# PKU-DAIR/SGL

Hardware: AMD Instinct MI355X
Metric: pre-prop SpMM throughput (edge·featdim/s), ogbn-products k=3, 1/2/4/8 GPU (higher is better)
Workload: dtype f32

## Files before the change

include/sgl_hip.h:

```cpp
#ifndef SGL_HIP_H
#define SGL_HIP_H

#include <stddef.h>
#include <stdint.h>

#ifdef __cplusplus
extern "C" {
#endif

#define SGL_OK 0
#define SGL_ERR_INVALID 1001
#define SGL_ERR_NO_DEVICE 1002
#define SGL_ERR_UNSUPPORTED 1003
#define SGL_ERR_ALLOC 1004

#define SGL_MAX_HOPS 64

int sgl_version(void);
const char *sgl_last_error(void);
int sgl_device_count(int *count);
int sgl_set_tuning(const char *key, int64_t value);
int sgl_get_tuning(const char *key, int64_t *value);

typedef struct sgl_plan sgl_plan_t;
int sgl_plan_build(sgl_plan_t **out, const int64_t *h_rowptr, int64_t n_rows, int32_t item_nnz, int32_t long_row_nnz);
int sgl_plan_counts(const sgl_plan_t *plan, int64_t counts[8]);
int sgl_plan_export(const sgl_plan_t *plan, int32_t *h_items, int64_t *h_piece_begin, int32_t *h_piece_len,
                    int32_t *h_piece_row, int32_t *h_long_row, int32_t *h_long_first);
void sgl_plan_destroy(sgl_plan_t *plan);

typedef struct sgl_csr sgl_csr_t;

#define SGL_CSR_STRICT_ORDER 0x1u
#define SGL_CSR_NO_XCD_REMAP 0x2u

int sgl_csr_create(sgl_csr_t **out, int64_t n_rows, int64_t n_cols, int64_t nnz, const int64_t *d_rowptr,
                   const int32_t *d_col, const float *d_val, uint32_t flags, int32_t item_nnz,
                   int32_t long_row_nnz, void *stream);
int sgl_csr_destroy(sgl_csr_t *csr);
int sgl_csr_set_values(sgl_csr_t *csr, const float *d_val);
int sgl_csr_info(const sgl_csr_t *csr, int64_t info[8]);

int sgl_spmm_f32(sgl_csr_t *csr, const float *d_x, int64_t ldx, float *d_y, int64_t ldy, int64_t d,
                 int accumulate, void *stream);

int sgl_spmm_multi_f32(sgl_csr_t *csr, const float *d_x, int64_t ldx, int n_out, float *const *h_y, int64_t ldy,
                       int64_t d, const uint8_t *d_row_mask, void *stream);

int sgl_spmm_chain_f32(sgl_csr_t *csr, int n_hops, const float *d_x0, int64_t ldx0, float *const *h_y,
                       const int64_t *h_ldy, int64_t d, void *stream);

typedef struct sgl_graph sgl_graph_t;
int sgl_chain_graph_create(sgl_graph_t **out, sgl_csr_t *csr, int n_hops, const float *d_x0, int64_t ldx0,
                           float *const *h_y, const int64_t *h_ldy, int64_t d);
int sgl_chain_graph_launch(sgl_graph_t *graph, void *stream);
int sgl_chain_graph_destroy(sgl_graph_t *graph);

int sgl_spmm_axpb_clamp_f32(sgl_csr_t *csr, const float *d_x, int64_t ldx, float *d_y, int64_t ldy, int64_t d,
                            float alpha, const float *d_res, int64_t ldres, float lo, float hi, void *stream);

enum { SGL_ACC_SUM = 0, SGL_ACC_WSUM = 1, SGL_ACC_MAX = 2, SGL_ACC_MIN = 3 };
int sgl_spmm_acc_f32(sgl_csr_t *csr, const float *d_x, int64_t ldx, float *d_y, int64_t ldy, int64_t d, float *d_acc,
                     int64_t ldacc, float w, int mode, float divisor, void *stream);

int sgl_spmm_bf16(sgl_csr_t *csr, const uint16_t *d_x, int64_t ldx, uint16_t *d_y, int64_t ldy, int64_t d, void *stream);
int sgl_spmm_chain_bf16(sgl_csr_t *csr, int n_hops, const uint16_t *d_x0, int64_t ldx0, uint16_t *const *h_y,
                        const int64_t *h_ldy, int64_t d, void *stream);
int sgl_spmm_acc_bf16(sgl_csr_t *csr, const uint16_t *d_x, int64_t ldx, uint16_t *d_y, int64_t ldy, int64_t d, float *d_acc,
                      int64_t ldacc, float w, int mode, float divisor, void *stream);
int sgl_gather_rows_bf16_f32(const uint16_t *d_x, int64_t ldx, int64_t n_rows, const int64_t *d_idx, int64_t n_idx, float *d_out,
                             int64_t ldo, int64_t d, int64_t pad_cols, void *stream);
int sgl_gather_hops_bf16_f32(int n_hops, const uint16_t *const *h_x, const int64_t *h_ldx, int64_t n_rows, const int64_t *d_idx,
                             int64_t n_idx, float *const *h_out, const int64_t *h_ldo, int64_t d, int64_t pad_cols, void *stream);

int sgl_hop_reduce_bf16_f32(int op, int n_hops, const uint16_t *const *h_x, const int64_t *h_ldx, const float *d_w, float *d_out,
                            int64_t ldo, int64_t pad_cols, int64_t n, int64_t d, void *stream);
int sgl_hop_concat_bf16(int n_hops, const uint16_t *const *h_x, const int64_t *h_ldx, uint16_t *d_out, int64_t ldo, int64_t pad_cols,
                        int64_t n, int64_t d, void *stream);
int sgl_hop_concat_bf16_f32(int n_hops, const uint16_t *const *h_x, const int64_t *h_ldx, float *d_out, int64_t ldo, int64_t pad_cols,
                            int64_t n, int64_t d, void *stream);
int sgl_nafs_bf16_f32(int n_hops, const uint16_t *const *h_x, const int64_t *h_ldx, float *d_out, int64_t ldo, int64_t pad_cols,
                      float *d_w_out, int64_t ldw, int64_t n, int64_t d, void *stream);

int sgl_download(void *h_dst, const void *d_src, int64_t bytes, void *stream);

int sgl_reorder_community(const int64_t *d_rowptr, const int32_t *d_col, int64_t n, int rounds, int64_t *d_order,
                          int64_t *h_info, void *stream);
int sgl_reorder_lpa_round(const int64_t *d_rowptr, const int32_t *d_col, int64_t n_local, int64_t row0, int64_t n_global,
                          const int32_t *d_labels, int32_t *d_out, int round, int last, uint64_t *d_moved, void *stream);

int sgl_csr_permute_rows(const int64_t *d_rowptr, const int32_t *d_col, const float *d_val, int64_t n, const int32_t *d_perm,
                         int64_t *d_out_rowptr, int32_t *d_out_col, float *d_out_val, void *stream);
int sgl_csr_set_rowmap(sgl_csr_t *csr, const int32_t *d_rowmap, void *stream);

int sgl_allgather_rows(void *nccl_comm, int rank, int world, const int64_t *h_bounds, float *d_x, int64_t ldx, void *stream);
int sgl_exchange_rows(void *nccl_comm, int rank, int world, const float *d_send, const int64_t *h_send_off, float *d_recv,
                      const int64_t *h_recv_off, int64_t ld, void *stream);
const char *sgl_exchange_backend(void);
int sgl_exchange_selftest(void *nccl_comm, int rank, const float *d_src, float *d_dst, int64_t n, int n_ops, void *stream);

void FloatCSRMulDenseOMP(float answer[], float data[], int indices[], int indptr[], float mat[], int mat_row,
                         int mat_col);
int FloatCSRMulDense(float answer[], int data_nnz, float data[], int indices[], int indptr[], float mat[],
                     int mat_row, int mat_col);

int sgl_shim_cache_stats(int64_t *hits, int64_t *misses);

int sgl_norm_prepare(int64_t n, int64_t nnz, const int64_t *d_rowptr, const int32_t *d_col, int64_t *nnz_out,
                     void *stream);
int sgl_norm_execute(int64_t n, int64_t nnz, const int64_t *d_rowptr, const int32_t *d_col, const float *d_val,
                     double r, int use_alpha, double alpha, int64_t nnz_out, int64_t *d_out_rowptr,
                     int32_t *d_out_col, float *d_out_val, double *d_out_val64, void *stream);

int sgl_norm_degrees(int64_t n, int64_t row0, const int64_t *d_rowptr, const int32_t *d_col, const float *d_val,
                     double *d_deg, void *stream);
int sgl_norm_execute_lr(int64_t n, int64_t nnz, const int64_t *d_rowptr, const int32_t *d_col, const float *d_val,
                        const double *d_left, const double *d_right, int use_alpha, double alpha, int64_t nnz_out,
                        int64_t *d_out_rowptr, int32_t *d_out_col, float *d_out_val, double *d_out_val64, void *stream);

int sgl_norm_block_prepare(int64_t n, int64_t row0, int64_t nnz, const int64_t *d_rowptr, const int32_t *d_col,
                           int64_t *nnz_out, void *stream);
int sgl_norm_block_build(int64_t n, int64_t row0, int64_t nnz, const int64_t *d_rowptr, const int32_t *d_col,
                         const float *d_val, int64_t nnz_out, int64_t *d_out_rowptr, int32_t *d_out_col,
                         double *d_out_val64, double *d_rowsum, void *stream);
int sgl_norm_build_symcheck(int64_t n, int64_t nnz, const int64_t *d_rowptr, const int32_t *d_col, const float *d_val,
                            int64_t nnz_out, int64_t *d_out_rowptr, int32_t *d_out_col, double *d_out_val64, double *d_rowsum,
                            uint64_t *d_sym_hash, void *stream);
int sgl_norm_block_colsum(int64_t n_cols, int64_t nnz, const int32_t *d_col, const double *d_val64, double *d_colsum,
                          void *stream);
int sgl_norm_block_scale(int64_t n, int64_t row0, const int64_t *d_rowptr, const int32_t *d_col, const double *d_val64,
                         const double *d_left_local, const double *d_right_global, int use_alpha, double alpha,
                         float *d_out_val, double *d_out_val64, void *stream);
int sgl_norm_block_mix(int64_t n, int64_t row0, const int64_t *d_rowptr, const int32_t *d_col, const double *d_hat64,
                       double alpha, float *d_out_val, double *d_out_val64, void *stream);
int sgl_norm_block_diag_positions(int64_t n, int64_t row0, const int64_t *d_rowptr, const int32_t *d_col, int64_t *d_diag, void *stream);
int sgl_norm_block_mix_at(int64_t nnz, int64_t n, const double *d_hat64, const int64_t *d_diag, double alpha, float *d_out_val,
                          double *d_out_val64, void *stream);
int sgl_norm_degree_powers(int64_t n, const double *d_deg, double r, double *d_left, double *d_right, void *stream);

int sgl_coo_to_csr(int64_t n_rows, int64_t n_cols, int64_t nnz, const int64_t *d_row, const int64_t *d_col,
                   const float *d_val, int64_t *d_out_rowptr, int32_t *d_out_col, float *d_out_val, int64_t *h_nnz_out,
                   void *stream);

#define SGL_REDUCE_SUM 0
#define SGL_REDUCE_MEAN 1
#define SGL_REDUCE_MAX 2
#define SGL_REDUCE_MIN 3
#define SGL_REDUCE_WSUM 4

int sgl_hop_reduce_f32(int op, int n_hops, const float *const *h_x, const int64_t *h_ldx, const float *d_w,
                       float *d_out, int64_t ldo, int64_t n, int64_t d, void *stream);
int sgl_hop_wsum2d_f32(int n_hops, const float *const *h_x, const int64_t *h_ldx, const float *d_w, int64_t ldw,
                       float *d_out, int64_t ldo, int64_t n, int64_t d, void *stream);
int sgl_hop_wsum2d_bwd_f32(int n_hops, const float *const *h_x, const int64_t *h_ldx, const float *d_w, int64_t ldw,
                           const float *d_dout, int64_t lddo, float *d_dw, int64_t lddw, float *const *h_dx,
                           const int64_t *h_lddx, int64_t n, int64_t d, void *stream);
int sgl_hop_rowdot_f32(int n_hops, const float *const *h_x, const int64_t *h_ldx, const float *d_vec, float *d_out,
                       int64_t ldo, int64_t n, int64_t d, void *stream);
int64_t sgl_hop_wsum1d_bwd_scratch(int n_hops);
int sgl_hop_wsum1d_bwd_f32(int n_hops, const float *const *h_x, const int64_t *h_ldx, const float *d_dout,
                           int64_t lddo, float *d_dw, float *d_scratch, int64_t n, int64_t d, void *stream);
int sgl_hop_lincomb_f32(int n_in, const float *const *h_x, const int64_t *h_ldx, int n_out, float *const *h_out, const int64_t *h_ldo,
                        const float *d_w, int64_t ldw, int64_t n, int64_t d, void *stream);
int sgl_hop_select_bwd_f32(int op, int n_hops, const float *const *h_x, const int64_t *h_ldx, const float *d_gout, int64_t ldg,
                           float *const *h_dx, const int64_t *h_lddx, int64_t n, int64_t d, void *stream);
int sgl_hop_concat_f32(int n_hops, const float *const *h_x, const int64_t *h_ldx, float *d_out, int64_t ldo,
                       int64_t n, int64_t d, void *stream);
int sgl_hop_concat_padded_f32(int n_hops, const float *const *h_x, const int64_t *h_ldx, float *d_out, int64_t ldo,
                              int64_t pad_cols, int64_t n, int64_t d, void *stream);
int sgl_nafs_f32(int n_hops, const float *const *h_x, const int64_t *h_ldx, float *d_out, int64_t ldo,
                 float *d_w_out, int64_t ldw, int64_t n, int64_t d, void *stream);
int sgl_nafs_padded_f32(int n_hops, const float *const *h_x, const int64_t *h_ldx, float *d_out, int64_t ldo, int64_t pad_cols,
                        float *d_w_out, int64_t ldw, int64_t n, int64_t d, void *stream);
int sgl_nafs_prefix_f32(int n_hops, const float *const *h_x, const int64_t *h_ldx, uint64_t emit_mask, float *const *h_out,
                        const int64_t *h_ldo, int64_t pad_cols, int combine, float divisor, int64_t n, int64_t d, void *stream);

int sgl_hop_gate_f32(int n_hops, const float *const *h_x, const int64_t *h_ldx, const float *d_vec, float bias, float *d_out,
                     int64_t ldo, float *d_w_out, int64_t ldw, float *d_g_out, int64_t ldg, int64_t n, int64_t d, void *stream);
int sgl_hop_gate_padded_f32(int n_hops, const float *const *h_x, const int64_t *h_ldx, const float *d_vec, float bias, float *d_out,
                            int64_t ldo, int64_t pad_cols, float *d_w_out, int64_t ldw, float *d_g_out, int64_t ldg, int64_t n,
                            int64_t d, void *stream);
int sgl_hop_recursive_f32(int n_hops, const float *const *h_x, const int64_t *h_ldx, const float *d_vec, float bias, float *d_out,
                          int64_t ldo, int64_t pad_cols, float *d_w_out, int64_t ldw, float *d_a_out, int64_t lda, float *d_c_out,
                          int64_t ldc, int64_t n, int64_t d, void *stream);
int sgl_hop_recursive_bwd_f32(int n_hops, const float *d_a, int64_t lda, const float *d_c, int64_t ldc, float bias, const float *d_bias,
                              const float *d_gw, int64_t ldg, float *d_da, int64_t ldda, float *d_dc, int64_t lddc, float *d_db,
                              int64_t n, void *stream);
int64_t sgl_hop_colsum_scratch(int n_hops, int64_t n, int64_t d);
int sgl_hop_colsum_f32(int n_hops, const float *const *h_x, const int64_t *h_ldx, const float *d_w, int64_t ldw, int sw, float *d_out,
                       int64_t ldo, float *d_scratch, int64_t n, int64_t d, void *stream);
int sgl_hop_rowdot2_f32(int n_hops, const float *const *h_x, const int64_t *h_ldx, const float *d_u, int64_t ldu, uint64_t u_mask,
                        const float *d_vec, int h0, int h1, float *d_p, int64_t ldp, float *d_a, int64_t n, int64_t d, void *stream);
int sgl_gather_rows_f32(const float *d_x, int64_t ldx, int64_t n_rows, const int64_t *d_idx, int64_t n_idx,
                        float *d_out, int64_t ldo, int64_t d, void *stream);
int sgl_gather_rows_padded_f32(const float *d_x, int64_t ldx, int64_t n_rows, const int64_t *d_idx, int64_t n_idx, float *d_out,
                               int64_t ldo, int64_t d, int64_t pad_cols, void *stream);
int sgl_gather_hops_padded_f32(int n_hops, const float *const *h_x, const int64_t *h_ldx, int64_t n_rows, const int64_t *d_idx,
                               int64_t n_idx, float *const *h_out, const int64_t *h_ldo, int64_t d, int64_t pad_cols, void *stream);
int sgl_scatter_rows_f32(const float *d_x, int64_t ldx, int64_t n_rows, const int64_t *d_src, const int64_t *d_dst,
                         int64_t n_idx, float *d_out, int64_t ldo, int64_t n_out_rows, int64_t d, void *stream);

int sgl_edge_dot_f32(const float *d_a, int64_t lda, int64_t n_a, const float *d_b, int64_t ldb, int64_t n_b,
                     const int64_t *d_edges, int64_t n_edges, int64_t d, float *d_out, void *stream);

int sgl_col_signature_f32(const float *d_x, int64_t ldx, int64_t n, int64_t d, uint64_t *d_sig, void *stream);

int sgl_content_hash(const void *h_ptr, int64_t bytes, uint64_t *out);

#ifdef __cplusplus
}
#endif
#endif
```

sgl_amd/_lib.py:

```python
import ctypes
import os
from ctypes import POINTER, c_char_p, c_double, c_float, c_int, c_int32, c_int64, c_uint32, c_uint64, c_void_p

import torch

_HERE = os.path.dirname(os.path.abspath(__file__))
LIB_PATH = os.environ.get("SGL_HIP_LIB") or os.path.join(_HERE, "csrc", "libsgl_hip.so")

SGL_CSR_STRICT_ORDER = 0x1
SGL_CSR_NO_XCD_REMAP = 0x2
SGL_REDUCE_SUM, SGL_REDUCE_MEAN, SGL_REDUCE_MAX, SGL_REDUCE_MIN, SGL_REDUCE_WSUM = 0, 1, 2, 3, 4
SGL_MAX_HOPS = 64
SGL_ERR_UNSUPPORTED = 1003
SGL_MEM_DEFAULT, SGL_MEM_CONTIGUOUS, SGL_MEM_VMM = 0, 1, 2

_lib = None

PROTOTYPES = {
    "sgl_version": (c_int, []),
    "sgl_last_error": (c_char_p, []),
    "sgl_device_count": (c_int, [POINTER(c_int)]),
    "sgl_set_tuning": (c_int, [c_char_p, c_int64]),
    "sgl_get_tuning": (c_int, [c_char_p, POINTER(c_int64)]),
    "sgl_plan_build": (c_int, [POINTER(c_void_p), c_void_p, c_int64, c_int32, c_int32]),
    "sgl_plan_counts": (c_int, [c_void_p, POINTER(c_int64)]),
    "sgl_plan_export": (c_int, [c_void_p, c_void_p, c_void_p, c_void_p, c_void_p, c_void_p, c_void_p]),
    "sgl_plan_destroy": (None, [c_void_p]),
    "sgl_csr_create": (c_int, [POINTER(c_void_p), c_int64, c_int64, c_int64, c_void_p, c_void_p, c_void_p, c_uint32,
                               c_int32, c_int32, c_void_p]),
    "sgl_csr_destroy": (c_int, [c_void_p]),
    "sgl_csr_set_values": (c_int, [c_void_p, c_void_p]),
    "sgl_csr_info": (c_int, [c_void_p, POINTER(c_int64)]),
    "sgl_spmm_f32": (c_int, [c_void_p, c_void_p, c_int64, c_void_p, c_int64, c_int64, c_int, c_void_p]),
    "sgl_spmm_multi_f32": (c_int, [c_void_p, c_void_p, c_int64, c_int, c_void_p, c_int64, c_int64, c_void_p, c_void_p]),
    "sgl_spmm_chain_f32": (c_int, [c_void_p, c_int, c_void_p, c_int64, c_void_p, c_void_p, c_int64, c_void_p]),
    "sgl_chain_graph_create": (c_int, [POINTER(c_void_p), c_void_p, c_int, c_void_p, c_int64, c_void_p, c_void_p, c_int64]),
    "sgl_chain_graph_launch": (c_int, [c_void_p, c_void_p]),
    "sgl_chain_graph_destroy": (c_int, [c_void_p]),
    "sgl_spmm_axpb_clamp_f32": (c_int, [c_void_p, c_void_p, c_int64, c_void_p, c_int64, c_int64, c_float, c_void_p, c_int64,
                                        c_float, c_float, c_void_p]),
    "sgl_spmm_acc_f32": (c_int, [c_void_p, c_void_p, c_int64, c_void_p, c_int64, c_int64, c_void_p, c_int64, c_float, c_int,
                                 c_float, c_void_p]),
    "sgl_spmm_bf16": (c_int, [c_void_p, c_void_p, c_int64, c_void_p, c_int64, c_int64, c_void_p]),
    "sgl_spmm_chain_bf16": (c_int, [c_void_p, c_int, c_void_p, c_int64, c_void_p, c_void_p, c_int64, c_void_p]),
    "sgl_spmm_acc_bf16": (c_int, [c_void_p, c_void_p, c_int64, c_void_p, c_int64, c_int64, c_void_p, c_int64, c_float, c_int,
                                  c_float, c_void_p]),
    "sgl_gather_rows_bf16_f32": (c_int, [c_void_p, c_int64, c_int64, c_void_p, c_int64, c_void_p, c_int64, c_int64, c_int64,
                                         c_void_p]),
    "sgl_gather_hops_bf16_f32": (c_int, [c_int, c_void_p, c_void_p, c_int64, c_void_p, c_int64, c_void_p, c_void_p, c_int64, c_int64,
                                         c_void_p]),
    "sgl_hop_reduce_bf16_f32": (c_int, [c_int, c_int, c_void_p, c_void_p, c_void_p, c_void_p, c_int64, c_int64, c_int64, c_int64,
                                        c_void_p]),
    "sgl_hop_concat_bf16": (c_int, [c_int, c_void_p, c_void_p, c_void_p, c_int64, c_int64, c_int64, c_int64, c_void_p]),
    "sgl_hop_concat_bf16_f32": (c_int, [c_int, c_void_p, c_void_p, c_void_p, c_int64, c_int64, c_int64, c_int64, c_void_p]),
    "sgl_nafs_bf16_f32": (c_int, [c_int, c_void_p, c_void_p, c_void_p, c_int64, c_int64, c_void_p, c_int64, c_int64, c_int64,
                                  c_void_p]),
    "sgl_allgather_rows": (c_int, [c_void_p, c_int, c_int, c_void_p, c_void_p, c_int64, c_void_p]),
    "sgl_exchange_rows": (c_int, [c_void_p, c_int, c_int, c_void_p, c_void_p, c_void_p, c_void_p, c_int64, c_void_p]),
    "sgl_exchange_backend": (c_char_p, []),
    "sgl_exchange_selftest": (c_int, [c_void_p, c_int, c_void_p, c_void_p, c_int64, c_int, c_void_p]),
    "FloatCSRMulDenseOMP": (None, [c_void_p, c_void_p, c_void_p, c_void_p, c_void_p, c_int, c_int]),
    "FloatCSRMulDense": (c_int, [c_void_p, c_int, c_void_p, c_void_p, c_void_p, c_void_p, c_int, c_int]),
    "sgl_shim_cache_stats": (c_int, [POINTER(c_int64), POINTER(c_int64)]),
    "sgl_norm_prepare": (c_int, [c_int64, c_int64, c_void_p, c_void_p, POINTER(c_int64), c_void_p]),
    "sgl_norm_execute": (c_int, [c_int64, c_int64, c_void_p, c_void_p, c_void_p, c_double, c_int, c_double, c_int64,
                                 c_void_p, c_void_p, c_void_p, c_void_p, c_void_p]),
    "sgl_norm_degrees": (c_int, [c_int64, c_int64, c_void_p, c_void_p, c_void_p, c_void_p, c_void_p]),
    "sgl_norm_execute_lr": (c_int, [c_int64, c_int64, c_void_p, c_void_p, c_void_p, c_void_p, c_void_p, c_int, c_double,
                                    c_int64, c_void_p, c_void_p, c_void_p, c_void_p, c_void_p]),
    "sgl_norm_block_prepare": (c_int, [c_int64, c_int64, c_int64, c_void_p, c_void_p, POINTER(c_int64), c_void_p]),
    "sgl_norm_block_build": (c_int, [c_int64, c_int64, c_int64, c_void_p, c_void_p, c_void_p, c_int64, c_void_p, c_void_p,
                                     c_void_p, c_void_p, c_void_p]),
    "sgl_norm_build_symcheck": (c_int, [c_int64, c_int64, c_void_p, c_void_p, c_void_p, c_int64, c_void_p, c_void_p, c_void_p,
                                        c_void_p, c_void_p, c_void_p]),
    "sgl_norm_block_colsum": (c_int, [c_int64, c_int64, c_void_p, c_void_p, c_void_p, c_void_p]),
    "sgl_norm_block_scale": (c_int, [c_int64, c_int64, c_void_p, c_void_p, c_void_p, c_void_p, c_void_p, c_int, c_double,
                                     c_void_p, c_void_p, c_void_p]),
    "sgl_norm_block_mix": (c_int, [c_int64, c_int64, c_void_p, c_void_p, c_void_p, c_double, c_void_p, c_void_p, c_void_p]),
    "sgl_norm_block_diag_positions": (c_int, [c_int64, c_int64, c_void_p, c_void_p, c_void_p, c_void_p]),
    "sgl_norm_block_mix_at": (c_int, [c_int64, c_int64, c_void_p, c_void_p, c_double, c_void_p, c_void_p, c_void_p]),
    "sgl_norm_degree_powers": (c_int, [c_int64, c_void_p, c_double, c_void_p, c_void_p, c_void_p]),
    "sgl_coo_to_csr": (c_int, [c_int64, c_int64, c_int64, c_void_p, c_void_p, c_void_p, c_void_p, c_void_p, c_void_p,
                               POINTER(c_int64), c_void_p]),
    "sgl_download": (c_int, [c_void_p, c_void_p, c_int64, c_void_p]),
    "sgl_csr_permute_rows": (c_int, [c_void_p, c_void_p, c_void_p, c_int64, c_void_p, c_void_p, c_void_p, c_void_p, c_void_p]),
    "sgl_csr_set_rowmap": (c_int, [c_void_p, c_void_p, c_void_p]),
    "sgl_reorder_lpa_round": (c_int, [c_void_p, c_void_p, c_int64, c_int64, c_int64, c_void_p, c_void_p, c_int, c_int, c_void_p, c_void_p]),
    "sgl_reorder_community": (c_int, [c_void_p, c_void_p, c_int64, c_int, c_void_p, POINTER(c_int64), c_void_p]),
    "sgl_hop_reduce_f32": (c_int, [c_int, c_int, c_void_p, c_void_p, c_void_p, c_void_p, c_int64, c_int64, c_int64,
                                   c_void_p]),
    "sgl_hop_lincomb_f32": (c_int, [c_int, c_void_p, c_void_p, c_int, c_void_p, c_void_p, c_void_p, c_int64, c_int64, c_int64, c_void_p]),
    "sgl_hop_select_bwd_f32": (c_int, [c_int, c_int, c_void_p, c_void_p, c_void_p, c_int64, c_void_p, c_void_p, c_int64, c_int64,
                                       c_void_p]),
    "sgl_hop_wsum2d_f32": (c_int, [c_int, c_void_p, c_void_p, c_void_p, c_int64, c_void_p, c_int64, c_int64, c_int64,
                                   c_void_p]),
    "sgl_hop_wsum2d_bwd_f32": (c_int, [c_int, c_void_p, c_void_p, c_void_p, c_int64, c_void_p, c_int64, c_void_p,
                                       c_int64, c_void_p, c_void_p, c_int64, c_int64, c_void_p]),
    "sgl_hop_rowdot_f32": (c_int, [c_int, c_void_p, c_void_p, c_void_p, c_void_p, c_int64, c_int64, c_int64, c_void_p]),
    "sgl_hop_gate_f32": (c_int, [c_int, c_void_p, c_void_p, c_void_p, c_float, c_void_p, c_int64, c_void_p, c_int64, c_void_p,
                                 c_int64, c_int64, c_int64, c_void_p]),
    "sgl_hop_rowdot2_f32": (c_int, [c_int, c_void_p, c_void_p, c_void_p, c_int64, c_uint64, c_void_p, c_int, c_int, c_void_p,
                                    c_int64, c_void_p, c_int64, c_int64, c_void_p]),
    "sgl_hop_colsum_scratch": (c_int64, [c_int, c_int64, c_int64]),
    "sgl_hop_colsum_f32": (c_int, [c_int, c_void_p, c_void_p, c_void_p, c_int64, c_int, c_void_p, c_int64, c_void_p, c_int64, c_int64,
                                   c_void_p]),
    "sgl_hop_wsum1d_bwd_scratch": (c_int64, [c_int]),
    "sgl_hop_wsum1d_bwd_f32": (c_int, [c_int, c_void_p, c_void_p, c_void_p, c_int64, c_void_p, c_void_p, c_int64,
                                       c_int64, c_void_p]),
    "sgl_hop_concat_f32": (c_int, [c_int, c_void_p, c_void_p, c_void_p, c_int64, c_int64, c_int64, c_void_p]),
    "sgl_hop_concat_padded_f32": (c_int, [c_int, c_void_p, c_void_p, c_void_p, c_int64, c_int64, c_int64, c_int64, c_void_p]),
    "sgl_nafs_f32": (c_int, [c_int, c_void_p, c_void_p, c_void_p, c_int64, c_void_p, c_int64, c_int64, c_int64,
                             c_void_p]),
    "sgl_nafs_padded_f32": (c_int, [c_int, c_void_p, c_void_p, c_void_p, c_int64, c_int64, c_void_p, c_int64, c_int64, c_int64,
                                    c_void_p]),
    "sgl_nafs_prefix_f32": (c_int, [c_int, c_void_p, c_void_p, c_uint64, c_void_p, c_void_p, c_int64, c_int, c_float, c_int64, c_int64,
                                    c_void_p]),
    "sgl_hop_gate_padded_f32": (c_int, [c_int, c_void_p, c_void_p, c_void_p, c_float, c_void_p, c_int64, c_int64, c_void_p, c_int64,
                                        c_void_p, c_int64, c_int64, c_int64, c_void_p]),
    "sgl_hop_recursive_f32": (c_int, [c_int, c_void_p, c_void_p, c_void_p, c_float, c_void_p, c_int64, c_int64, c_void_p, c_int64,
                                      c_void_p, c_int64, c_void_p, c_int64, c_int64, c_int64, c_void_p]),
    "sgl_hop_recursive_bwd_f32": (c_int, [c_int, c_void_p, c_int64, c_void_p, c_int64, c_float, c_void_p, c_void_p, c_int64, c_void_p,
                                          c_int64, c_void_p, c_int64, c_void_p, c_int64, c_void_p]),
    "sgl_gather_rows_f32": (c_int, [c_void_p, c_int64, c_int64, c_void_p, c_int64, c_void_p, c_int64, c_int64,
                                    c_void_p]),
    "sgl_gather_rows_padded_f32": (c_int, [c_void_p, c_int64, c_int64, c_void_p, c_int64, c_void_p, c_int64, c_int64, c_int64,
                                           c_void_p]),
    "sgl_gather_hops_padded_f32": (c_int, [c_int, c_void_p, c_void_p, c_int64, c_void_p, c_int64, c_void_p, c_void_p, c_int64, c_int64,
                                           c_void_p]),
    "sgl_scatter_rows_f32": (c_int, [c_void_p, c_int64, c_int64, c_void_p, c_void_p, c_int64, c_void_p, c_int64, c_int64,
                                     c_int64, c_void_p]),
    "sgl_edge_dot_f32": (c_int, [c_void_p, c_int64, c_int64, c_void_p, c_int64, c_int64, c_void_p, c_int64, c_int64, c_void_p,
                                 c_void_p]),
    "sgl_col_signature_f32": (c_int, [c_void_p, c_int64, c_int64, c_int64, c_void_p, c_void_p]),
    "sgl_content_hash": (c_int, [c_void_p, c_int64, POINTER(c_uint64)]),
}


PROBE_LIB_PATH = os.environ.get("SGL_PROBE_LIB") or os.path.join(_HERE, "csrc", "libsgl_probe.so")
PROBE_PROTOTYPES = {
    "sgl_probe_last_error": (c_char_p, []),
    "sgl_synth_degrees": (c_int, [c_uint64, c_int64, c_int64, c_void_p, c_void_p, c_void_p]),
    "sgl_synth_fill": (c_int, [c_uint64, c_int64, c_int64, c_int64, c_void_p, c_void_p, c_void_p, c_void_p]),
    "sgl_synth_features": (c_int, [c_uint64, c_int64, c_int64, c_int64, c_int64, c_void_p, c_void_p]),
    "sgl_mem_alloc": (c_int, [POINTER(c_void_p), c_int64, c_int, c_int64]),
    "sgl_mem_free": (c_int, [c_void_p]),
    "sgl_probe_stream_f32": (c_int, [c_void_p, c_int64, c_void_p, c_void_p]),
    "sgl_probe_gather_f32": (c_int, [c_void_p, c_int64, c_void_p, c_int64, c_int, c_int, c_void_p, c_void_p]),
}
_probe = None


class SglHipError(RuntimeError):
    pass


def lib():
    global _lib
    if _lib is None:
        if not os.path.exists(LIB_PATH):
            raise SglHipError(
                f"{LIB_PATH} is missing: build it with `python -m sgl_amd.csrc.build` (needs hipcc). "
                "sgl_amd has no CPU fallback for the propagation hot path.")
        handle = ctypes.CDLL(LIB_PATH)
        for name, (res, args) in PROTOTYPES.items():
            fn = getattr(handle, name)
            fn.restype = res
            fn.argtypes = args
        _lib = handle
    return _lib


def probe_lib():
    global _probe
    if _probe is None:
        if not os.path.exists(PROBE_LIB_PATH):
            raise SglHipError(f"{PROBE_LIB_PATH} is missing: build it with `python -m sgl_amd.csrc.build` (needs hipcc)")
        handle = ctypes.CDLL(PROBE_LIB_PATH)
        for name, (res, args) in PROBE_PROTOTYPES.items():
            fn = getattr(handle, name)
            fn.restype = res
            fn.argtypes = args
        _probe = handle
    return _probe


def check_probe(rc, what=""):
    if rc != 0:
        raise SglHipError(f"{what or 'libsgl_probe'} failed (code {rc}): {probe_lib().sgl_probe_last_error().decode('utf-8', 'replace')}")


def last_error():
    return lib().sgl_last_error().decode("utf-8", "replace")


def check(rc, what=""):
    if rc != 0:
        raise SglHipError(f"{what or 'libsgl_hip'} failed (code {rc}): {last_error()}")


def device_count():
    n = c_int(0)
    check(lib().sgl_device_count(ctypes.byref(n)), "sgl_device_count")
    return n.value


def require_gpu():
    if not torch.cuda.is_available() or device_count() < 1:
        raise SglHipError("no MI355X/HIP device visible: the sgl_amd propagation path is GPU-only (no CPU fallback)")


def set_tuning(key, value):
    check(lib().sgl_set_tuning(key.encode(), int(value)), f"sgl_set_tuning({key})")


def get_tuning(key):
    v = c_int64(0)
    check(lib().sgl_get_tuning(key.encode(), ctypes.byref(v)), f"sgl_get_tuning({key})")
    return v.value


def current_stream_ptr():
    return ctypes.c_void_p(torch.cuda.current_stream().cuda_stream)


def ptr(t):
    return ctypes.c_void_p(t.data_ptr())


def hop_arrays(tensors):
    n = len(tensors)
    ptrs = (c_void_p * n)(*[t.data_ptr() for t in tensors])
    lds = (c_int64 * n)(*[t.stride(0) if t.shape[0] > 1 else max(t.shape[1], t.stride(0)) for t in tensors])
    return ptrs, lds


def content_hash(arr):
    import numpy as np
    a = np.ascontiguousarray(arr)
    h = c_uint64(0)
    check(lib().sgl_content_hash(c_void_p(a.ctypes.data), a.nbytes, ctypes.byref(h)), "sgl_content_hash")
    return int(h.value)
```

sgl_amd/csrc/sgl_common.h:

```cpp
#pragma once
#include <hip/hip_runtime.h>

#include <cstdarg>
#include <cstdint>
#include <cstdio>
#include <cstring>
#include <string>
#include <vector>

#include "../../include/sgl_hip.h"

#define SGL_EXPORT extern "C" __attribute__((visibility("default")))

namespace sgl {

void set_error(const char *fmt, ...) __attribute__((format(printf, 1, 2)));
const char *get_error();

inline int fail(int code, const char *fmt, ...) __attribute__((format(printf, 2, 3)));
inline int fail(int code, const char *fmt, ...) {
    char buf[512];
    va_list ap;
    va_start(ap, fmt);
    vsnprintf(buf, sizeof(buf), fmt, ap);
    va_end(ap);
    set_error("%s", buf);
    return code;
}

#define SGL_HIP_CHECK(expr)                                                                          \
    do {                                                                                             \
        hipError_t _e = (expr);                                                                      \
        if (_e != hipSuccess)                                                                        \
            return ::sgl::fail((int)_e, "%s failed: %s (%s:%d)", #expr, hipGetErrorString(_e), __FILE__, \
                               __LINE__);                                                            \
    } while (0)

#define SGL_REQUIRE(cond, ...)                                     \
    do {                                                           \
        if (!(cond)) return ::sgl::fail(SGL_ERR_INVALID, __VA_ARGS__); \
    } while (0)

struct Piece {
    int64_t begin;
    int32_t len;
    int32_t row;
};

struct Plan {
    int64_t n_rows = 0;
    std::vector<int32_t> items;
    std::vector<Piece> pieces;
    std::vector<int32_t> long_row;
    std::vector<int32_t> long_first;
    int64_t max_item_rows = 0, max_item_nnz = 0;
};

constexpr int kMaxItemRows = 63;
constexpr int kDefaultItemNnz = 512;
constexpr int kDefaultLongRowNnz = 2048;
constexpr int64_t kSmallLaunchNnz = 100000000;

int build_plan(Plan &plan, const int64_t *rowptr, int64_t n_rows, int32_t item_nnz, int32_t long_row_nnz);

int64_t tuning(const char *key, int64_t dflt);

int32_t default_item_nnz(int64_t nnz);
int32_t default_long_row_nnz(int64_t nnz);

struct SpmmLayout {
    int group, nch, ulevel, waves;
    bool nt;
};
SpmmLayout spmm_layout(int lanes, bool strict, int64_t nnz, int64_t n_rows, bool bf16);

constexpr int unroll_of(int group, int nch, int ulevel) {
    const int uh = (nch == 1) ? 8 : (nch == 2 ? 4 : 2);
    return ulevel == 2 ? uh * 2 / (nch == 1 ? 1 : 2) : ulevel == 3 ? ((nch == 1 && group == 64) ? 32 : uh) : ulevel == 0 ? uh / 2 : uh;
}

struct RowLayout {
    int lpr, ch;
};
struct RowInstance {
    int lpr, ch, hmax;
};
int pick_lpr(int64_t d, int vec);
RowLayout row_layout(int64_t d, int n_hops, bool allow_8x5 = false);
RowInstance row_instance(int64_t d, int n_hops, bool allow_8x5 = false);
int out_cols(int64_t d, int64_t pad, int64_t room);
int check_pad(const char *who, int64_t width, int64_t pad, int64_t ldo);

inline hipStream_t as_stream(void *s) { return reinterpret_cast<hipStream_t>(s); }

inline bool launch_fits(int64_t blocks, int64_t threads_per_block) {
    return blocks >= 0 && blocks * threads_per_block < ((int64_t)1 << 32) && blocks < (int64_t)INT32_MAX;
}

}

inline bool aligned_to(const void *p, size_t a) { return (reinterpret_cast<uintptr_t>(p) % a) == 0; }

struct sgl_plan {
    sgl::Plan p;
};
```

sgl_amd/csrc/sgl_core.cpp:

```cpp
#include <algorithm>
#include <atomic>
#include <map>
#include <mutex>
#include <thread>

#include "sgl_common.h"

namespace sgl {

static thread_local std::string g_err;

void set_error(const char *fmt, ...) {
    char buf[512];
    va_list ap;
    va_start(ap, fmt);
    vsnprintf(buf, sizeof(buf), fmt, ap);
    va_end(ap);
    g_err = buf;
}
const char *get_error() { return g_err.c_str(); }

static std::mutex g_tune_mu;
static std::map<std::string, int64_t> &tune_map() {
    static std::map<std::string, int64_t> m = {
        {"spmm_unroll", 0},
        {"spmm_vec", 0},
        {"spmm_nt", 0},
        {"spmm_group", 0},
        {"spmm_waves", 0},
        {"spmm_xcd_remap", 1},
        {"spmm_heavy_first", 1},
        {"agg_blocks", 0},
        {"nafs_fused", 1},
        {"row_lpr32x2", 1},
        {"row_whole_lines", 1},
        {"row_narrow_groups", 1},
        {"gather_lpr", 0},
        {"gather_hops_grid", 1},
        {"gather_rows_per_thread", 0},
        {"concat_flat_read", 1},
        {"concat_lds", 1},
    };
    return m;
}

int64_t tuning(const char *key, int64_t dflt) {
    std::lock_guard<std::mutex> lk(g_tune_mu);
    auto &m = tune_map();
    auto it = m.find(key);
    if (it == m.end()) return dflt;
    return it->second;
}

int32_t default_item_nnz(int64_t nnz) {
    const int64_t want_items = 256 * 4 * 8;
    const int64_t cap = nnz >= kSmallLaunchNnz ? kDefaultItemNnz : kDefaultItemNnz / 2;
    return (int32_t)std::min<int64_t>(cap, std::max<int64_t>(16, nnz / want_items));
}

int32_t default_long_row_nnz(int64_t nnz) {
    return nnz < (1 << 18) ? 32 : nnz < (1 << 20) ? 128 : nnz < (1 << 22) ? 512 : kDefaultLongRowNnz;
}

SpmmLayout spmm_layout(int lanes, bool strict, int64_t nnz, int64_t n_rows, bool bf16) {
    SpmmLayout L;
    L.group = 64;
    L.nch = 1;
    if (lanes > 64) {
        const int need = (lanes + 63) / 64;
        L.nch = need <= 2 ? need : 4;
    } else if (!strict && lanes <= 16) {
        L.group = 8;
        while (L.group < lanes) L.group <<= 1;
    }
    const int64_t forced = tuning("spmm_group", 0);
    if (!strict && (forced == 8 || forced == 16 || forced == 32 || forced == 64) && L.nch == 1 && forced >= lanes) L.group = (int)forced;
    const bool whole_wave = L.group == 64 && L.nch == 1;
    L.ulevel = whole_wave ? 2 : 1;
    if (L.nch == 1 && n_rows > 0) {
        const double avg = (double)nnz / (double)n_rows;
        if (whole_wave) {
            if (avg < 12.0) L.ulevel = 0;
            else if (avg < 40.0) L.ulevel = 1;
        } else {
            L.ulevel = bf16 ? (avg >= 40.0 ? 2 : 1) : 1;
        }
    }
    const int64_t un = tuning("spmm_unroll", 0);
    if (un == 1) L.ulevel = 0;
    if (un == 2) L.ulevel = 2;
    if (un == 3) L.ulevel = 1;
    if (un == 4) L.ulevel = bf16 ? L.ulevel : 3;
    L.nt = bf16 ? false : tuning("spmm_nt", 0) != 0;
    L.waves = (int)tuning("spmm_waves", 0);
    if (L.waves != 1 && L.waves != 2 && L.waves != 4) L.waves = 4;
    return L;
}

int pick_lpr(int64_t d, int vec) {
    const int64_t lanes = (d + vec - 1) / vec;
    int lpr = 8;
    while (lpr < lanes && lpr < 64) lpr <<= 1;
    return lpr;
}

static const int kNarrow[2][3] = {{16, 3, 12}, {8, 5, 6}};

RowLayout row_layout(int64_t d, int n_hops, bool allow_8x5) {
    RowLayout r;
    r.lpr = pick_lpr(d, 4);
    r.ch = (d > r.lpr * 4) ? 2 : 1;
    if (r.lpr == 64 && r.ch == 1 && d > 128 && tuning("row_lpr32x2", 1) != 0) {
        r.lpr = 32;
        r.ch = 2;
    }
    if (tuning("row_narrow_groups", 1) != 0 && d <= r.lpr * 4 * r.ch) {
        const int slots = (int)((d + 3) / 4);
        const int64_t mode = tuning("row_narrow_groups", 1);
        for (const auto &c : kNarrow) {
            const int idle = c[0] * c[1] - slots;
            if (((mode == 2 || !allow_8x5) && c[0] == 8) || (mode == 3 && c[0] == 16)) continue;
            if (idle >= 0 && n_hops <= c[2] && 2 * idle <= r.lpr * r.ch - slots) {
                r.lpr = c[0];
                r.ch = c[1];
            }
        }
    }
    return r;
}

RowInstance row_instance(int64_t d, int n_hops, bool allow_8x5) {
    const RowLayout r = row_layout(d, n_hops, allow_8x5);
    int most = 16;
    for (const auto &c : kNarrow)
        if (r.lpr == c[0] && r.ch == c[1]) most = c[2];
    const int hmax = (n_hops < 1 || n_hops > most) ? 0 : std::max(2, (n_hops + 1) / 2 * 2);
    return RowInstance{r.lpr, r.ch, hmax};
}

int out_cols(int64_t d, int64_t pad, int64_t room) {
    int64_t dw = tuning("row_whole_lines", 1) != 0 ? d + pad : d;
    if (dw > room) dw = room > d ? room / 4 * 4 : d;
    if (dw > d && dw % 4 != 0) dw = d;
    return (int)dw;
}

int check_pad(const char *who, int64_t width, int64_t pad, int64_t ldo) {
    if (pad < 0 || width + pad > ldo) return fail(SGL_ERR_INVALID, "%s: pad_cols=%lld does not fit the output pitch", who, (long long)pad);
    if (pad > 0 && ((width + pad) % 4 != 0 || ldo % 4 != 0))
        return fail(SGL_ERR_INVALID, "%s: padded rows must be whole 16-byte vectors (width + pad_cols and ldo multiples of 4)", who);
    return SGL_OK;
}

static void heavy_items_first(Plan &plan, const int64_t *rowptr, int32_t item_nnz) {
    const int64_t n = (int64_t)plan.items.size() / 2;
    if (n < 64) return;
    const int64_t range = (((n + 3) / 4 + 7) / 8) * 4;
    const int64_t heavy = 2 * (int64_t)std::max(item_nnz, 1);
    struct It {
        int32_t b, e;
        int64_t nnz;
    };
    std::vector<It> seg;
    for (int64_t lo = 0; lo < n; lo += range) {
        const int64_t hi = std::min(n, lo + range);
        seg.clear();
        for (int64_t i = lo; i < hi; ++i) {
            const int32_t b = plan.items[2 * i], e = plan.items[2 * i + 1];
            seg.push_back(It{b, e, rowptr[e] - rowptr[b]});
        }
        auto mid = std::stable_partition(seg.begin(), seg.end(), [&](const It &t) { return t.nnz >= heavy; });
        std::stable_sort(seg.begin(), mid, [](const It &x, const It &y) { return x.nnz > y.nnz; });
        for (int64_t i = lo; i < hi; ++i) {
            plan.items[2 * i] = seg[(size_t)(i - lo)].b;
            plan.items[2 * i + 1] = seg[(size_t)(i - lo)].e;
        }
    }
}

static int build_segment(Plan &plan, const int64_t *rowptr, int64_t r0, int64_t r1, int32_t item_nnz, int32_t long_row_nnz) {
    const bool split = long_row_nnz > 0;
    int64_t cur_begin = r0, cur_nnz = 0;
    auto close_item = [&](int64_t end) {
        if (end > cur_begin) {
            plan.items.push_back((int32_t)cur_begin);
            plan.items.push_back((int32_t)end);
            plan.max_item_rows = std::max<int64_t>(plan.max_item_rows, end - cur_begin);
            plan.max_item_nnz = std::max<int64_t>(plan.max_item_nnz, cur_nnz);
        }
        cur_begin = end;
        cur_nnz = 0;
    };
    for (int64_t r = r0; r < r1; ++r) {
        const int64_t b = rowptr[r], e = rowptr[r + 1];
        if (e < b) return fail(SGL_ERR_INVALID, "build_plan: row pointers decrease at row %lld", (long long)r);
        const int64_t deg = e - b;
        if (!split && deg >= (int64_t)INT32_MAX)
            return fail(SGL_ERR_UNSUPPORTED, "build_plan: a row with >= 2^31 non-zeros needs long_row_nnz > 0");
        if (split && deg > long_row_nnz) {
            close_item(r);
            plan.long_row.push_back((int32_t)r);
            for (int64_t p = b; p < e; p += long_row_nnz) {
                Piece pc;
                pc.begin = p;
                pc.len = (int32_t)std::min<int64_t>(long_row_nnz, e - p);
                pc.row = (int32_t)r;
                plan.pieces.push_back(pc);
            }
            plan.long_first.push_back((int32_t)plan.pieces.size());
            cur_begin = r + 1;
            cur_nnz = 0;
            continue;
        }
        if (cur_nnz > 0 && cur_nnz + deg >= (int64_t)INT32_MAX) close_item(r);
        cur_nnz += deg;
        if (cur_nnz >= item_nnz || (r + 1 - cur_begin) >= kMaxItemRows) close_item(r + 1);
    }
    close_item(r1);
    return SGL_OK;
}

constexpr int64_t kPlanSegmentRows = (int64_t)1 << 20;

int build_plan(Plan &plan, const int64_t *rowptr, int64_t n_rows, int32_t item_nnz, int32_t long_row_nnz) {
    if (n_rows < 0 || (n_rows > 0 && rowptr == nullptr)) return fail(SGL_ERR_INVALID, "build_plan: bad arguments");
    if (n_rows >= (int64_t)INT32_MAX) return fail(SGL_ERR_UNSUPPORTED, "build_plan: n_rows >= 2^31 (shard the matrix)");
    if (item_nnz <= 0) item_nnz = kDefaultItemNnz;
    plan = Plan();
    plan.n_rows = n_rows;
    plan.long_first.push_back(0);
    if (n_rows <= 2 * kPlanSegmentRows) {
        const int rc = build_segment(plan, rowptr, 0, n_rows, item_nnz, long_row_nnz);
        if (rc != SGL_OK) return rc;
    } else {
        const int64_t n_seg = (n_rows + kPlanSegmentRows - 1) / kPlanSegmentRows;
        std::vector<Plan> segs((size_t)n_seg);
        std::vector<int> rcs((size_t)n_seg, SGL_OK);
        std::vector<std::string> errs((size_t)n_seg);
        const int n_thr = (int)std::max<int64_t>(1, std::min<int64_t>({(int64_t)std::thread::hardware_concurrency(), (int64_t)16, n_seg}));
        std::atomic<int64_t> next{0};
        auto work = [&]() {
            for (int64_t sidx = next.fetch_add(1); sidx < n_seg; sidx = next.fetch_add(1)) {
                const int64_t r0 = sidx * kPlanSegmentRows, r1 = std::min(n_rows, r0 + kPlanSegmentRows);
                rcs[(size_t)sidx] = build_segment(segs[(size_t)sidx], rowptr, r0, r1, item_nnz, long_row_nnz);
                if (rcs[(size_t)sidx] != SGL_OK) errs[(size_t)sidx] = get_error();
            }
        };
        std::vector<std::thread> team;
        for (int t = 1; t < n_thr; ++t) team.emplace_back(work);
        work();
        for (auto &t : team) t.join();
        size_t n_items = 0, n_pieces = 0, n_long = 0;
        for (int64_t sidx = 0; sidx < n_seg; ++sidx) {
            if (rcs[(size_t)sidx] != SGL_OK) return fail(rcs[(size_t)sidx], "%s", errs[(size_t)sidx].c_str());
            n_items += segs[(size_t)sidx].items.size();
            n_pieces += segs[(size_t)sidx].pieces.size();
            n_long += segs[(size_t)sidx].long_row.size();
        }
        plan.items.reserve(n_items);
        plan.pieces.reserve(n_pieces);
        plan.long_row.reserve(n_long);
        plan.long_first.reserve(n_long + 1);
        for (auto &sg : segs) {
            const int32_t piece0 = (int32_t)plan.pieces.size();
            plan.items.insert(plan.items.end(), sg.items.begin(), sg.items.end());
            plan.pieces.insert(plan.pieces.end(), sg.pieces.begin(), sg.pieces.end());
            plan.long_row.insert(plan.long_row.end(), sg.long_row.begin(), sg.long_row.end());
            for (int32_t lf : sg.long_first) plan.long_first.push_back(piece0 + lf);
            plan.max_item_rows = std::max(plan.max_item_rows, sg.max_item_rows);
            plan.max_item_nnz = std::max(plan.max_item_nnz, sg.max_item_nnz);
            sg = Plan();
        }
    }
    if (tuning("spmm_heavy_first", 1) != 0) heavy_items_first(plan, rowptr, item_nnz);
    return SGL_OK;
}

}

SGL_EXPORT int sgl_version(void) { return 103; }

SGL_EXPORT const char *sgl_last_error(void) { return sgl::get_error(); }

SGL_EXPORT int sgl_device_count(int *count) {
    if (!count) return sgl::fail(SGL_ERR_INVALID, "sgl_device_count: NULL");
    int n = 0;
    hipError_t e = hipGetDeviceCount(&n);
    if (e != hipSuccess) {
        (void)hipGetLastError();
        n = 0;
    }
    *count = n;
    return SGL_OK;
}

SGL_EXPORT int sgl_set_tuning(const char *key, int64_t value) {
    if (!key) return sgl::fail(SGL_ERR_INVALID, "sgl_set_tuning: NULL key");
    std::lock_guard<std::mutex> lk(sgl::g_tune_mu);
    auto &m = sgl::tune_map();
    auto it = m.find(key);
    if (it == m.end()) return sgl::fail(SGL_ERR_INVALID, "sgl_set_tuning: unknown key '%s'", key);
    it->second = value;
    return SGL_OK;
}

SGL_EXPORT int sgl_get_tuning(const char *key, int64_t *value) {
    if (!key || !value) return sgl::fail(SGL_ERR_INVALID, "sgl_get_tuning: NULL");
    std::lock_guard<std::mutex> lk(sgl::g_tune_mu);
    auto &m = sgl::tune_map();
    auto it = m.find(key);
    if (it == m.end()) return sgl::fail(SGL_ERR_INVALID, "sgl_get_tuning: unknown key '%s'", key);
    *value = it->second;
    return SGL_OK;
}

SGL_EXPORT int sgl_plan_build(sgl_plan_t **out, const int64_t *h_rowptr, int64_t n_rows, int32_t item_nnz,
                              int32_t long_row_nnz) {
    if (!out) return sgl::fail(SGL_ERR_INVALID, "sgl_plan_build: NULL out");
    *out = nullptr;
    sgl_plan_t *p = new (std::nothrow) sgl_plan_t();
    if (!p) return sgl::fail(SGL_ERR_ALLOC, "sgl_plan_build: out of memory");
    int rc = sgl::build_plan(p->p, h_rowptr, n_rows, item_nnz, long_row_nnz);
    if (rc != SGL_OK) {
        delete p;
        return rc;
    }
    *out = p;
    return SGL_OK;
}

SGL_EXPORT int sgl_plan_counts(const sgl_plan_t *plan, int64_t counts[8]) {
    if (!plan || !counts) return sgl::fail(SGL_ERR_INVALID, "sgl_plan_counts: NULL");
    memset(counts, 0, 8 * sizeof(int64_t));
    counts[0] = (int64_t)plan->p.items.size() / 2;
    counts[1] = (int64_t)plan->p.pieces.size();
    counts[2] = (int64_t)plan->p.long_row.size();
    counts[3] = plan->p.max_item_rows;
    counts[4] = plan->p.max_item_nnz;
    counts[5] = plan->p.n_rows;
    return SGL_OK;
}

SGL_EXPORT int sgl_plan_export(const sgl_plan_t *plan, int32_t *h_items, int64_t *h_piece_begin, int32_t *h_piece_len,
                               int32_t *h_piece_row, int32_t *h_long_row, int32_t *h_long_first) {
    if (!plan) return sgl::fail(SGL_ERR_INVALID, "sgl_plan_export: NULL plan");
    const sgl::Plan &p = plan->p;
    if (h_items && !p.items.empty()) memcpy(h_items, p.items.data(), p.items.size() * sizeof(int32_t));
    for (size_t i = 0; i < p.pieces.size(); ++i) {
        if (h_piece_begin) h_piece_begin[i] = p.pieces[i].begin;
        if (h_piece_len) h_piece_len[i] = p.pieces[i].len;
        if (h_piece_row) h_piece_row[i] = p.pieces[i].row;
    }
    if (h_long_row && !p.long_row.empty()) memcpy(h_long_row, p.long_row.data(), p.long_row.size() * sizeof(int32_t));
    if (h_long_first) memcpy(h_long_first, p.long_first.data(), p.long_first.size() * sizeof(int32_t));
    return SGL_OK;
}

SGL_EXPORT void sgl_plan_destroy(sgl_plan_t *plan) { delete plan; }
```

sgl_amd/csrc/sgl_csr.h:

```cpp
#pragma once
#include "sgl_common.h"

#include <atomic>
#include <memory>

struct sgl_csr {
    int64_t n_rows = 0, n_cols = 0, nnz = 0;
    const int64_t *d_rowptr = nullptr;
    const int32_t *d_col = nullptr;
    const float *d_val = nullptr;
    uint32_t flags = 0;
    int64_t n_items = 0, n_pieces = 0, n_long = 0;
    int32_t *d_items = nullptr;
    sgl::Piece *d_pieces = nullptr;
    int32_t *d_long_row = nullptr;
    int32_t *d_long_first = nullptr;
    float *d_partial = nullptr;
    size_t partial_cap = 0;
    std::vector<float *> retired;
    int device = 0;
    const int32_t *d_rowmap = nullptr;
    int32_t *d_long_out = nullptr;
    std::shared_ptr<std::atomic<uint64_t>> epoch = std::make_shared<std::atomic<uint64_t>>(0);
};
```

sgl_amd/csrc/sgl_csr.hip:

```cpp
#include "sgl_csr.h"

__global__ __launch_bounds__(256) void rowmap_check_kernel(const int32_t *__restrict__ map, const int64_t n, unsigned *__restrict__ seen,
                                                           int *__restrict__ bad) {
    const int64_t i = (int64_t)blockIdx.x * blockDim.x + threadIdx.x;
    if (i >= n) return;
    const int32_t m = map[i];
    if (m < 0 || m >= n) {
        atomicOr(bad, 1);
        return;
    }
    const unsigned bit = 1u << (m & 31);
    if (atomicOr(&seen[m >> 5], bit) & bit) atomicOr(bad, 2);
}

static int fetch_rowptr(std::vector<int64_t> &h, const int64_t *d, hipStream_t st) {
    const size_t n = h.size();
    constexpr size_t kChunk = (size_t)4 << 20;
    if (n <= 2 * kChunk) {
        SGL_HIP_CHECK(hipMemcpyAsync(h.data(), d, n * sizeof(int64_t), hipMemcpyDeviceToHost, st));
        SGL_HIP_CHECK(hipStreamSynchronize(st));
        return SGL_OK;
    }
    int64_t *stage[2] = {nullptr, nullptr};
    hipEvent_t ev[2] = {nullptr, nullptr};
    int rc = SGL_OK;
    auto cleanup = [&]() {
        for (int i = 0; i < 2; ++i) {
            if (stage[i]) (void)hipHostFree(stage[i]);
            if (ev[i]) (void)hipEventDestroy(ev[i]);
        }
    };
    for (int i = 0; i < 2 && rc == SGL_OK; ++i) {
        if (hipHostMalloc((void **)&stage[i], kChunk * sizeof(int64_t), hipHostMallocDefault) != hipSuccess ||
            hipEventCreateWithFlags(&ev[i], hipEventDisableTiming) != hipSuccess)
            rc = sgl::fail(SGL_ERR_ALLOC, "sgl_csr_create: no page-locked staging buffer for the row pointers");
    }
    const size_t n_chunks = (n + kChunk - 1) / kChunk;
    auto issue = [&](size_t c) -> hipError_t {
        const size_t off = c * kChunk, len = std::min(kChunk, n - off);
        hipError_t e = hipMemcpyAsync(stage[c & 1], d + off, len * sizeof(int64_t), hipMemcpyDeviceToHost, st);
        return e != hipSuccess ? e : hipEventRecord(ev[c & 1], st);
    };
    if (rc == SGL_OK && issue(0) != hipSuccess) rc = sgl::fail(SGL_ERR_INVALID, "sgl_csr_create: copying the row pointers failed");
    for (size_t c = 0; c < n_chunks && rc == SGL_OK; ++c) {
        if (hipEventSynchronize(ev[c & 1]) != hipSuccess) {
            rc = sgl::fail(SGL_ERR_INVALID, "sgl_csr_create: copying the row pointers failed");
            break;
        }
        const size_t off = c * kChunk, len = std::min(kChunk, n - off);
        if (c + 1 < n_chunks && issue(c + 1) != hipSuccess) {
            rc = sgl::fail(SGL_ERR_INVALID, "sgl_csr_create: copying the row pointers failed");
            break;
        }
        memcpy(h.data() + off, stage[c & 1], len * sizeof(int64_t));
    }
    if (rc != SGL_OK) (void)hipStreamSynchronize(st);
    cleanup();
    return rc;
}

SGL_EXPORT int sgl_csr_create(sgl_csr_t **out, int64_t n_rows, int64_t n_cols, int64_t nnz, const int64_t *d_rowptr,
                              const int32_t *d_col, const float *d_val, uint32_t flags, int32_t item_nnz,
                              int32_t long_row_nnz, void *stream) {
    if (!out) return sgl::fail(SGL_ERR_INVALID, "sgl_csr_create: NULL out");
    *out = nullptr;
    SGL_REQUIRE(n_rows >= 0 && n_cols >= 0 && nnz >= 0, "sgl_csr_create: negative size");
    SGL_REQUIRE(n_rows < INT32_MAX && n_cols < INT32_MAX, "sgl_csr_create: n_rows/n_cols must be < 2^31 (int32 ids)");
    SGL_REQUIRE(d_rowptr != nullptr, "sgl_csr_create: NULL row pointers");
    SGL_REQUIRE(nnz == 0 || (d_col && d_val), "sgl_csr_create: NULL col/val with nnz > 0");
    hipStream_t st = sgl::as_stream(stream);
    std::vector<int64_t> h_rowptr((size_t)n_rows + 1);
    {
        const int rc_fetch = fetch_rowptr(h_rowptr, d_rowptr, st);
        if (rc_fetch != SGL_OK) return rc_fetch;
    }
    SGL_REQUIRE(h_rowptr[0] == 0 && h_rowptr[n_rows] == nnz, "sgl_csr_create: rowptr[0]=%lld rowptr[n]=%lld but nnz=%lld",
                (long long)h_rowptr[0], (long long)h_rowptr[n_rows], (long long)nnz);
    if (item_nnz <= 0) item_nnz = sgl::default_item_nnz(nnz);
    if (long_row_nnz == 0) long_row_nnz = sgl::default_long_row_nnz(nnz);
    if (flags & SGL_CSR_STRICT_ORDER) long_row_nnz = -1;
    sgl::Plan plan;
    int rc = sgl::build_plan(plan, h_rowptr.data(), n_rows, item_nnz, long_row_nnz);
    if (rc != SGL_OK) return rc;

    sgl_csr_t *h = new (std::nothrow) sgl_csr_t();
    if (!h) return sgl::fail(SGL_ERR_ALLOC, "sgl_csr_create: out of memory");
    h->n_rows = n_rows;
    h->n_cols = n_cols;
    h->nnz = nnz;
    h->d_rowptr = d_rowptr;
    h->d_col = d_col;
    h->d_val = d_val;
    h->flags = flags;
    h->n_items = (int64_t)plan.items.size() / 2;
    h->n_pieces = (int64_t)plan.pieces.size();
    h->n_long = (int64_t)plan.long_row.size();
    (void)hipGetDevice(&h->device);
    auto upload = [&](void **dst, const void *src, size_t bytes) -> int {
        if (bytes == 0) return SGL_OK;
        SGL_HIP_CHECK(hipMalloc(dst, bytes));
        SGL_HIP_CHECK(hipMemcpyAsync(*dst, src, bytes, hipMemcpyHostToDevice, st));
        return SGL_OK;
    };
    rc = upload((void **)&h->d_items, plan.items.data(), plan.items.size() * sizeof(int32_t));
    if (rc == SGL_OK) rc = upload((void **)&h->d_pieces, plan.pieces.data(), plan.pieces.size() * sizeof(sgl::Piece));
    if (rc == SGL_OK) rc = upload((void **)&h->d_long_row, plan.long_row.data(), plan.long_row.size() * sizeof(int32_t));
    if (rc == SGL_OK && h->n_long > 0)
        rc = upload((void **)&h->d_long_first, plan.long_first.data(), plan.long_first.size() * sizeof(int32_t));
    if (rc == SGL_OK) {
        hipError_t e = hipStreamSynchronize(st);
        if (e != hipSuccess) rc = sgl::fail((int)e, "sgl_csr_create: sync failed: %s", hipGetErrorString(e));
    }
    if (rc != SGL_OK) {
        sgl_csr_destroy(h);
        return rc;
    }
    *out = h;
    return SGL_OK;
}

SGL_EXPORT int sgl_csr_destroy(sgl_csr_t *h) {
    if (!h) return SGL_OK;
    h->epoch->store(~0ull);
    (void)hipFree(h->d_items);
    (void)hipFree(h->d_pieces);
    (void)hipFree(h->d_long_row);
    (void)hipFree(h->d_long_first);
    (void)hipFree(h->d_partial);
    (void)hipFree(h->d_long_out);
    for (float *p : h->retired) (void)hipFree(p);
    delete h;
    return SGL_OK;
}

SGL_EXPORT int sgl_csr_set_rowmap(sgl_csr_t *h, const int32_t *d_rowmap, void *stream) {
    if (!h) return sgl::fail(SGL_ERR_INVALID, "sgl_csr_set_rowmap: NULL handle");
    h->d_rowmap = nullptr;
    h->epoch->fetch_add(1);
    if (!d_rowmap || h->n_rows == 0) return SGL_OK;
    hipStream_t st = sgl::as_stream(stream);
    {
        const size_t words = (size_t)(h->n_rows + 31) / 32;
        unsigned *d_seen = nullptr;
        SGL_HIP_CHECK(hipMalloc(&d_seen, (words + 1) * sizeof(unsigned)));
        int *d_bad = reinterpret_cast<int *>(d_seen + words);
        hipError_t e = hipMemsetAsync(d_seen, 0, (words + 1) * sizeof(unsigned), st);
        int bad = 0;
        if (e == hipSuccess) {
            hipLaunchKernelGGL(rowmap_check_kernel, dim3((unsigned)((h->n_rows + 255) / 256)), dim3(256), 0, st, d_rowmap, h->n_rows, d_seen, d_bad);
            e = hipGetLastError();
        }
        if (e == hipSuccess) e = hipMemcpyAsync(&bad, d_bad, sizeof(int), hipMemcpyDeviceToHost, st);
        if (e == hipSuccess) e = hipStreamSynchronize(st);
        (void)hipFree(d_seen);
        if (e != hipSuccess) return sgl::fail((int)e, "sgl_csr_set_rowmap: validation failed: %s", hipGetErrorString(e));
        SGL_REQUIRE(!(bad & 1), "sgl_csr_set_rowmap: map entry outside [0, n_rows)");
        SGL_REQUIRE(!(bad & 2), "sgl_csr_set_rowmap: the map names an output row twice (it must be a permutation)");
    }
    if (h->n_long > 0) {
        std::vector<int32_t> map((size_t)h->n_rows), rows((size_t)h->n_long);
        SGL_HIP_CHECK(hipMemcpyAsync(map.data(), d_rowmap, map.size() * sizeof(int32_t), hipMemcpyDeviceToHost, st));
        SGL_HIP_CHECK(hipMemcpyAsync(rows.data(), h->d_long_row, rows.size() * sizeof(int32_t), hipMemcpyDeviceToHost, st));
        SGL_HIP_CHECK(hipStreamSynchronize(st));
        for (auto &r : rows) {
            SGL_REQUIRE(r >= 0 && r < h->n_rows && map[r] >= 0 && map[r] < h->n_rows, "sgl_csr_set_rowmap: map entry outside [0, n_rows)");
            r = map[r];
        }
        if (!h->d_long_out) SGL_HIP_CHECK(hipMalloc(&h->d_long_out, rows.size() * sizeof(int32_t)));
        SGL_HIP_CHECK(hipMemcpyAsync(h->d_long_out, rows.data(), rows.size() * sizeof(int32_t), hipMemcpyHostToDevice, st));
        SGL_HIP_CHECK(hipStreamSynchronize(st));
    }
    h->d_rowmap = d_rowmap;
    return SGL_OK;
}

SGL_EXPORT int sgl_csr_set_values(sgl_csr_t *h, const float *d_val) {
    if (!h) return sgl::fail(SGL_ERR_INVALID, "sgl_csr_set_values: NULL handle");
    SGL_REQUIRE(h->nnz == 0 || d_val, "sgl_csr_set_values: NULL values");
    if (d_val != h->d_val) h->epoch->fetch_add(1);
    h->d_val = d_val;
    return SGL_OK;
}

SGL_EXPORT int sgl_csr_info(const sgl_csr_t *h, int64_t info[8]) {
    if (!h || !info) return sgl::fail(SGL_ERR_INVALID, "sgl_csr_info: NULL");
    info[0] = h->n_rows;
    info[1] = h->n_cols;
    info[2] = h->nnz;
    info[3] = h->n_items;
    info[4] = h->n_pieces;
    info[5] = h->n_long;
    info[6] = h->flags;
    info[7] = (int64_t)(h->partial_cap * sizeof(float));
    return SGL_OK;
}
```

sgl_amd/csrc/sgl_spmm.hip:

```cpp
#include "sgl_spmm_common.h"

namespace {

template <int VEC>
struct VecT;
template <>
struct VecT<1> {
    using type = float;
};
template <>
struct VecT<2> {
    using type = float __attribute__((ext_vector_type(2)));
};
template <>
struct VecT<4> {
    using type = float __attribute__((ext_vector_type(4)));
};

template <int VEC>
__device__ __forceinline__ typename VecT<VEC>::type vzero() {
    typename VecT<VEC>::type z;
    if constexpr (VEC == 1) {
        z = 0.f;
    } else {
#pragma unroll
        for (int e = 0; e < VEC; ++e) z[e] = 0.f;
    }
    return z;
}

template <int VEC>
__device__ __forceinline__ void vfma(typename VecT<VEC>::type &acc, float v, const typename VecT<VEC>::type &x) {
    if constexpr (VEC == 1) {
        acc = __builtin_fmaf(v, x, acc);
    } else {
#pragma unroll
        for (int e = 0; e < VEC; ++e) acc[e] = __builtin_fmaf(v, x[e], acc[e]);
    }
}

template <int VEC>
__device__ __forceinline__ void vadd_xor(typename VecT<VEC>::type &acc, int off) {
    if constexpr (VEC == 1) {
        acc += __shfl_xor(acc, off, 64);
    } else {
#pragma unroll
        for (int e = 0; e < VEC; ++e) acc[e] += __shfl_xor(acc[e], off, 64);
    }
}

template <bool NT, typename T>
__device__ __forceinline__ T ld_stream(const T *p) {
    if constexpr (NT)
        return __builtin_nontemporal_load(p);
    else
        return *p;
}

template <bool NT, typename T>
__device__ __forceinline__ void st_stream(T *p, const T &v) {
    if constexpr (NT)
        __builtin_nontemporal_store(v, p);
    else
        *p = v;
}

struct SpmmArgs {
    const int32_t *items;
    const sgl::Piece *pieces;
    const int64_t *rowptr;
    const int32_t *col;
    const float *val;
    const float *x;
    float *y;
    float *partial;
    int64_t ldx, ldy, ldp;
    int32_t n_items, n_pieces, d, accumulate;
    BlockMap map;
    const float *res;
    int64_t ldres;
    float epi_alpha, epi_lo, epi_hi;
    int32_t epi;
    float *acc;
    int64_t ldacc;
    float acc_w, acc_div;
    int32_t acc_mode;
    float *y_more[7];
    int32_t n_more;
    const uint8_t *row_mask;
    const int32_t *rowmap;
};

struct MultiOut {
    float *p[7];
    int n;
    const uint8_t *mask;
};

struct Epilogue {
    const float *res = nullptr;
    float alpha = 1.f, lo = 0.f, hi = 0.f;
    int on = 0;
    float *acc = nullptr;
    int64_t ldacc = 0;
    float acc_w = 1.f, acc_div = 1.f;
    int acc_mode = 0;
};

__device__ __forceinline__ float acc_apply(float a, float y, const Epilogue &e) { return acc_apply(a, y, e.acc_mode, e.acc_w, e.acc_div); }

__device__ __forceinline__ float epi_apply(float v, float r, const Epilogue &e, bool has_res) {
    float t = __fmul_rn(e.alpha, v);
    if (has_res) t = __fadd_rn(t, r);
    return t < e.lo ? e.lo : (t > e.hi ? e.hi : t);
}

template <int VEC, int GROUP, int NCH, int U, bool NT, bool MULTI>
__device__ __forceinline__ void run_rows(const int32_t *__restrict__ colb, const float *__restrict__ valb,
                                         const int my_rel, const int nrows, const int tot,
                                         const float *__restrict__ x, const int64_t ldx, float *__restrict__ out,
                                         const int64_t ldo, const int d, const bool accumulate, const int lane,
                                         const Epilogue epi, const int64_t ldres, const MultiOut mo,
                                         const RowMap rm = RowMap()) {
    using V = typename VecT<VEC>::type;
    constexpr int R = 64 / GROUP;
    const int s = (R == 1) ? 0 : (lane / GROUP);
    const int l = lane % GROUP;
    int colofs[NCH];
    bool on[NCH];
#pragma unroll
    for (int ch = 0; ch < NCH; ++ch) {
        colofs[ch] = (ch * GROUP + l) * VEC;
        on[ch] = colofs[ch] < d;
    }
    int cbr = 0;
    int my_c = 0, nx_c = 0;
    float my_v = 0.f, nx_v = 0.f;
    if (lane < tot) {
        my_c = ld_stream<NT>(colb + lane);
        my_v = ld_stream<NT>(valb + lane);
    }
    if (64 + lane < tot) {
        nx_c = ld_stream<NT>(colb + 64 + lane);
        nx_v = ld_stream<NT>(valb + 64 + lane);
    }

    for (int ri = 0; ri < nrows; ++ri) {
        const int jb = __builtin_amdgcn_readlane(my_rel, ri);
        const int je = __builtin_amdgcn_readlane(my_rel, ri + 1);
        const int64_t ro = rm.on ? (int64_t)__builtin_amdgcn_readlane(rm.my_map, ri) : (int64_t)ri;
        float *orow = out + ro * ldo;
        V acc[NCH];
#pragma unroll
        for (int ch = 0; ch < NCH; ++ch) acc[ch] = vzero<VEC>();
        if (accumulate && s == 0) {
#pragma unroll
            for (int ch = 0; ch < NCH; ++ch)
                if (on[ch]) acc[ch] = *reinterpret_cast<const V *>(orow + colofs[ch]);
        }
        int j = jb;
        while (j < je) {
            const int lim = min(je, cbr + 64);
            const int o = j - cbr;
            const int cnt = lim - j;
            const int sh = (R == 1) ? 0 : ((s - (j - jb)) & (R - 1));
            int t = 0;
            for (; t + R * U <= cnt; t += R * U) {
                int c[U];
                float v[U];
                V xv[U][NCH];
#pragma unroll
                for (int u = 0; u < U; ++u) {
                    const int idx = o + t + u * R + sh;
                    c[u] = bcast_i<R>(my_c, idx);
                    v[u] = bcast_f<R>(my_v, idx);
                }
#pragma unroll
                for (int ch = 0; ch < NCH; ++ch) {
                    if (on[ch]) {
#pragma unroll
                        for (int u = 0; u < U; ++u)
                            xv[u][ch] = *reinterpret_cast<const V *>(x + (int64_t)c[u] * ldx + colofs[ch]);
                    } else {
#pragma unroll
                        for (int u = 0; u < U; ++u) xv[u][ch] = vzero<VEC>();
                    }
                }
#pragma unroll
                for (int u = 0; u < U; ++u)
#pragma unroll
                    for (int ch = 0; ch < NCH; ++ch) vfma<VEC>(acc[ch], v[u], xv[u][ch]);
            }
            for (; t < cnt; t += R) {
                const int idx = (o + t + sh) & 63;
                const bool valid = (t + sh) < cnt;
                const int c = bcast_i<R>(my_c, idx);
                const float v = bcast_f<R>(my_v, idx);
                if (valid) {
#pragma unroll
                    for (int ch = 0; ch < NCH; ++ch)
                        if (on[ch]) {
                            const V xv = *reinterpret_cast<const V *>(x + (int64_t)c * ldx + colofs[ch]);
                            vfma<VEC>(acc[ch], v, xv);
                        }
                }
            }
            j = lim;
            if (lim == cbr + 64) {
                cbr += 64;
                my_c = nx_c;
                my_v = nx_v;
                if (cbr + 64 + lane < tot) {
                    nx_c = ld_stream<NT>(colb + cbr + 64 + lane);
                    nx_v = ld_stream<NT>(valb + cbr + 64 + lane);
                }
            }
        }
        if constexpr (R > 1) {
#pragma unroll
            for (int off = GROUP; off < 64; off <<= 1)
#pragma unroll
                for (int ch = 0; ch < NCH; ++ch) vadd_xor<VEC>(acc[ch], off);
        }
        if (s == 0) {
#pragma unroll
            for (int ch = 0; ch < NCH; ++ch)
                if (on[ch]) {
                    V v = acc[ch];
                    if (epi.on) {
                        const bool has_res = epi.res != nullptr;
                        V r = vzero<VEC>();
                        if (has_res) r = *reinterpret_cast<const V *>(epi.res + ro * ldres + colofs[ch]);
                        if constexpr (VEC == 1) {
                            v = epi_apply(v, r, epi, has_res);
                        } else {
#pragma unroll
                            for (int e = 0; e < VEC; ++e) v[e] = epi_apply(v[e], r[e], epi, has_res);
                        }
                    }
                    if (epi.acc) {
                        float *ap = epi.acc + ro * epi.ldacc + colofs[ch];
                        V a = *reinterpret_cast<const V *>(ap);
                        if constexpr (VEC == 1) {
                            a = acc_apply(a, v, epi);
                        } else {
#pragma unroll
                            for (int e = 0; e < VEC; ++e) a[e] = acc_apply(a[e], v[e], epi);
                        }
                        *reinterpret_cast<V *>(ap) = a;
                    }
                    st_stream<NT>(reinterpret_cast<V *>(orow + colofs[ch]), v);
                    if constexpr (MULTI) {
                        const int need = mo.mask ? (int)mo.mask[ri] : 0x7f;
#pragma unroll
                        for (int q = 0; q < 7; ++q)
                            if (q < mo.n && ((need >> q) & 1))
                                *reinterpret_cast<V *>(mo.p[q] + ro * ldo + colofs[ch]) = v;
                    }
                }
        }
    }
}

template <int VEC, int GROUP, int NCH, int U, bool NT, bool MULTI>
__global__ __launch_bounds__(256) void spmm_kernel(const SpmmArgs a) {
    const int lane = threadIdx.x & 63;
    const int wave = __builtin_amdgcn_readfirstlane(threadIdx.x >> 6);
    const int b = blockIdx.x;
    if (b < a.map.piece_blocks) {
        const int p = b * a.map.waves + wave;
        if (p >= a.n_pieces) return;
        const sgl::Piece pc = a.pieces[p];
        const int my_rel = (lane == 0) ? 0 : pc.len;
        const Epilogue none;
        MultiOut solo;
        solo.n = 0;
        solo.mask = nullptr;
        run_rows<VEC, GROUP, NCH, U, NT, false>(a.col + pc.begin, a.val + pc.begin, my_rel, 1, pc.len, a.x, a.ldx,
                                         a.partial + (int64_t)p * a.ldp, a.ldp, a.d, false, lane, none, 0, solo);
    } else {
        int ib = b - a.map.piece_blocks;
        if (a.map.xcd_remap) ib = xcd_block(ib, a.map.item_blocks_per_xcd);
        const int item = ib * a.map.waves + wave;
        if (item >= a.n_items) return;
        const int row_begin = a.items[2 * item], row_end = a.items[2 * item + 1];
        const int nrows = row_end - row_begin;
        const ItemWindow w = item_window(a.rowptr, row_begin, nrows, lane);
        const RowMap rm = item_rowmap(a.rowmap, row_begin, nrows, lane);
        const int64_t first = rm.on ? 0 : row_begin;
        Epilogue epi;
        epi.res = a.res ? a.res + first * a.ldres : nullptr;
        epi.alpha = a.epi_alpha;
        epi.lo = a.epi_lo;
        epi.hi = a.epi_hi;
        epi.on = a.epi;
        epi.acc = a.acc ? a.acc + first * a.ldacc : nullptr;
        epi.ldacc = a.ldacc;
        epi.acc_w = a.acc_w;
        epi.acc_div = a.acc_div;
        epi.acc_mode = a.acc_mode;
        MultiOut mo;
        mo.n = MULTI ? a.n_more : 0;
        mo.mask = (MULTI && a.row_mask) ? a.row_mask + row_begin : nullptr;
#pragma unroll
        for (int q = 0; q < 7; ++q) mo.p[q] = (MULTI && q < a.n_more) ? a.y_more[q] + (int64_t)row_begin * a.ldy : nullptr;
        run_rows<VEC, GROUP, NCH, U, NT, MULTI>(a.col + w.base, a.val + w.base, w.my_rel, nrows, w.tot, a.x, a.ldx,
                                         a.y + first * a.ldy, a.ldy, a.d, a.accumulate != 0, lane, epi,
                                         a.ldres, mo, rm);
    }
}

__global__ __launch_bounds__(256) void spmm_fixup_kernel(const int32_t *__restrict__ long_row,
                                                         const int32_t *__restrict__ long_first,
                                                         const float *__restrict__ partial, int64_t ldp,
                                                         float *__restrict__ y, int64_t ldy, int d, int accumulate,
                                                         const float *__restrict__ res, int64_t ldres, Epilogue epi,
                                                         MultiOut mo) {
    const int kblocks = (d + 255) / 256;
    const int lr = blockIdx.x / kblocks;
    const int k = (blockIdx.x % kblocks) * 256 + threadIdx.x;
    if (k >= d) return;
    const int row = long_row[lr];
    const int p0 = long_first[lr], p1 = long_first[lr + 1];
    float *yp = y + (int64_t)row * ldy + k;
    float acc = accumulate ? *yp : 0.f;
    for (int p = p0; p < p1; ++p) acc += partial[(int64_t)p * ldp + k];
    if (epi.on) acc = epi_apply(acc, res ? res[(int64_t)row * ldres + k] : 0.f, epi, res != nullptr);
    if (epi.acc) {
        float *ap = epi.acc + (int64_t)row * epi.ldacc + k;
        *ap = acc_apply(*ap, acc, epi);
    }
    *yp = acc;
    const int need = mo.mask ? (int)mo.mask[row] : 0x7f;
#pragma unroll
    for (int q = 0; q < 7; ++q)
        if (q < mo.n && ((need >> q) & 1)) mo.p[q][(int64_t)row * ldy + k] = acc;
}

template <int VEC, int GROUP, int NCH, int U, bool NT>
hipError_t launch_variant(const SpmmArgs &a, int grid, hipStream_t st) {
    if (a.n_more > 0)
        hipLaunchKernelGGL((spmm_kernel<VEC, GROUP, NCH, U, NT, true>), dim3(grid), dim3(64 * a.map.waves), 0, st, a);
    else
        hipLaunchKernelGGL((spmm_kernel<VEC, GROUP, NCH, U, NT, false>), dim3(grid), dim3(64 * a.map.waves), 0, st, a);
    return hipGetLastError();
}

template <int VEC, int GROUP, int NCH, int U>
hipError_t launch_nt(const SpmmArgs &a, int grid, hipStream_t st, bool nt) {
    return nt ? launch_variant<VEC, GROUP, NCH, U, true>(a, grid, st)
              : launch_variant<VEC, GROUP, NCH, U, false>(a, grid, st);
}

template <int VEC, int GROUP, int NCH>
hipError_t launch_u(const SpmmArgs &a, int grid, hipStream_t st, bool nt, int ulevel) {
    using sgl::unroll_of;
    if (ulevel == 2) return launch_nt<VEC, GROUP, NCH, unroll_of(GROUP, NCH, 2)>(a, grid, st, nt);
    if (ulevel == 3) return launch_nt<VEC, GROUP, NCH, unroll_of(GROUP, NCH, 3)>(a, grid, st, nt);
    return ulevel == 0 ? launch_nt<VEC, GROUP, NCH, unroll_of(GROUP, NCH, 0)>(a, grid, st, nt)
                       : launch_nt<VEC, GROUP, NCH, unroll_of(GROUP, NCH, 1)>(a, grid, st, nt);
}

template <int VEC>
hipError_t launch_group(const SpmmArgs &a, int grid, hipStream_t st, bool nt, int ulevel, int group, int nch) {
    if (nch == 1) {
        switch (group) {
            case 8:
                return launch_u<VEC, 8, 1>(a, grid, st, nt, ulevel);
            case 16:
                return launch_u<VEC, 16, 1>(a, grid, st, nt, ulevel);
            case 32:
                return launch_u<VEC, 32, 1>(a, grid, st, nt, ulevel);
            default:
                return launch_u<VEC, 64, 1>(a, grid, st, nt, ulevel);
        }
    }
    if (nch == 2) return launch_u<VEC, 64, 2>(a, grid, st, nt, ulevel);
    return launch_u<VEC, 64, 4>(a, grid, st, nt, ulevel);
}

}

static int pick_vec(const float *d_x, int64_t ldx, const float *d_y, int64_t ldy, int64_t d) {
    if (d % 4 == 0 && ldx % 4 == 0 && ldy % 4 == 0 && aligned_to(d_x, 16) && aligned_to(d_y, 16)) return 4;
    if (d % 2 == 0 && ldx % 2 == 0 && ldy % 2 == 0 && aligned_to(d_x, 8) && aligned_to(d_y, 8)) return 2;
    return 1;
}

struct EpiHost {
    int on = 0;
    float alpha = 1.f, lo = 0.f, hi = 0.f;
    const float *res = nullptr;
    int64_t ldres = 0;
    int n_more = 0;
    float *y_more[7] = {nullptr, nullptr, nullptr, nullptr, nullptr, nullptr, nullptr};
    const uint8_t *row_mask = nullptr;
    float *acc = nullptr;
    int64_t ldacc = 0;
    float acc_w = 1.f, acc_div = 1.f;
    int acc_mode = 0;
};

static int spmm_slice(sgl_csr_t *h, const float *d_x, int64_t ldx, float *d_y, int64_t ldy, int d, int vec,
                      int accumulate, hipStream_t st, const EpiHost &eh, const char *who) {
    SpmmLaunch L;
    int rc = spmm_launch(L, h, d / vec, d, false, who);
    if (rc == SGL_OK) rc = grow_partial(h, L.ldp);
    if (rc != SGL_OK) return rc;
    if (L.grid == 0) return SGL_OK;

    SpmmArgs a;
    a.items = h->d_items;
    a.pieces = h->d_pieces;
    a.rowptr = h->d_rowptr;
    a.col = h->d_col;
    a.val = h->d_val;
    a.x = d_x;
    a.y = d_y;
    a.ldx = ldx;
    a.ldy = ldy;
    a.ldp = L.ldp;
    a.n_items = (int32_t)h->n_items;
    a.n_pieces = (int32_t)h->n_pieces;
    a.d = d;
    a.accumulate = accumulate;
    a.res = eh.res;
    a.ldres = eh.ldres;
    a.epi_alpha = eh.alpha;
    a.epi_lo = eh.lo;
    a.epi_hi = eh.hi;
    a.epi = eh.on;
    a.acc = eh.acc;
    a.ldacc = eh.ldacc;
    a.acc_w = eh.acc_w;
    a.acc_div = eh.acc_div;
    a.acc_mode = eh.acc_mode;
    a.n_more = eh.n_more;
    a.row_mask = eh.row_mask;
    for (int q = 0; q < 7; ++q) a.y_more[q] = eh.y_more[q];
    a.rowmap = h->d_rowmap;
    a.map = L.map;
    a.partial = h->d_partial;
    hipError_t e;
    if (vec == 4)
        e = launch_group<4>(a, L.grid, st, L.nt, L.ulevel, L.group, L.nch);
    else if (vec == 2)
        e = launch_group<2>(a, L.grid, st, L.nt, L.ulevel, L.group, L.nch);
    else
        e = launch_group<1>(a, L.grid, st, L.nt, L.ulevel, L.group, L.nch);
    if (e != hipSuccess) return sgl::fail((int)e, "%s: kernel launch failed: %s", who, hipGetErrorString(e));
    if (L.fixup_grid > 0) {
        Epilogue fe;
        fe.alpha = eh.alpha;
        fe.lo = eh.lo;
        fe.hi = eh.hi;
        fe.on = eh.on;
        fe.acc = eh.acc;
        fe.ldacc = eh.ldacc;
        fe.acc_w = eh.acc_w;
        fe.acc_div = eh.acc_div;
        fe.acc_mode = eh.acc_mode;
        MultiOut fmo;
        fmo.n = eh.n_more;
        fmo.mask = eh.row_mask;
        for (int q = 0; q < 7; ++q) fmo.p[q] = eh.y_more[q];
        hipLaunchKernelGGL(spmm_fixup_kernel, dim3((unsigned)L.fixup_grid), dim3(256), 0, st, h->d_rowmap ? h->d_long_out : h->d_long_row,
                           h->d_long_first, h->d_partial, a.ldp,
                           d_y, ldy, d, accumulate, eh.res, eh.ldres, fe, fmo);
        e = hipGetLastError();
        if (e != hipSuccess) return sgl::fail((int)e, "%s: fix-up launch failed: %s", who, hipGetErrorString(e));
    }
    return SGL_OK;
}

static int spmm_impl(sgl_csr_t *h, const float *d_x, int64_t ldx, float *d_y, int64_t ldy, int64_t d, int accumulate,
                     void *stream, EpiHost eh, const char *who) {
    if (!h) return sgl::fail(SGL_ERR_INVALID, "%s: NULL handle", who);
    SGL_REQUIRE(d >= 0 && d < INT32_MAX, "%s: bad d", who);
    if (d == 0 || h->n_rows == 0) return SGL_OK;
    SGL_REQUIRE(d_x && d_y, "%s: NULL X or Y", who);
    if (h->d_rowmap && eh.n_more > 0)
        return sgl::fail(SGL_ERR_UNSUPPORTED, "%s: a row-mapped handle does not support replicas", who);
    SGL_REQUIRE(ldx >= d && ldy >= d, "%s: leading dimension smaller than d", who);
    SGL_REQUIRE(aligned_to(d_x, 4) && aligned_to(d_y, 4), "%s: X/Y not 4-byte aligned", who);
    hipStream_t st = sgl::as_stream(stream);
    int vec = pick_vec(d_x, ldx, d_y, ldy, d);
    for (int q = 0; q < eh.n_more; ++q) {
        SGL_REQUIRE(eh.y_more[q] && aligned_to(eh.y_more[q], 4), "%s: bad replica pointer", who);
        if (vec == 4 && !aligned_to(eh.y_more[q], 16)) vec = aligned_to(eh.y_more[q], 8) && d % 2 == 0 ? 2 : 1;
        if (vec == 2 && !aligned_to(eh.y_more[q], 8)) vec = 1;
    }
    const int64_t vcap = sgl::tuning("spmm_vec", 0);
    if ((vcap == 1 || vcap == 2) && vcap < vec) vec = (int)vcap;
    if (eh.on && eh.res) {
        SGL_REQUIRE(eh.ldres >= d && aligned_to(eh.res, 4), "%s: bad residual matrix", who);
        if (vec == 4 && !(eh.ldres % 4 == 0 && aligned_to(eh.res, 16))) vec = (eh.ldres % 2 == 0 && aligned_to(eh.res, 8) && d % 2 == 0) ? 2 : 1;
        if (vec == 2 && !(eh.ldres % 2 == 0 && aligned_to(eh.res, 8))) vec = 1;
    }
    if (eh.acc) {
        SGL_REQUIRE(eh.ldacc >= d && aligned_to(eh.acc, 4), "%s: bad accumulator matrix", who);
        if (vec == 4 && !(eh.ldacc % 4 == 0 && aligned_to(eh.acc, 16))) vec = (eh.ldacc % 2 == 0 && aligned_to(eh.acc, 8) && d % 2 == 0) ? 2 : 1;
        if (vec == 2 && !(eh.ldacc % 2 == 0 && aligned_to(eh.acc, 8))) vec = 1;
    }
    const int64_t max_cols = 64 * 4 * vec;
    for (int64_t c0 = 0; c0 < d; c0 += max_cols) {
        const int dc = (int)std::min<int64_t>(max_cols, d - c0);
        EpiHost es = eh;
        if (es.res) es.res += c0;
        if (es.acc) es.acc += c0;
        for (int q = 0; q < es.n_more; ++q) es.y_more[q] += c0;
        int rc = spmm_slice(h, d_x + c0, ldx, d_y + c0, ldy, dc, vec, accumulate, st, es, who);
        if (rc != SGL_OK) return rc;
    }
    return SGL_OK;
}

SGL_EXPORT int sgl_spmm_f32(sgl_csr_t *h, const float *d_x, int64_t ldx, float *d_y, int64_t ldy, int64_t d,
                            int accumulate, void *stream) {
    return spmm_impl(h, d_x, ldx, d_y, ldy, d, accumulate, stream, EpiHost(), "sgl_spmm_f32");
}

SGL_EXPORT int sgl_spmm_multi_f32(sgl_csr_t *h, const float *d_x, int64_t ldx, int n_out, float *const *h_y, int64_t ldy,
                                  int64_t d, const uint8_t *d_row_mask, void *stream) {
    SGL_REQUIRE(n_out >= 1 && n_out <= 8 && h_y, "sgl_spmm_multi_f32: n_out must be in [1, 8]");
    EpiHost eh;
    eh.row_mask = d_row_mask;
    eh.n_more = n_out - 1;
    for (int q = 1; q < n_out; ++q) eh.y_more[q - 1] = h_y[q];
    return spmm_impl(h, d_x, ldx, h_y[0], ldy, d, 0, stream, eh, "sgl_spmm_multi_f32");
}

SGL_EXPORT int sgl_spmm_chain_f32(sgl_csr_t *h, int n_hops, const float *d_x0, int64_t ldx0, float *const *h_y,
                                  const int64_t *h_ldy, int64_t d, void *stream) {
    if (!h) return sgl::fail(SGL_ERR_INVALID, "sgl_spmm_chain_f32: NULL handle");
    SGL_REQUIRE(n_hops >= 0 && (n_hops == 0 || (h_y && h_ldy)), "sgl_spmm_chain_f32: bad hop arrays");
    SGL_REQUIRE(n_hops == 0 || h->n_rows == h->n_cols, "sgl_spmm_chain_f32: repeated products need a square matrix");
    const float *cur = d_x0;
    int64_t ldc = ldx0;
    for (int k = 0; k < n_hops; ++k) {
        int rc = spmm_impl(h, cur, ldc, h_y[k], h_ldy[k], d, 0, stream, EpiHost(), "sgl_spmm_chain_f32");
        if (rc != SGL_OK) return rc;
        cur = h_y[k];
        ldc = h_ldy[k];
    }
    return SGL_OK;
}

struct sgl_graph {
    hipGraph_t graph = nullptr;
    hipGraphExec_t exec = nullptr;
    std::shared_ptr<std::atomic<uint64_t>> epoch;
    uint64_t captured = 0;
};

SGL_EXPORT int sgl_chain_graph_create(sgl_graph_t **out, sgl_csr_t *h, int n_hops, const float *d_x0, int64_t ldx0,
                                      float *const *h_y, const int64_t *h_ldy, int64_t d) {
    if (!out) return sgl::fail(SGL_ERR_INVALID, "sgl_chain_graph_create: NULL out");
    *out = nullptr;
    SGL_REQUIRE(h && n_hops >= 1 && h_y && h_ldy, "sgl_chain_graph_create: bad arguments");
    int rc = sgl_spmm_chain_f32(h, n_hops, d_x0, ldx0, h_y, h_ldy, d, nullptr);
    if (rc != SGL_OK) return rc;
    SGL_HIP_CHECK(hipDeviceSynchronize());
    hipStream_t cap = nullptr;
    SGL_HIP_CHECK(hipStreamCreateWithFlags(&cap, hipStreamNonBlocking));
    sgl_graph_t *g = new (std::nothrow) sgl_graph_t();
    if (!g) {
        (void)hipStreamDestroy(cap);
        return sgl::fail(SGL_ERR_ALLOC, "sgl_chain_graph_create: out of memory");
    }
    hipError_t e = hipStreamBeginCapture(cap, hipStreamCaptureModeThreadLocal);
    if (e == hipSuccess) {
        rc = sgl_spmm_chain_f32(h, n_hops, d_x0, ldx0, h_y, h_ldy, d, cap);
        e = hipStreamEndCapture(cap, &g->graph);
        if (rc != SGL_OK && e == hipSuccess) e = hipErrorUnknown;
    }
    if (e == hipSuccess) e = hipGraphInstantiate(&g->exec, g->graph, nullptr, nullptr, 0);
    (void)hipStreamDestroy(cap);
    if (e != hipSuccess) {
        if (g->graph) (void)hipGraphDestroy(g->graph);
        delete g;
        return sgl::fail((int)e, "sgl_chain_graph_create: capture/instantiate failed: %s", hipGetErrorString(e));
    }
    g->epoch = h->epoch;
    g->captured = h->epoch->load();
    *out = g;
    return SGL_OK;
}

SGL_EXPORT int sgl_chain_graph_launch(sgl_graph_t *g, void *stream) {
    if (!g || !g->exec) return sgl::fail(SGL_ERR_INVALID, "sgl_chain_graph_launch: NULL graph");
    if (g->epoch && g->epoch->load() != g->captured)
        return sgl::fail(SGL_ERR_INVALID, "sgl_chain_graph_launch: the adjacency handle changed after the capture (new values / row map, "
                                          "or it was destroyed): capture the chain again");
    SGL_HIP_CHECK(hipGraphLaunch(g->exec, sgl::as_stream(stream)));
    return SGL_OK;
}

SGL_EXPORT int sgl_chain_graph_destroy(sgl_graph_t *g) {
    if (!g) return SGL_OK;
    if (g->exec) (void)hipGraphExecDestroy(g->exec);
    if (g->graph) (void)hipGraphDestroy(g->graph);
    delete g;
    return SGL_OK;
}

SGL_EXPORT int sgl_spmm_acc_f32(sgl_csr_t *h, const float *d_x, int64_t ldx, float *d_y, int64_t ldy, int64_t d, float *d_acc,
                                int64_t ldacc, float w, int mode, float divisor, void *stream) {
    EpiHost eh;
    const int rc = acc_mode_of("sgl_spmm_acc_f32", d_acc, mode, divisor, eh.acc_mode);
    if (rc != SGL_OK) return rc;
    eh.acc = d_acc;
    eh.ldacc = ldacc;
    eh.acc_w = w;
    eh.acc_div = divisor;
    return spmm_impl(h, d_x, ldx, d_y, ldy, d, 0, stream, eh, "sgl_spmm_acc_f32");
}

SGL_EXPORT int sgl_spmm_axpb_clamp_f32(sgl_csr_t *h, const float *d_x, int64_t ldx, float *d_y, int64_t ldy, int64_t d,
                                       float alpha, const float *d_res, int64_t ldres, float lo, float hi,
                                       void *stream) {
    EpiHost eh;
    eh.on = 1;
    eh.alpha = alpha;
    eh.lo = lo;
    eh.hi = hi;
    eh.res = d_res;
    eh.ldres = ldres;
    SGL_REQUIRE(!(lo > hi), "sgl_spmm_axpb_clamp_f32: lo > hi");
    return spmm_impl(h, d_x, ldx, d_y, ldy, d, 0, stream, eh, "sgl_spmm_axpb_clamp_f32");
}
```

sgl_amd/csrc/sgl_spmm_bf16.hip:

```cpp
#include "sgl_spmm_common.h"

namespace {

typedef float f2 __attribute__((ext_vector_type(2)));
typedef float f4 __attribute__((ext_vector_type(4)));
typedef __bf16 bf2 __attribute__((ext_vector_type(2)));
typedef uint32_t u2 __attribute__((ext_vector_type(2)));
typedef uint32_t u4 __attribute__((ext_vector_type(4)));

__device__ __forceinline__ uint32_t pack2(float a, float b) {
    const f2 v = {a, b};
    return __builtin_bit_cast(uint32_t, __builtin_convertvector(v, bf2));
}
__device__ __forceinline__ float widen_lo(uint32_t w) { return __uint_as_float(w << 16); }
__device__ __forceinline__ float widen_hi(uint32_t w) { return __uint_as_float(w & 0xffff0000u); }

template <int BV>
struct RawT;
template <>
struct RawT<8> {
    using type = u4;
};
template <>
struct RawT<4> {
// ... 5 lines not shown
};
template <>
struct RawT<1> {
    using type = uint16_t;
};

template <int BV>
__device__ __forceinline__ typename RawT<BV>::type rzero() {
    if constexpr (BV == 8)
        return (u4){0u, 0u, 0u, 0u};
    else if constexpr (BV == 4)
        return (u2){0u, 0u};
    else
        return 0;
}

template <int BV>
__device__ __forceinline__ void widen(const typename RawT<BV>::type &r, float (&f)[BV]) {
    if constexpr (BV == 1) {
        f[0] = __uint_as_float((uint32_t)r << 16);
    } else if constexpr (BV == 2) {
        f[0] = widen_lo(r);
        f[1] = widen_hi(r);
    } else {
#pragma unroll
        for (int w = 0; w < BV / 2; ++w) {
            f[2 * w] = widen_lo(r[w]);
            f[2 * w + 1] = widen_hi(r[w]);
        }
    }
}

template <int BV>
__device__ __forceinline__ typename RawT<BV>::type narrow(const float (&f)[BV]) {
    if constexpr (BV == 1) {
        return (uint16_t)(pack2(f[0], 0.f) & 0xffffu);
    } else if constexpr (BV == 2) {
        return pack2(f[0], f[1]);
    } else {
        typename RawT<BV>::type r;
#pragma unroll
        for (int w = 0; w < BV / 2; ++w) r[w] = pack2(f[2 * w], f[2 * w + 1]);
        return r;
    }
}

template <int BV>
__device__ __forceinline__ void load_f(const float *p, float (&f)[BV]) {
    if constexpr (BV >= 4) {
#pragma unroll
        for (int q = 0; q < BV / 4; ++q) {
            const f4 t = *reinterpret_cast<const f4 *>(p + 4 * q);
#pragma unroll
            for (int e = 0; e < 4; ++e) f[4 * q + e] = t[e];
        }
    } else if constexpr (BV == 2) {
        const f2 t = *reinterpret_cast<const f2 *>(p);
        f[0] = t[0];
        f[1] = t[1];
    } else {
        f[0] = *p;
    }
}

template <int BV>
__device__ __forceinline__ void store_f(float *p, const float (&f)[BV]) {
    if constexpr (BV >= 4) {
#pragma unroll
        for (int q = 0; q < BV / 4; ++q) {
            const f4 t = {f[4 * q], f[4 * q + 1], f[4 * q + 2], f[4 * q + 3]};
            *reinterpret_cast<f4 *>(p + 4 * q) = t;
        }
    } else if constexpr (BV == 2) {
        const f2 t = {f[0], f[1]};
        *reinterpret_cast<f2 *>(p) = t;
    } else {
        *p = f[0];
    }
}

template <int BV>
__device__ __forceinline__ void vfma(float (&acc)[BV], float v, const typename RawT<BV>::type &x) {
    float xf[BV];
    widen<BV>(x, xf);
#pragma unroll
    for (int e = 0; e < BV; ++e) acc[e] = __builtin_fmaf(v, xf[e], acc[e]);
}

struct AccEpi {
    float *acc = nullptr;
    int64_t ldacc = 0;
    float acc_w = 1.f, acc_div = 1.f;
    int acc_mode = 0;
};

__device__ __forceinline__ float acc_apply(float a, float y, const AccEpi &e) { return acc_apply(a, y, e.acc_mode, e.acc_w, e.acc_div); }

struct Bf16Args {
    const int32_t *items;
    const sgl::Piece *pieces;
    const int64_t *rowptr;
    const int32_t *col;
    const float *val;
    const uint16_t *x;
    uint16_t *y;
    float *partial;
    int64_t ldx, ldy, ldp;
    int32_t n_items, n_pieces, d;
    BlockMap map;
    AccEpi epi;
    const int32_t *rowmap;
};

template <int BV, int GROUP, int NCH, int U, bool PARTIAL>
__device__ __forceinline__ void run_rows(const int32_t *__restrict__ colb, const float *__restrict__ valb, const int my_rel,
                                         const int nrows, const int tot, const uint16_t *__restrict__ x, const int64_t ldx,
                                         uint16_t *__restrict__ yout, float *__restrict__ pout, const int64_t ldo, const int d,
                                         const int lane, const AccEpi epi, const RowMap rm = RowMap()) {
    using Raw = typename RawT<BV>::type;
    constexpr int R = 64 / GROUP;
    const int s = (R == 1) ? 0 : (lane / GROUP);
    const int l = lane % GROUP;
    int colofs[NCH];
    bool on[NCH];
#pragma unroll
    for (int ch = 0; ch < NCH; ++ch) {
        colofs[ch] = (ch * GROUP + l) * BV;
        on[ch] = colofs[ch] < d;
    }
    int cbr = 0;
    int my_c = 0, nx_c = 0;
    float my_v = 0.f, nx_v = 0.f;
    if (lane < tot) {
        my_c = colb[lane];
        my_v = valb[lane];
    }
    if (64 + lane < tot) {
        nx_c = colb[64 + lane];
        nx_v = valb[64 + lane];
    }

    for (int ri = 0; ri < nrows; ++ri) {
        const int jb = __builtin_amdgcn_readlane(my_rel, ri);
        const int je = __builtin_amdgcn_readlane(my_rel, ri + 1);
        const int64_t ro = rm.on ? (int64_t)__builtin_amdgcn_readlane(rm.my_map, ri) : (int64_t)ri;
        float acc[NCH][BV];
#pragma unroll
        for (int ch = 0; ch < NCH; ++ch)
#pragma unroll
            for (int e = 0; e < BV; ++e) acc[ch][e] = 0.f;
        int j = jb;
        while (j < je) {
            const int lim = min(je, cbr + 64);
            const int o = j - cbr;
            const int cnt = lim - j;
            const int sh = (R == 1) ? 0 : ((s - (j - jb)) & (R - 1));
            int t = 0;
            for (; t + R * U <= cnt; t += R * U) {
                int c[U];
                float v[U];
                Raw xv[U][NCH];
#pragma unroll
                for (int u = 0; u < U; ++u) {
                    const int idx = o + t + u * R + sh;
                    c[u] = bcast_i<R>(my_c, idx);
                    v[u] = bcast_f<R>(my_v, idx);
                }
#pragma unroll
                for (int ch = 0; ch < NCH; ++ch) {
                    if (on[ch]) {
#pragma unroll
                        for (int u = 0; u < U; ++u)
                            xv[u][ch] = *reinterpret_cast<const Raw *>(x + (int64_t)c[u] * ldx + colofs[ch]);
                    } else {
#pragma unroll
                        for (int u = 0; u < U; ++u) xv[u][ch] = rzero<BV>();
                    }
                }
#pragma unroll
                for (int u = 0; u < U; ++u)
#pragma unroll
                    for (int ch = 0; ch < NCH; ++ch) vfma<BV>(acc[ch], v[u], xv[u][ch]);
            }
            if (t < cnt) {
                int c[U];
                float v[U];
                bool valid[U];
                Raw xv[U][NCH];
#pragma unroll
                for (int u = 0; u < U; ++u) {
                    valid[u] = (t + u * R + sh) < cnt;
                    const int idx = (o + t + u * R + sh) & 63;
                    c[u] = bcast_i<R>(my_c, idx);
                    v[u] = bcast_f<R>(my_v, idx);
                }
#pragma unroll
                for (int ch = 0; ch < NCH; ++ch)
#pragma unroll
                    for (int u = 0; u < U; ++u) {
                        xv[u][ch] = rzero<BV>();
                        if (valid[u] && on[ch]) xv[u][ch] = *reinterpret_cast<const Raw *>(x + (int64_t)c[u] * ldx + colofs[ch]);
                    }
#pragma unroll
                for (int u = 0; u < U; ++u)
                    if (valid[u]) {
#pragma unroll
                        for (int ch = 0; ch < NCH; ++ch) vfma<BV>(acc[ch], v[u], xv[u][ch]);
                    }
            }
            j = lim;
            if (lim == cbr + 64) {
                cbr += 64;
                my_c = nx_c;
                my_v = nx_v;
                if (cbr + 64 + lane < tot) {
                    nx_c = colb[cbr + 64 + lane];
                    nx_v = valb[cbr + 64 + lane];
                }
            }
        }
        if constexpr (R > 1) {
#pragma unroll
            for (int off = GROUP; off < 64; off <<= 1)
#pragma unroll
                for (int ch = 0; ch < NCH; ++ch)
#pragma unroll
                    for (int e = 0; e < BV; ++e) acc[ch][e] += __shfl_xor(acc[ch][e], off, 64);
        }
        if (s == 0) {
#pragma unroll
            for (int ch = 0; ch < NCH; ++ch)
                if (on[ch]) {
                    if constexpr (PARTIAL) {
                        store_f<BV>(pout + ro * ldo + colofs[ch], acc[ch]);
                    } else {
                        const Raw r = narrow<BV>(acc[ch]);
                        if (epi.acc) {
                            float yv[BV], a[BV];
                            widen<BV>(r, yv);
                            float *ap = epi.acc + ro * epi.ldacc + colofs[ch];
                            load_f<BV>(ap, a);
#pragma unroll
                            for (int e = 0; e < BV; ++e) a[e] = acc_apply(a[e], yv[e], epi);
                            store_f<BV>(ap, a);
                        }
                        *reinterpret_cast<Raw *>(yout + ro * ldo + colofs[ch]) = r;
                    }
                }
        }
    }
}

template <int BV, int GROUP, int NCH, int U>
__global__ __launch_bounds__(256) void spmm_bf16_kernel(const Bf16Args a) {
    const int lane = threadIdx.x & 63;
    const int wave = __builtin_amdgcn_readfirstlane(threadIdx.x >> 6);
    const int b = blockIdx.x;
    if (b < a.map.piece_blocks) {
        const int p = b * a.map.waves + wave;
        if (p >= a.n_pieces) return;
        const sgl::Piece pc = a.pieces[p];
        const int my_rel = (lane == 0) ? 0 : pc.len;
        const AccEpi none;
        run_rows<BV, GROUP, NCH, U, true>(a.col + pc.begin, a.val + pc.begin, my_rel, 1, pc.len, a.x, a.ldx, nullptr,
                                          a.partial + (int64_t)p * a.ldp, a.ldp, a.d, lane, none);
    } else {
        int ib = b - a.map.piece_blocks;
        if (a.map.xcd_remap) ib = xcd_block(ib, a.map.item_blocks_per_xcd);
        const int item = ib * a.map.waves + wave;
        if (item >= a.n_items) return;
        const int row_begin = a.items[2 * item], row_end = a.items[2 * item + 1];
        const int nrows = row_end - row_begin;
        const ItemWindow w = item_window(a.rowptr, row_begin, nrows, lane);
        const RowMap rm = item_rowmap(a.rowmap, row_begin, nrows, lane);
        const int64_t first = rm.on ? 0 : row_begin;
        AccEpi epi = a.epi;
        if (epi.acc) epi.acc += first * epi.ldacc;
        run_rows<BV, GROUP, NCH, U, false>(a.col + w.base, a.val + w.base, w.my_rel, nrows, w.tot, a.x, a.ldx, a.y + first * a.ldy,
                                           nullptr, a.ldy, a.d, lane, epi, rm);
    }
}

__global__ __launch_bounds__(256) void spmm_bf16_fixup_kernel(const int32_t *__restrict__ long_row,
                                                              const int32_t *__restrict__ long_first,
                                                              const float *__restrict__ partial, int64_t ldp,
                                                              uint16_t *__restrict__ y, int64_t ldy, int d, AccEpi epi) {
    const int kblocks = (d + 255) / 256;
    const int lr = blockIdx.x / kblocks;
    const int k = (blockIdx.x % kblocks) * 256 + threadIdx.x;
    if (k >= d) return;
    const int row = long_row[lr];
    const int p0 = long_first[lr], p1 = long_first[lr + 1];
    float acc = 0.f;
    for (int p = p0; p < p1; ++p) acc += partial[(int64_t)p * ldp + k];
    const uint16_t r = (uint16_t)(pack2(acc, 0.f) & 0xffffu);
    if (epi.acc) {
        float *ap = epi.acc + (int64_t)row * epi.ldacc + k;
        *ap = acc_apply(*ap, __uint_as_float((uint32_t)r << 16), epi);
    }
    y[(int64_t)row * ldy + k] = r;
}

template <int BV, int GROUP, int NCH, int U>
hipError_t launch_variant(const Bf16Args &a, int grid, hipStream_t st) {
    hipLaunchKernelGGL((spmm_bf16_kernel<BV, GROUP, NCH, U>), dim3(grid), dim3(64 * a.map.waves), 0, st, a);
    return hipGetLastError();
}

template <int BV, int GROUP, int NCH>
hipError_t launch_u(const Bf16Args &a, int grid, hipStream_t st, int ulevel) {
    using sgl::unroll_of;
    if (ulevel == 2) return launch_variant<BV, GROUP, NCH, unroll_of(GROUP, NCH, 2)>(a, grid, st);
    return ulevel == 0 ? launch_variant<BV, GROUP, NCH, unroll_of(GROUP, NCH, 0)>(a, grid, st)
                       : launch_variant<BV, GROUP, NCH, unroll_of(GROUP, NCH, 1)>(a, grid, st);
}

template <int BV>
hipError_t launch_group(const Bf16Args &a, int grid, hipStream_t st, int ulevel, int group, int nch) {
    if (nch == 1) {
        switch (group) {
            case 8:
                return launch_u<BV, 8, 1>(a, grid, st, ulevel);
            case 16:
                return launch_u<BV, 16, 1>(a, grid, st, ulevel);
            case 32:
                return launch_u<BV, 32, 1>(a, grid, st, ulevel);
            default:
                return launch_u<BV, 64, 1>(a, grid, st, ulevel);
        }
    }
    if (nch == 2) return launch_u<BV, 64, 2>(a, grid, st, ulevel);
    return launch_u<BV, 64, 4>(a, grid, st, ulevel);
}

int pick_bv(const uint16_t *d_x, int64_t ldx, const uint16_t *d_y, int64_t ldy, int64_t d) {
    for (int bv = 8; bv > 1; bv >>= 1)
        if (d % bv == 0 && ldx % bv == 0 && ldy % bv == 0 && aligned_to(d_x, 2 * bv) && aligned_to(d_y, 2 * bv)) return bv;
    return 1;
}

int spmm_slice(sgl_csr_t *h, const uint16_t *d_x, int64_t ldx, uint16_t *d_y, int64_t ldy, int d, int bv, hipStream_t st,
               const AccEpi &ah, const char *who) {
    SpmmLaunch L;
    int rc = spmm_launch(L, h, d / bv, d, true, who);
    if (rc == SGL_OK) rc = grow_partial(h, L.ldp);
    if (rc != SGL_OK) return rc;
    if (L.grid == 0) return SGL_OK;

    Bf16Args a;
    a.items = h->d_items;
    a.pieces = h->d_pieces;
    a.rowptr = h->d_rowptr;
    a.col = h->d_col;
    a.val = h->d_val;
    a.x = d_x;
    a.y = d_y;
    a.ldx = ldx;
    a.ldy = ldy;
    a.ldp = L.ldp;
    a.n_items = (int32_t)h->n_items;
    a.n_pieces = (int32_t)h->n_pieces;
    a.d = d;
    a.epi = ah;
    a.rowmap = h->d_rowmap;
    a.map = L.map;
    a.partial = h->d_partial;
    hipError_t e;
    if (bv == 8)
        e = launch_group<8>(a, L.grid, st, L.ulevel, L.group, L.nch);
    else if (bv == 4)
        e = launch_group<4>(a, L.grid, st, L.ulevel, L.group, L.nch);
    else if (bv == 2)
        e = launch_group<2>(a, L.grid, st, L.ulevel, L.group, L.nch);
    else
        e = launch_group<1>(a, L.grid, st, L.ulevel, L.group, L.nch);
    if (e != hipSuccess) return sgl::fail((int)e, "%s: kernel launch failed: %s", who, hipGetErrorString(e));
    if (L.fixup_grid > 0) {
        hipLaunchKernelGGL(spmm_bf16_fixup_kernel, dim3((unsigned)L.fixup_grid), dim3(256), 0, st, h->d_rowmap ? h->d_long_out : h->d_long_row,
                           h->d_long_first, h->d_partial, a.ldp, d_y, ldy, d, a.epi);
        e = hipGetLastError();
        if (e != hipSuccess) return sgl::fail((int)e, "%s: fix-up launch failed: %s", who, hipGetErrorString(e));
    }
    return SGL_OK;
}

int spmm_impl(sgl_csr_t *h, const uint16_t *d_x, int64_t ldx, uint16_t *d_y, int64_t ldy, int64_t d, void *stream, AccEpi ah,
              const char *who) {
    if (!h) return sgl::fail(SGL_ERR_INVALID, "%s: NULL handle", who);
    SGL_REQUIRE(d >= 0 && d < INT32_MAX, "%s: bad d", who);
    if (d == 0 || h->n_rows == 0) return SGL_OK;
    SGL_REQUIRE(d_x && d_y, "%s: NULL X or Y", who);
    SGL_REQUIRE(ldx >= d && ldy >= d, "%s: leading dimension smaller than d", who);
    SGL_REQUIRE(aligned_to(d_x, 2) && aligned_to(d_y, 2), "%s: X/Y not 2-byte aligned", who);
    hipStream_t st = sgl::as_stream(stream);
    int bv = pick_bv(d_x, ldx, d_y, ldy, d);
    if (ah.acc) {
        SGL_REQUIRE(ah.ldacc >= d && aligned_to(ah.acc, 4), "%s: bad accumulator matrix", who);
        if (bv >= 4 && !(ah.ldacc % 4 == 0 && aligned_to(ah.acc, 16))) bv = 2;
        if (bv == 2 && !(ah.ldacc % 2 == 0 && aligned_to(ah.acc, 8))) bv = 1;
    }
    const int64_t vcap = sgl::tuning("spmm_vec", 0);
    if ((vcap == 1 || vcap == 2) && vcap < bv) bv = (int)vcap;
    const int64_t max_cols = 64 * 4 * bv;
    for (int64_t c0 = 0; c0 < d; c0 += max_cols) {
        const int dc = (int)std::min<int64_t>(max_cols, d - c0);
        AccEpi as = ah;
        if (as.acc) as.acc += c0;
        int rc = spmm_slice(h, d_x + c0, ldx, d_y + c0, ldy, dc, bv, st, as, who);
        if (rc != SGL_OK) return rc;
    }
    return SGL_OK;
}

constexpr int kGatherMaxHops = 16;
struct GIn {
    const uint16_t *p[kGatherMaxHops];
    int64_t ld[kGatherMaxHops];
};
struct GOut {
    float *p[kGatherMaxHops];
    int64_t ld[kGatherMaxHops];
};

template <int VEC, int U>
__global__ __launch_bounds__(256) void gather_bf16_kernel(const GIn hx, const GOut ho, const int64_t n_rows,
                                                          const int64_t *__restrict__ idx, const int64_t n_idx, const int d,
                                                          const int dw, const int lpr) {
    const int h = blockIdx.y;
    const uint16_t *__restrict__ x = hx.p[h];
    const int64_t ldx = hx.ld[h];
    float *__restrict__ out = ho.p[h];
    const int64_t ldo = ho.ld[h];
    const int rpb = 256 / lpr;
    const int l = threadIdx.x % lpr;
    const int64_t i0 = (int64_t)blockIdx.x * (rpb * U) + threadIdx.x / lpr;
    int64_t src[U];
#pragma unroll
    for (int u = 0; u < U; ++u) {
        const int64_t i = i0 + (int64_t)u * rpb;
        int64_t s = i < n_idx ? idx[i] : 0;
        if (s < 0) s += n_rows;
        if (s < 0 || s >= n_rows) s = -1;
        src[u] = s;
    }
    const float qnan = __uint_as_float(0x7fc00000u);
    for (int c = l * VEC; c < dw; c += lpr * VEC) {
        if constexpr (VEC == 4) {
            f4 v[U];
#pragma unroll
            for (int u = 0; u < U; ++u) {
                v[u] = (f4){0.f, 0.f, 0.f, 0.f};
                if (src[u] < 0) {
#pragma unroll
                    for (int e = 0; e < 4; ++e)
                        if (c + e < d) v[u][e] = qnan;
                } else if (c + 4 <= d) {
                    const u2 r = *reinterpret_cast<const u2 *>(x + src[u] * ldx + c);
                    v[u] = (f4){widen_lo(r[0]), widen_hi(r[0]), widen_lo(r[1]), widen_hi(r[1])};
                } else {
#pragma unroll
                    for (int e = 0; e < 4; ++e)
                        if (c + e < d) v[u][e] = __uint_as_float((uint32_t)x[src[u] * ldx + c + e] << 16);
                }
            }
#pragma unroll
            for (int u = 0; u < U; ++u) {
                const int64_t i = i0 + (int64_t)u * rpb;
                if (i < n_idx) __builtin_nontemporal_store(v[u], reinterpret_cast<f4 *>(out + i * ldo + c));
            }
        } else {
            float v[U];
#pragma unroll
            for (int u = 0; u < U; ++u)
                v[u] = c >= d ? 0.f : (src[u] < 0 ? qnan : __uint_as_float((uint32_t)x[src[u] * ldx + c] << 16));
#pragma unroll
            for (int u = 0; u < U; ++u) {
                const int64_t i = i0 + (int64_t)u * rpb;
                if (i < n_idx) __builtin_nontemporal_store(v[u], out + i * ldo + c);
            }
        }
    }
}

int gather_impl(const char *who, int n_hops, const uint16_t *const *h_x, const int64_t *h_ldx, int64_t n_rows, const int64_t *d_idx,
                int64_t n_idx, float *const *h_out, const int64_t *h_ldo, int64_t d, int64_t pad, void *stream) {
    SGL_REQUIRE(n_idx >= 0 && d >= 0 && pad >= 0 && n_rows >= 0 && d + pad < INT32_MAX, "%s: bad sizes", who);
    SGL_REQUIRE(n_hops >= 1 && h_x && h_ldx && h_out && h_ldo, "%s: NULL hop arrays or n_hops < 1", who);
    if (n_hops > kGatherMaxHops)
        return sgl::fail(SGL_ERR_UNSUPPORTED, "%s: at most %d hop matrices per launch (gather hop by hop)", who, kGatherMaxHops);
    const int64_t dw = d + pad;
    GIn hx;
    GOut ho;
    bool vec4 = dw % 4 == 0;
    for (int h = 0; h < n_hops; ++h) {
        hx.p[h] = h_x[h];
        hx.ld[h] = h_ldx[h];
        ho.p[h] = h_out[h];
        ho.ld[h] = h_ldo[h];
        SGL_REQUIRE(n_idx == 0 || d == 0 || (hx.p[h] && ho.p[h]), "%s: hop %d: NULL matrix", who, h);
        SGL_REQUIRE(hx.ld[h] >= d && aligned_to(hx.p[h], 2), "%s: hop %d: source pitch < d or pointer not 2-byte aligned", who, h);
        SGL_REQUIRE(ho.ld[h] >= dw && aligned_to(ho.p[h], 4), "%s: output %d: pitch < d + pad_cols or pointer not 4-byte aligned", who, h);
        vec4 = vec4 && hx.ld[h] % 4 == 0 && aligned_to(hx.p[h], 8) && ho.ld[h] % 4 == 0 && aligned_to(ho.p[h], 16);
    }
    for (int h = n_hops; h < kGatherMaxHops; ++h) {
        hx.p[h] = nullptr;
        ho.p[h] = nullptr;
        hx.ld[h] = ho.ld[h] = 0;
    }
    if (n_idx == 0 || dw == 0) return SGL_OK;
    SGL_REQUIRE(d_idx != nullptr, "%s: NULL indices", who);
    SGL_REQUIRE(n_rows > 0, "%s: indices into a matrix without rows", who);
    const int vec = vec4 ? 4 : 1;
    int lpr = 8;
    while (lpr < 64 && (int64_t)lpr * vec < dw) lpr <<= 1;
    constexpr int U = 4;
    const int64_t blocks = (n_idx + (256 / lpr) * U - 1) / ((256 / lpr) * U);
    if (!sgl::launch_fits(blocks * n_hops, 256)) return sgl::fail(SGL_ERR_UNSUPPORTED, "%s: too many indices for one launch", who);
    hipStream_t st = sgl::as_stream(stream);
    if (vec4)
        hipLaunchKernelGGL((gather_bf16_kernel<4, U>), dim3((unsigned)blocks, (unsigned)n_hops), dim3(256), 0, st, hx, ho, n_rows, d_idx,
                           n_idx, (int)d, (int)dw, lpr);
    else
        hipLaunchKernelGGL((gather_bf16_kernel<1, U>), dim3((unsigned)blocks, (unsigned)n_hops), dim3(256), 0, st, hx, ho, n_rows, d_idx,
                           n_idx, (int)d, (int)dw, lpr);
    const hipError_t e = hipGetLastError();
    if (e != hipSuccess) return sgl::fail((int)e, "%s: kernel launch failed: %s", who, hipGetErrorString(e));
    return SGL_OK;
}

}

SGL_EXPORT int sgl_spmm_bf16(sgl_csr_t *h, const uint16_t *d_x, int64_t ldx, uint16_t *d_y, int64_t ldy, int64_t d, void *stream) {
    return spmm_impl(h, d_x, ldx, d_y, ldy, d, stream, AccEpi(), "sgl_spmm_bf16");
}

SGL_EXPORT int sgl_spmm_chain_bf16(sgl_csr_t *h, int n_hops, const uint16_t *d_x0, int64_t ldx0, uint16_t *const *h_y,
                                   const int64_t *h_ldy, int64_t d, void *stream) {
    if (!h) return sgl::fail(SGL_ERR_INVALID, "sgl_spmm_chain_bf16: NULL handle");
    SGL_REQUIRE(n_hops >= 0 && (n_hops == 0 || (h_y && h_ldy)), "sgl_spmm_chain_bf16: bad hop arrays");
    SGL_REQUIRE(n_hops == 0 || h->n_rows == h->n_cols, "sgl_spmm_chain_bf16: repeated products need a square matrix");
    const uint16_t *cur = d_x0;
    int64_t ldc = ldx0;
    for (int k = 0; k < n_hops; ++k) {
        int rc = spmm_impl(h, cur, ldc, h_y[k], h_ldy[k], d, stream, AccEpi(), "sgl_spmm_chain_bf16");
        if (rc != SGL_OK) return rc;
        cur = h_y[k];
        ldc = h_ldy[k];
    }
    return SGL_OK;
}

SGL_EXPORT int sgl_spmm_acc_bf16(sgl_csr_t *h, const uint16_t *d_x, int64_t ldx, uint16_t *d_y, int64_t ldy, int64_t d, float *d_acc,
                                 int64_t ldacc, float w, int mode, float divisor, void *stream) {
    AccEpi ah;
    const int rc = acc_mode_of("sgl_spmm_acc_bf16", d_acc, mode, divisor, ah.acc_mode);
    if (rc != SGL_OK) return rc;
    ah.acc = d_acc;
    ah.ldacc = ldacc;
    ah.acc_w = w;
    ah.acc_div = divisor;
    return spmm_impl(h, d_x, ldx, d_y, ldy, d, stream, ah, "sgl_spmm_acc_bf16");
}

SGL_EXPORT int sgl_gather_rows_bf16_f32(const uint16_t *d_x, int64_t ldx, int64_t n_rows, const int64_t *d_idx, int64_t n_idx,
                                        float *d_out, int64_t ldo, int64_t d, int64_t pad_cols, void *stream) {
    const uint16_t *xs[1] = {d_x};
    float *os[1] = {d_out};
    return gather_impl("sgl_gather_rows_bf16_f32", 1, xs, &ldx, n_rows, d_idx, n_idx, os, &ldo, d, pad_cols, stream);
}

SGL_EXPORT int sgl_gather_hops_bf16_f32(int n_hops, const uint16_t *const *h_x, const int64_t *h_ldx, int64_t n_rows,
                                        const int64_t *d_idx, int64_t n_idx, float *const *h_out, const int64_t *h_ldo, int64_t d,
                                        int64_t pad_cols, void *stream) {
    return gather_impl("sgl_gather_hops_bf16_f32", n_hops, h_x, h_ldx, n_rows, d_idx, n_idx, h_out, h_ldo, d, pad_cols, stream);
}
```

sgl_amd/csrc/sgl_spmm_common.h:

```cpp
#pragma once
#include "sgl_csr.h"

namespace {

template <int R>
__device__ __forceinline__ int bcast_i(int v, int idx) {
    if constexpr (R == 1)
        return __builtin_amdgcn_readlane(v, idx);
    else
        return __builtin_amdgcn_ds_bpermute(idx << 2, v);
}
template <int R>
__device__ __forceinline__ float bcast_f(float v, int idx) {
    return __int_as_float(bcast_i<R>(__float_as_int(v), idx));
}

__device__ __forceinline__ float acc_apply(float a, float y, int mode, float w, float div) {
    if ((mode & 3) == 3)
        return (mode & 8) ? ((y < a || y != y) ? y : a) : ((y > a || y != y) ? y : a);
    a = ((mode & 3) == 2) ? __fadd_rn(a, __fmul_rn(y, w)) : __fadd_rn(a, y);
    if (mode & 4) a = __fdiv_rn(a, div);
    return a;
}

struct RowMap {
    int my_map = 0;
    bool on = false;
};

struct BlockMap {
    int32_t piece_blocks, item_blocks_per_xcd, xcd_remap, waves;
};
__device__ __forceinline__ int xcd_block(int ib, int item_blocks_per_xcd) { return (ib & 7) * item_blocks_per_xcd + (ib >> 3); }

struct ItemWindow {
    int64_t base;
    int my_rel, tot;
};

__device__ __forceinline__ ItemWindow item_window(const int64_t *rowptr, int row_begin, int nrows, int lane) {
    ItemWindow w;
    const int64_t rp = rowptr[(int64_t)row_begin + min(lane, nrows)];
    const int lo = __builtin_amdgcn_readfirstlane((int)(uint32_t)rp);
    const int hi = __builtin_amdgcn_readfirstlane((int)(uint32_t)((uint64_t)rp >> 32));
    w.base = (int64_t)(((uint64_t)(uint32_t)hi << 32) | (uint32_t)lo);
    w.my_rel = (int)(rp - w.base);
    w.tot = __builtin_amdgcn_readlane(w.my_rel, nrows);
    return w;
}

__device__ __forceinline__ RowMap item_rowmap(const int32_t *rowmap, int row_begin, int nrows, int lane) {
    RowMap rm;
    rm.on = rowmap != nullptr;
    rm.my_map = rm.on ? rowmap[(int64_t)row_begin + max(min(lane, nrows - 1), 0)] : 0;
    return rm;
}

struct SpmmLaunch : sgl::SpmmLayout {
    BlockMap map;
    int64_t ldp;
    int grid, fixup_grid;
};

int spmm_launch(SpmmLaunch &L, const sgl_csr_t *h, int lanes, int d, bool bf16, const char *who) {
    static_cast<sgl::SpmmLayout &>(L) = sgl::spmm_layout(lanes, (h->flags & SGL_CSR_STRICT_ORDER) != 0, h->nnz, h->n_rows, bf16);
    L.ldp = bf16 ? (d + 7) / 8 * 8 : (d + 3) / 4 * 4;
    L.map.waves = L.waves;
    L.map.piece_blocks = (int32_t)((h->n_pieces + L.waves - 1) / L.waves);
    const int64_t item_blocks = (h->n_items + L.waves - 1) / L.waves;
    L.map.xcd_remap = (!(h->flags & SGL_CSR_NO_XCD_REMAP) && sgl::tuning("spmm_xcd_remap", 1) != 0) ? 1 : 0;
    L.map.item_blocks_per_xcd = (int32_t)((item_blocks + 7) / 8);
    const int64_t grid64 = L.map.piece_blocks + (L.map.xcd_remap ? (int64_t)L.map.item_blocks_per_xcd * 8 : item_blocks);
    if (grid64 >= INT32_MAX) return sgl::fail(SGL_ERR_UNSUPPORTED, "%s: grid too large", who);
    const int64_t fg = (int64_t)((d + 255) / 256) * h->n_long;
    if (fg >= INT32_MAX) return sgl::fail(SGL_ERR_UNSUPPORTED, "%s: fix-up grid too large", who);
    L.grid = (int)grid64;
    L.fixup_grid = (int)fg;
    return SGL_OK;
}

int grow_partial(sgl_csr_t *h, int64_t ldp) {
    const size_t need = (size_t)h->n_pieces * (size_t)ldp;
    if (need > h->partial_cap) {
        if (h->d_partial) h->retired.push_back(h->d_partial);
        h->d_partial = nullptr;
        h->partial_cap = 0;
        SGL_HIP_CHECK(hipMalloc((void **)&h->d_partial, need * sizeof(float)));
        h->partial_cap = need;
    }
    return SGL_OK;
}

int acc_mode_of(const char *who, const float *d_acc, int mode, float divisor, int &acc_mode) {
    SGL_REQUIRE(d_acc != nullptr, "%s: NULL accumulator", who);
    SGL_REQUIRE(!(divisor == 0.f), "%s: zero divisor", who);
    SGL_REQUIRE(mode >= SGL_ACC_SUM && mode <= SGL_ACC_MIN, "%s: unknown mode %d", who, mode);
    SGL_REQUIRE(mode < SGL_ACC_MAX || divisor == 1.f, "%s: max / min take no divisor", who);
    acc_mode = mode >= SGL_ACC_MAX ? (3 | (mode == SGL_ACC_MIN ? 8 : 0)) : ((mode == SGL_ACC_WSUM ? 2 : 1) | (divisor != 1.f ? 4 : 0));
    return SGL_OK;
}

}
```

sgl_amd/device.py:

```python
import ctypes
import os
from ctypes import c_int64, c_void_p

import numpy as np
import torch
import torch.nn.functional as F

from . import _lib
from ._lib import check, current_stream_ptr, lib, ptr

__all__ = [
    "DeviceCSR", "default_long_row_nnz", "ChainGraph", "round_up", "row_pitch", "expected_lines", "alloc_rows", "upload_rows", "normalize_adj",
    "normalize_block", "degree_powers", "PreparedAdjacency", "PreparedBlock",
    "placed_empty", "MEM_MODES",
    "hop_reduce", "hop_concat", "hop_reduce_grad", "hop_concat_grad", "hop_lincomb", "hop_wsum1d", "hop_wsum2d", "hop_scores", "hop_scores2", "hop_gate", "gate_fusable", "nafs_aggregate", "nafs_prefix",
    "gather_rows", "edge_dot",
]


def round_up(x, m):
    return (x + m - 1) // m * m


HOP_DTYPES = {"float32": torch.float32, "bfloat16": torch.bfloat16}


def hop_torch_dtype(dtype):
    if isinstance(dtype, str):
        if dtype.strip().lower() not in HOP_DTYPES:
            raise ValueError(f"hop_dtype must be one of {sorted(HOP_DTYPES)}, not {dtype!r}")
        return HOP_DTYPES[dtype.strip().lower()]
    if dtype not in HOP_DTYPES.values():
        raise ValueError(f"hop matrices are stored as float32 or bfloat16, not {dtype}")
    return dtype


def _esize(dtype):
    return 2 if dtype == torch.bfloat16 else 4


def expected_lines(ld, d, elem_size=4):
    import math
    step = math.gcd(ld * elem_size, 128)
    offs = range(0, 128, step)
    return sum((o + d * elem_size + 127) // 128 for o in offs) / len(offs)


def row_pitch(d, growth=1.25, elem_size=4):
    d = max(int(d), 1)
    if elem_size not in (2, 4):
        raise ValueError("row_pitch: elem_size must be 4 (float32) or 2 (bfloat16)")
    vec, line = 16 // elem_size, 128 // elem_size
    ld4, ld32 = round_up(d, vec), round_up(d, line)
    cands = [(ld32, growth)]
    if d < line:
        p2 = vec
        while p2 < d:
            p2 *= 2
        cands.insert(0, (p2, max(growth, 1.34)))
    best, best_lines = ld4, expected_lines(ld4, d, elem_size)
    for ld, cap in cands:
        if ld != ld4 and ld <= cap * ld4 and expected_lines(ld, d, elem_size) <= 0.97 * best_lines:
            best, best_lines = ld, expected_lines(ld, d, elem_size)
    return best


def alloc_rows(n, d, device, zero_pad=True, dtype=torch.float32):
    ld = row_pitch(d, elem_size=_esize(dtype))
    buf = torch.empty((n, ld), dtype=dtype, device=device)
    if zero_pad and ld != d:
        buf[:, d:].zero_()
    return buf[:, :d] if ld != d else buf


def own_pad(t):
    n, d = t.shape
    if n <= 1:
        return 0
    ld = t.stride(0)
    return ld - d if (ld > d and (ld * t.element_size()) % 16 == 0 and t.stride(1) == 1 and t.data_ptr() % 16 == 0) else 0


def padded_parent(t):
    n, d = t.shape
    ld = t.stride(0) if n > 1 else row_pitch(d, elem_size=t.element_size())
    if ld == d:
        return t
    return torch.as_strided(t, (n, ld), (ld, 1), t.storage_offset())


MEM_MODES = {"default": _lib.SGL_MEM_DEFAULT, "contiguous": _lib.SGL_MEM_CONTIGUOUS, "vmm": _lib.SGL_MEM_VMM}


class _PlacedBlock:

    def __init__(self, n_floats, mode, chunk_bytes, device):
        self.device = torch.device(device)
        self.n = int(n_floats)
        p = c_void_p()
        with torch.cuda.device(self.device):
            _lib.check_probe(_lib.probe_lib().sgl_mem_alloc(ctypes.byref(p), self.n * 4, MEM_MODES[mode], int(chunk_bytes)), f"sgl_mem_alloc({mode})")
        self.ptr = p.value
        self.__cuda_array_interface__ = {"shape": (self.n,), "typestr": "<f4", "data": (self.ptr, False), "version": 2}

    def __del__(self):
        p, self.ptr = getattr(self, "ptr", None), None
        if p:
            try:
                with torch.cuda.device(self.device):
                    _lib.probe_lib().sgl_mem_free(c_void_p(p))
            except Exception:
                pass


def placed_empty(shape, device, mode="contiguous", chunk_bytes=0):
    n = 1
    for s_ in shape:
        n *= int(s_)
    blk = _PlacedBlock(max(n, 1), mode, chunk_bytes, device)
    flat = torch.as_tensor(blk, device=blk.device)
    return flat[:n].view(*shape)


_STAGED_MIN_BYTES = 8 << 20


def upload_rows(x, device):
    if isinstance(x, np.ndarray):
        x = torch.from_numpy(np.ascontiguousarray(x, dtype=np.float32))
    x = x.detach()
    n, d = x.shape
    out = alloc_rows(n, d, device)
    out.copy_(x.to(dtype=torch.float32), non_blocking=False)
    return out


def permute_rows(rowptr, col, val, perm):
    n = rowptr.numel() - 1
    perm = perm.to(torch.int32).contiguous()
    out_ptr = torch.empty(n + 1, dtype=torch.int64, device=rowptr.device)
    out_col = torch.empty_like(col)
    out_val = torch.empty_like(val)
    with torch.cuda.device(rowptr.device):
        check(lib().sgl_csr_permute_rows(ptr(rowptr), ptr(col), ptr(val), n, ptr(perm), ptr(out_ptr), ptr(out_col), ptr(out_val),
                                         current_stream_ptr()), "sgl_csr_permute_rows")
    return out_ptr, out_col, out_val


def download_rows(t):
    src = t if t.is_contiguous() else t.contiguous()
    host = torch.empty(src.shape, dtype=torch.float32)
    if src.numel() * 4 < _STAGED_MIN_BYTES:
        host.copy_(src)
        return host
    with torch.cuda.device(src.device):
        check(lib().sgl_download(host.data_ptr(), ptr(src), src.numel() * 4, current_stream_ptr()), "sgl_download")
    return host


def _wrote(*tensors):
    for t in tensors:
        if torch.is_tensor(t):
            torch.autograd.graph.increment_version(t)


def _check_mat(t, name, bf16=False):
    if not (isinstance(t, torch.Tensor) and t.is_cuda and t.dim() == 2 and (t.dtype == torch.float32 or (bf16 and t.dtype == torch.bfloat16))):
        raise TypeError(f"{name} must be a 2-D float32{' or bfloat16' if bf16 else ''} CUDA tensor")
    if t.shape[1] > 1 and t.stride(1) != 1:
        raise ValueError(f"{name} must be row-major (column stride 1)")
    if t.shape[0] > 1 and t.stride(0) < t.shape[1]:
        raise ValueError(f"{name}: row stride smaller than the row length")


def _ld(t):
    return t.stride(0) if t.shape[0] > 1 else max(t.shape[1], 1)


def _same_hop_dtype(who, *tensors):
    dts = {t.dtype for t in tensors}
    if len(dts) != 1:
        raise TypeError(f"{who}: x and out must have the same dtype (float32 or bfloat16), got {sorted(str(d_) for d_ in dts)}")
    return dts.pop()


def _no_bf16(who, *tensors):
    if any(torch.is_tensor(t) and t.dtype == torch.bfloat16 for t in tensors):
        raise TypeError(f"{who} has no bfloat16 form (bf16 hop storage covers spmm, spmm_chain, spmm_acc, the row gathers and the "
                        "reduce / concat / NAFS aggregators)")


def widen_hops(feats):
    out = []
    for f in feats:
        if torch.is_tensor(f) and f.is_cuda and f.dtype == torch.bfloat16 and f.dim() == 2:
            w = alloc_rows(f.shape[0], f.shape[1], f.device)
            w.copy_(f)
            f = w
        out.append(f)
    return out


def default_long_row_nnz(nnz):
    nnz = int(nnz)
    return 32 if nnz < (1 << 18) else 128 if nnz < (1 << 20) else 512 if nnz < (1 << 22) else 2048


class DeviceCSR:

    def __init__(self, rowptr, col, val, shape, strict=False, item_nnz=0, long_row_nnz=0, xcd_remap=True):
        _lib.require_gpu()
        for t, dt, nm in ((rowptr, torch.int64, "rowptr"), (col, torch.int32, "col"), (val, torch.float32, "val")):
            if not (t.is_cuda and t.dtype == dt and t.dim() == 1 and t.is_contiguous()):
                raise TypeError(f"{nm} must be a contiguous 1-D CUDA tensor of dtype {dt}")
        self.rowptr, self.col, self.val = rowptr, col, val
        self.shape = (int(shape[0]), int(shape[1]))
        self.nnz = int(col.numel())
        self.device = rowptr.device
        self.strict = bool(strict)
        flags = (_lib.SGL_CSR_STRICT_ORDER if strict else 0) | (0 if xcd_remap else _lib.SGL_CSR_NO_XCD_REMAP)
        h = c_void_p()
        with torch.cuda.device(self.device):
            check(lib().sgl_csr_create(ctypes.byref(h), self.shape[0], self.shape[1], self.nnz, ptr(rowptr), ptr(col),
                                       ptr(val), flags, int(item_nnz), int(long_row_nnz), current_stream_ptr()),
                  "sgl_csr_create")
        self._h = h

    @classmethod
    def from_scipy(cls, adj, device="cuda", **kw):
        import scipy.sparse as sp
        if not sp.isspmatrix_csr(adj):
            raise TypeError("expected a scipy.sparse.csr_matrix")
        rowptr = torch.from_numpy(adj.indptr.astype(np.int64)).to(device)
        col = torch.from_numpy(adj.indices.astype(np.int32)).to(device)
        val = torch.from_numpy(adj.data.astype(np.float32)).to(device)
        return cls(rowptr, col, val, adj.shape, **kw)

    def set_values(self, val):
        if not (val.is_cuda and val.dtype == torch.float32 and val.dim() == 1 and val.is_contiguous() and val.numel() == self.nnz):
            raise TypeError("val must be a contiguous float32 CUDA tensor with one entry per non-zero")
        check(lib().sgl_csr_set_values(self._h, ptr(val)), "sgl_csr_set_values")
        self.val = val
        return self

    rowmap = None

    def set_rowmap(self, rowmap):
        if rowmap is not None and not (rowmap.is_cuda and rowmap.dtype == torch.int32 and rowmap.dim() == 1
                                       and rowmap.is_contiguous() and rowmap.numel() == self.shape[0]):
            raise TypeError("rowmap must be a contiguous int32 CUDA tensor with one entry per row")
        with torch.cuda.device(self.device):
            check(lib().sgl_csr_set_rowmap(self._h, ptr(rowmap) if rowmap is not None else None, current_stream_ptr()),
                  "sgl_csr_set_rowmap")
        self.rowmap = rowmap
        return self

    def info(self):
        a = (c_int64 * 8)()
        check(lib().sgl_csr_info(self._h, a), "sgl_csr_info")
        keys = ("n_rows", "n_cols", "nnz", "n_items", "n_pieces", "n_long_rows", "flags", "workspace_bytes")
        return dict(zip(keys, list(a)))

    def spmm(self, x, out=None, accumulate=False):
        _check_mat(x, "x", bf16=True)
        if x.shape[0] != self.shape[1]:
            raise ValueError("Dimension mismatch detected for the adjacency and the feature matrix!")
        d = x.shape[1]
        if out is None:
            if accumulate:
                raise ValueError("accumulate=True needs an `out` tensor")
            out = alloc_rows(self.shape[0], d, x.device, zero_pad=True, dtype=x.dtype)
        else:
            _check_mat(out, "out", bf16=True)
            if out.shape != (self.shape[0], d):
                raise ValueError("out has the wrong shape")
        if _same_hop_dtype("spmm", x, out) == torch.bfloat16:
            if accumulate:
                raise ValueError("spmm: bfloat16 hops have no accumulate form")
            with torch.cuda.device(self.device):
                check(lib().sgl_spmm_bf16(self._h, ptr(x), _ld(x), ptr(out), _ld(out), d, current_stream_ptr()), "sgl_spmm_bf16")
            _wrote(out)
            return out
        with torch.cuda.device(self.device):
            check(lib().sgl_spmm_f32(self._h, ptr(x), _ld(x), ptr(out), _ld(out), d, int(bool(accumulate)),
                                     current_stream_ptr()), "sgl_spmm_f32")
        _wrote(out)
        return out

    ACC_MODES = {"sum": 0, "wsum": 1, "max": 2, "min": 3}

    def spmm_acc(self, x, out, acc, w=1.0, weighted=False, divisor=1.0, mode=None):
        mode = self.ACC_MODES[mode] if mode is not None else int(bool(weighted))
        _check_mat(x, "x", bf16=True)
        _check_mat(out, "out", bf16=True)
        _check_mat(acc, "acc")
        if x.shape[0] != self.shape[1] or out.shape != (self.shape[0], x.shape[1]) or acc.shape != out.shape:
            raise ValueError("Dimension mismatch detected for the adjacency and the feature matrix!")
        fn, name = ((lib().sgl_spmm_acc_bf16, "sgl_spmm_acc_bf16") if _same_hop_dtype("spmm_acc", x, out) == torch.bfloat16
                    else (lib().sgl_spmm_acc_f32, "sgl_spmm_acc_f32"))
        with torch.cuda.device(self.device):
            check(fn(self._h, ptr(x), _ld(x), ptr(out), _ld(out), x.shape[1], ptr(acc), _ld(acc),
                                         float(w), mode, float(divisor), current_stream_ptr()), name)
        _wrote(out, acc)
        return out

    def spmm_multi(self, x, out_ptrs, ld, row_mask=None):
        _no_bf16("spmm_multi", x)
        _check_mat(x, "x")
        if x.shape[0] != self.shape[1]:
            raise ValueError("Dimension mismatch detected for the adjacency and the feature matrix!")
        n_out = len(out_ptrs)
        if not 1 <= n_out <= 8:
            raise ValueError("between 1 and 8 output replicas are supported")
        arr = (c_void_p * n_out)(*[int(p) for p in out_ptrs])
        with torch.cuda.device(self.device):
            if row_mask is not None and not (row_mask.is_cuda and row_mask.dtype == torch.uint8 and row_mask.is_contiguous()
                                             and row_mask.numel() == self.shape[0]):
                raise ValueError("row_mask must be a contiguous uint8 CUDA tensor with one entry per row")
            check(lib().sgl_spmm_multi_f32(self._h, ptr(x), _ld(x), n_out, arr, int(ld), x.shape[1],
                                           ptr(row_mask) if row_mask is not None else None, current_stream_ptr()),
                  "sgl_spmm_multi_f32")

    def spmm_chain(self, x, n_hops, outs=None):
        _check_mat(x, "x", bf16=True)
        if x.shape[0] != self.shape[1] or self.shape[0] != self.shape[1]:
            raise ValueError("Dimension mismatch detected for the adjacency and the feature matrix!")
        d = x.shape[1]
        if outs is None:
            outs = [alloc_rows(self.shape[0], d, x.device, zero_pad=True, dtype=x.dtype) for _ in range(n_hops)]
        else:
            if len(outs) != n_hops:
                raise ValueError("need one output matrix per hop")
            for o in outs:
                _check_mat(o, "outs[*]", bf16=True)
                if o.shape != (self.shape[0], d):
                    raise ValueError("an output matrix has the wrong shape")
        if n_hops:
            bf16 = _same_hop_dtype("spmm_chain", x, *outs) == torch.bfloat16
            fn, name = (lib().sgl_spmm_chain_bf16, "sgl_spmm_chain_bf16") if bf16 else (lib().sgl_spmm_chain_f32, "sgl_spmm_chain_f32")
            ptrs = (c_void_p * n_hops)(*[o.data_ptr() for o in outs])
            lds = (c_int64 * n_hops)(*[_ld(o) for o in outs])
            with torch.cuda.device(self.device):
                check(fn(self._h, n_hops, ptr(x), _ld(x), ptrs, lds, d, current_stream_ptr()), name)
            _wrote(*outs)
        return outs

    def capture_chain(self, x, outs):
        _no_bf16("capture_chain", x, *outs)
        _check_mat(x, "x")
        for o in outs:
            _check_mat(o, "outs[*]")
            if o.shape != (self.shape[0], x.shape[1]):
                raise ValueError("an output matrix has the wrong shape")
        n_hops = len(outs)
        ptrs = (c_void_p * n_hops)(*[o.data_ptr() for o in outs])
        lds = (c_int64 * n_hops)(*[_ld(o) for o in outs])
        g = c_void_p()
        torch.cuda.synchronize(self.device)
        with torch.cuda.device(self.device):
            check(lib().sgl_chain_graph_create(ctypes.byref(g), self._h, n_hops, ptr(x), _ld(x), ptrs, lds, x.shape[1]),
                  "sgl_chain_graph_create")
        return ChainGraph(g, self, x, list(outs))

    def spmm_axpb_clamp(self, x, alpha, res=None, lo=float("-inf"), hi=float("inf"), out=None):
        _no_bf16("spmm_axpb_clamp", x, res, out)
        _check_mat(x, "x")
        if x.shape[0] != self.shape[1]:
            raise ValueError("Dimension mismatch detected for the adjacency and the feature matrix!")
        d = x.shape[1]
        if out is None:
            out = alloc_rows(self.shape[0], d, x.device, zero_pad=True)
        else:
            _check_mat(out, "out")
        if res is not None:
            _check_mat(res, "res")
            if res.shape != (self.shape[0], d):
                raise ValueError("res has the wrong shape")
        with torch.cuda.device(self.device):
            check(lib().sgl_spmm_axpb_clamp_f32(self._h, ptr(x), _ld(x), ptr(out), _ld(out), d, float(alpha),
                                                ptr(res) if res is not None else None, _ld(res) if res is not None else 0,
                                                float(lo), float(hi), current_stream_ptr()), "sgl_spmm_axpb_clamp_f32")
        _wrote(out)
        return out

    def close(self):
        h, self._h = getattr(self, "_h", None), None
        if h:
            lib().sgl_csr_destroy(h)

    def __del__(self):
        try:
            self.close()
        except Exception:
            pass


class ChainGraph:

    def __init__(self, handle, csr, x, outs):
        self._g, self.csr, self.x, self.outs = handle, csr, x, outs

    def replay(self):
        with torch.cuda.device(self.csr.device):
            check(lib().sgl_chain_graph_launch(self._g, current_stream_ptr()), "sgl_chain_graph_launch")
        _wrote(*self.outs)
        return self.outs

    def close(self):
        g, self._g = getattr(self, "_g", None), None
        if g:
            lib().sgl_chain_graph_destroy(g)

    def __del__(self):
        try:
            self.close()
        except Exception:
            pass


_POW_CACHE = []
_POW_THREADS = max(1, min(64, (os.cpu_count() or 2) // 2))
pow_stats = {"cache_hits": 0, "host_unique": 0, "host_full": 0, "device": 0}


def _host_powers(d, r):
    left, right = np.empty_like(d), np.empty_like(d)

    def run(a, b):
        with np.errstate(divide="ignore", invalid="ignore"):
            np.power(d[a:b], r - 1, out=left[a:b])
            left[a:b][np.isinf(left[a:b])] = 0.
            np.power(d[a:b], -r, out=right[a:b])
            right[a:b][np.isinf(right[a:b])] = 0.
    n = d.shape[0]
    chunk = 1 << 20
    if n <= 2 * chunk or _POW_THREADS == 1:
        run(0, n)
    else:
        from concurrent.futures import ThreadPoolExecutor
        with ThreadPoolExecutor(_POW_THREADS) as ex:
            list(ex.map(lambda a: run(a, min(a + chunk, n)), range(0, n, chunk)))
    return left, right


def _few_distinct(deg, sample=4096):
    n = deg.numel()
    if n <= 4 * sample:
        return True
    s = deg[:: n // sample][:sample]
    return torch.unique(s).numel() * 2 <= s.numel()


def degree_powers(deg, r, host_pow=True):
    r = float(r)
    for ent in _POW_CACHE:
        if ent[0] is deg and ent[1] == deg._version and ent[2] == r and ent[3] == host_pow:
            pow_stats["cache_hits"] += 1
            return ent[4], ent[5]
    asked = host_pow
    few = None
    if host_pow == "auto":
        few = (not deg.is_cuda) or deg.numel() <= 4096 or _few_distinct(deg)
        host_pow = few
    if deg.is_cuda and not host_pow:
        left, right = torch.empty_like(deg), torch.empty_like(deg)
        with torch.cuda.device(deg.device):
            check(lib().sgl_norm_degree_powers(deg.numel(), ptr(deg), r, ptr(left), ptr(right), current_stream_ptr()),
                  "sgl_norm_degree_powers")
        pow_stats["device"] += 1
    elif deg.is_cuda and deg.numel() > 4096 and (few if few is not None else _few_distinct(deg)):
        uniq, inv = torch.unique(deg, return_inverse=True)
        lu, ru = _host_powers(uniq.cpu().numpy(), r)
        left, right = torch.from_numpy(lu).to(deg.device)[inv], torch.from_numpy(ru).to(deg.device)[inv]
        pow_stats["host_unique"] += 1
    elif deg.is_cuda:
        from . import hostpool
        n = deg.numel()
        bufs = [hostpool.take((n,), torch.float64) if n >= (1 << 20) else None for _ in range(3)]
        h = bufs[0] if bufs[0] is not None else torch.empty(n, dtype=torch.float64)
        h.copy_(deg)
        hl, hr = _host_powers(h.numpy(), r)
        outs = []
        for src, buf in ((hl, bufs[1]), (hr, bufs[2])):
            t = torch.from_numpy(src)
            if buf is not None:
                buf.copy_(t)
                t = buf
            outs.append(t.to(deg.device, non_blocking=buf is not None))
        torch.cuda.current_stream(deg.device).synchronize()
        left, right = outs
        pow_stats["host_full"] += 1
    else:
        hl, hr = _host_powers(deg.detach().numpy().astype(np.float64, copy=False), r)
        left, right = torch.from_numpy(hl), torch.from_numpy(hr)
    _POW_CACHE[:] = [(deg, deg._version, r, asked, left, right)]
    return left, right


def clear_power_cache():
    _POW_CACHE.clear()


def _all_positive(val, deg=None):
    flags = [t.min() > 0 for t in (val, deg) if t is not None and t.numel()]
    return bool(torch.stack(flags).all().item()) if flags else True


def _drop_exact_zeros(rowptr, col, val32, val64):
    keep = val64 != 0
    if bool(keep.all().item()):
        return rowptr, col, val32, val64
    before = torch.zeros(keep.numel() + 1, dtype=torch.int64, device=keep.device)
    before[1:] = torch.cumsum(keep, 0)
    return before[rowptr], col[keep], val32[keep], val64[keep]


def _reference_pattern(prune, return_fp64, rowptr, col, values):
    if prune:
        rowptr, col, v32, v64 = _drop_exact_zeros(rowptr, col, *values)
        values = (v32, v64) if return_fp64 else (v32,)
    return (rowptr, col) + values


class PreparedAdjacency:

    def __init__(self, rowptr, col, val, n):
        _lib.require_gpu()
        dev = rowptr.device
        nnz = int(col.numel())
        self.n, self.src = int(n), (rowptr, col, val)
        nnz_out = c_int64(0)
        with torch.cuda.device(dev):
            check(lib().sgl_norm_block_prepare(n, 0, nnz, ptr(rowptr), ptr(col), ctypes.byref(nnz_out), current_stream_ptr()),
                  "sgl_norm_block_prepare")
            m = nnz_out.value
            self.rowptr = torch.empty(n + 1, dtype=torch.int64, device=dev)
            self.col = torch.empty(m, dtype=torch.int32, device=dev)
            self.t64 = torch.empty(m, dtype=torch.float64, device=dev)
            self.deg = torch.empty(n, dtype=torch.float64, device=dev)
            fp = torch.zeros(1, dtype=torch.int64, device=dev)
            check(lib().sgl_norm_build_symcheck(n, nnz, ptr(rowptr), ptr(col), ptr(val), m, ptr(self.rowptr), ptr(self.col),
                                                ptr(self.t64), ptr(self.deg), ptr(fp), current_stream_ptr()),
                  "sgl_norm_build_symcheck")
            ok = val.min() > 0 if nnz else torch.ones((), dtype=torch.bool, device=dev)
            asym, ok = torch.stack([fp[0] != 0, ok]).tolist()
            self.symmetric, self.may_hold_zero = not asym, not ok
        self.nnz_out = m
        self.device = dev
        if self.symmetric:
            self.src = None

    def nbytes(self):
        seen, total = set(), 0
        objs = [self] + ([self.__dict__["_tblock"]] if self.__dict__.get("_tblock") is not None else [])
        for o in objs:
            for name, v in o.__dict__.items():
                if name == "src":
                    continue
                if isinstance(v, tuple) and len(v) == 2 and torch.is_tensor(v[1]):
                    v = v[1]
                if torch.is_tensor(v) and v.is_cuda and v.data_ptr() not in seen:
                    seen.add(v.data_ptr())
                    total += v.numel() * v.element_size()
        return total
# ... 981 lines not shown
```

Measured before the change: 1447 billion.

## Add locality-aware finer item lists for SpMM to improve L2 reuse

At CSR creation a sampling kernel measures how often column ids fall near their row, within several window sizes. When enough neighbours are local and the feature table is large relative to the 4 MB L2 per XCD, extra work-item lists with smaller item_nnz (256/128/64) are built. At launch one is chosen from L2 capacity, row bytes and occupancy so that rows in flight on an XCD fit in cache. The cost is an extra sampling kernel and a host sync at create time, plus memory for the additional item lists.

```diff
diff --git a/include/sgl_hip.h b/include/sgl_hip.h
--- a/include/sgl_hip.h
+++ b/include/sgl_hip.h
@@ -29,6 +29,11 @@
                     int32_t *h_piece_row, int32_t *h_long_row, int32_t *h_long_first);
 void sgl_plan_destroy(sgl_plan_t *plan);
 
+int sgl_locality_host(const int64_t *h_rowptr, const int32_t *h_col, int64_t n_rows, const int32_t *h_rowmap, int64_t n_sample,
+                      int64_t counts[8]);
+int sgl_local_list_rule(const int64_t counts[8], int64_t n_rows, int64_t n_cols, int64_t nnz, int64_t row_bytes, int waves_per_cu,
+                        const int32_t *list_nnz, int n_lists, int *applied);
+
 typedef struct sgl_csr sgl_csr_t;
 
 #define SGL_CSR_STRICT_ORDER 0x1u
@@ -40,6 +45,7 @@
 int sgl_csr_destroy(sgl_csr_t *csr);
 int sgl_csr_set_values(sgl_csr_t *csr, const float *d_val);
 int sgl_csr_info(const sgl_csr_t *csr, int64_t info[8]);
+int sgl_csr_locality(const sgl_csr_t *csr, int64_t out[8]);
 
 int sgl_spmm_f32(sgl_csr_t *csr, const float *d_x, int64_t ldx, float *d_y, int64_t ldy, int64_t d,
                  int accumulate, void *stream);
diff --git a/sgl_amd/_lib.py b/sgl_amd/_lib.py
--- a/sgl_amd/_lib.py
+++ b/sgl_amd/_lib.py
@@ -31,6 +31,9 @@
     "sgl_csr_destroy": (c_int, [c_void_p]),
     "sgl_csr_set_values": (c_int, [c_void_p, c_void_p]),
     "sgl_csr_info": (c_int, [c_void_p, POINTER(c_int64)]),
+    "sgl_csr_locality": (c_int, [c_void_p, POINTER(c_int64)]),
+    "sgl_locality_host": (c_int, [c_void_p, c_void_p, c_int64, c_void_p, c_int64, POINTER(c_int64)]),
+    "sgl_local_list_rule": (c_int, [POINTER(c_int64), c_int64, c_int64, c_int64, c_int64, c_int, c_void_p, c_int, POINTER(c_int)]),
     "sgl_spmm_f32": (c_int, [c_void_p, c_void_p, c_int64, c_void_p, c_int64, c_int64, c_int, c_void_p]),
     "sgl_spmm_multi_f32": (c_int, [c_void_p, c_void_p, c_int64, c_int, c_void_p, c_int64, c_int64, c_void_p, c_void_p]),
     "sgl_spmm_chain_f32": (c_int, [c_void_p, c_int, c_void_p, c_int64, c_void_p, c_void_p, c_int64, c_void_p]),
diff --git a/sgl_amd/csrc/sgl_common.h b/sgl_amd/csrc/sgl_common.h
--- a/sgl_amd/csrc/sgl_common.h
+++ b/sgl_amd/csrc/sgl_common.h
@@ -68,6 +68,37 @@
 int32_t default_item_nnz(int64_t nnz);
 int32_t default_long_row_nnz(int64_t nnz);
 
+constexpr int kLocalityWindows = 5;
+constexpr int64_t kLocalityWindow[kLocalityWindows] = {1024, 2048, 4096, 8192, 16384};
+constexpr int64_t kLocalitySample = 65536;
+constexpr int32_t kLocalItemNnz[3] = {256, 128, 64};
+
+#if defined(__HIPCC__)
+#define SGL_HD __host__ __device__
+#else
+#define SGL_HD
+#endif
+SGL_HD inline uint32_t locality_mix(uint32_t v) {
+    v ^= v >> 16;
+    v *= 0x7feb352du;
+    v ^= v >> 15;
+    v *= 0x846ca68bu;
+    v ^= v >> 16;
+    return v;
+}
+SGL_HD inline int64_t locality_sample_row(int64_t s, int64_t n_rows, int64_t n_sample) {
+    if (n_rows <= n_sample) return s;
+    const int64_t lo = s * n_rows / n_sample;
+    return lo + (int64_t)(locality_mix((uint32_t)s + 0x9e3779b9u) % (uint64_t)(n_rows / n_sample));
+}
+int locality_host(const int64_t *rowptr, const int32_t *col, int64_t n_rows, const int32_t *rowmap, int64_t n_sample,
+                  int64_t counts[1 + kLocalityWindows]);
+
+int pick_local_list(const int64_t counts[1 + kLocalityWindows], int64_t n_rows, int64_t n_cols, int64_t nnz, int64_t row_bytes,
+                    int waves_per_cu, const int32_t *list_nnz, int n_lists, bool *applied);
+bool wants_local_lists(const int64_t counts[1 + kLocalityWindows]);
+int build_items(std::vector<int32_t> &items, const int64_t *rowptr, int64_t n_rows, int32_t item_nnz, int32_t long_row_nnz);
+
 struct SpmmLayout {
     int group, nch, ulevel, waves;
     bool nt;
diff --git a/sgl_amd/csrc/sgl_core.cpp b/sgl_amd/csrc/sgl_core.cpp
--- a/sgl_amd/csrc/sgl_core.cpp
+++ b/sgl_amd/csrc/sgl_core.cpp
@@ -30,6 +30,10 @@
         {"spmm_waves", 0},
         {"spmm_xcd_remap", 1},
         {"spmm_heavy_first", 1},
+        {"spmm_local", 0},
+        {"spmm_local_f_pct", 50},
+        {"spmm_local_min_share_pct", 50},
+        {"spmm_local_table_x", 8},
         {"agg_blocks", 0},
         {"nafs_fused", 1},
         {"row_lpr32x2", 1},
@@ -222,7 +226,7 @@
 
 constexpr int64_t kPlanSegmentRows = (int64_t)1 << 20;
 
-int build_plan(Plan &plan, const int64_t *rowptr, int64_t n_rows, int32_t item_nnz, int32_t long_row_nnz) {
+static int build_plan_ordered(Plan &plan, const int64_t *rowptr, int64_t n_rows, int32_t item_nnz, int32_t long_row_nnz, bool heavy_first) {
     if (n_rows < 0 || (n_rows > 0 && rowptr == nullptr)) return fail(SGL_ERR_INVALID, "build_plan: bad arguments");
     if (n_rows >= (int64_t)INT32_MAX) return fail(SGL_ERR_UNSUPPORTED, "build_plan: n_rows >= 2^31 (shard the matrix)");
     if (item_nnz <= 0) item_nnz = kDefaultItemNnz;
@@ -272,8 +276,84 @@
             sg = Plan();
         }
     }
-    if (tuning("spmm_heavy_first", 1) != 0) heavy_items_first(plan, rowptr, item_nnz);
-    return SGL_OK;
+    if (heavy_first) heavy_items_first(plan, rowptr, item_nnz);
+    return SGL_OK;
+}
+
+int build_plan(Plan &plan, const int64_t *rowptr, int64_t n_rows, int32_t item_nnz, int32_t long_row_nnz) {
+    return build_plan_ordered(plan, rowptr, n_rows, item_nnz, long_row_nnz, tuning("spmm_heavy_first", 1) != 0);
+}
+
+int build_items(std::vector<int32_t> &items, const int64_t *rowptr, int64_t n_rows, int32_t item_nnz, int32_t long_row_nnz) {
+    Plan plan;
+    const int rc = build_plan_ordered(plan, rowptr, n_rows, item_nnz, long_row_nnz, false);
+    if (rc == SGL_OK) items.swap(plan.items);
+    return rc;
+}
+
+int locality_host(const int64_t *rowptr, const int32_t *col, int64_t n_rows, const int32_t *rowmap, int64_t n_sample,
+                  int64_t counts[1 + kLocalityWindows]) {
+    for (int w = 0; w <= kLocalityWindows; ++w) counts[w] = 0;
+    if (n_rows < 0 || (n_rows > 0 && !rowptr) || n_sample <= 0) return fail(SGL_ERR_INVALID, "locality: bad arguments");
+    if (n_rows > 0 && rowptr[n_rows] > rowptr[0] && !col) return fail(SGL_ERR_INVALID, "locality: NULL column ids");
+    std::vector<int32_t> inv;
+    if (rowmap) {
+        inv.assign((size_t)n_rows, -1);
+        for (int64_t i = 0; i < n_rows; ++i) {
+            if (rowmap[i] < 0 || rowmap[i] >= n_rows) return fail(SGL_ERR_INVALID, "locality: map entry outside [0, n_rows)");
+            inv[(size_t)rowmap[i]] = (int32_t)i;
+        }
+    }
+    const int64_t ns = std::min(n_rows, n_sample);
+    for (int64_t s = 0; s < ns; ++s) {
+        const int64_t i = locality_sample_row(s, n_rows, n_sample);
+        for (int64_t p = rowptr[i]; p < rowptr[i + 1]; ++p) {
+            const int64_t c = col[p];
+            ++counts[0];
+            int64_t pos = c;
+            if (rowmap) {
+                if (c < 0 || c >= n_rows || inv[(size_t)c] < 0) continue;
+                pos = inv[(size_t)c];
+            }
+            const int64_t dist = pos > i ? pos - i : i - pos;
+            for (int w = 0; w < kLocalityWindows; ++w)
+                if (dist < kLocalityWindow[w]) ++counts[1 + w];
+        }
+    }
+    return SGL_OK;
+}
+
+constexpr int64_t kL2Bytes = (int64_t)4 << 20;
+constexpr int64_t kCusPerXcd = 32;
+
+bool wants_local_lists(const int64_t counts[1 + kLocalityWindows]) {
+    const int64_t mode = tuning("spmm_local", 0);
+    if (mode == 1) return true;
+    if (mode == 2 || counts[0] <= 0) return false;
+    return counts[kLocalityWindows] * 100 >= counts[0] * tuning("spmm_local_min_share_pct", 50);
+}
+
+int pick_local_list(const int64_t counts[1 + kLocalityWindows], int64_t n_rows, int64_t n_cols, int64_t nnz, int64_t row_bytes,
+                    int waves_per_cu, const int32_t *list_nnz, int n_lists, bool *applied) {
+    const int64_t mode = tuning("spmm_local", 0);
+    if (applied) *applied = false;
+    if (mode == 2 || n_lists <= 0 || n_rows <= 0 || row_bytes <= 0 || waves_per_cu <= 0) return 0;
+    const int64_t f = std::max<int64_t>(1, std::min<int64_t>(100, tuning("spmm_local_f_pct", 50)));
+    const int64_t rows_in_flight = kL2Bytes * f / 100 / row_bytes;
+    if (mode != 1) {
+        if (n_cols * row_bytes < tuning("spmm_local_table_x", 8) * kL2Bytes) return 0;
+        int w = -1;
+        for (int k = 0; k < kLocalityWindows; ++k)
+            if (kLocalityWindow[k] <= rows_in_flight) w = k;
+        if (w < 0 || counts[0] <= 0) return 0;
+        if (counts[1 + w] * 100 < counts[0] * tuning("spmm_local_min_share_pct", 50)) return 0;
+    }
+    if (applied) *applied = true;
+    const int64_t rows_per_item = rows_in_flight / (kCusPerXcd * waves_per_cu);
+    const int64_t want_nnz = rows_per_item * nnz / n_rows;
+    for (int k = 0; k < n_lists; ++k)
+        if (list_nnz[k] <= want_nnz) return k;
+    return n_lists - 1;
 }
 
 }
@@ -357,3 +437,19 @@
 }
 
 SGL_EXPORT void sgl_plan_destroy(sgl_plan_t *plan) { delete plan; }
+
+SGL_EXPORT int sgl_locality_host(const int64_t *h_rowptr, const int32_t *h_col, int64_t n_rows, const int32_t *h_rowmap,
+                                 int64_t n_sample, int64_t counts[8]) {
+    if (!counts) return sgl::fail(SGL_ERR_INVALID, "sgl_locality_host: NULL counts");
+    memset(counts, 0, 8 * sizeof(int64_t));
+    return sgl::locality_host(h_rowptr, h_col, n_rows, h_rowmap, n_sample > 0 ? n_sample : sgl::kLocalitySample, counts);
+}
+
+SGL_EXPORT int sgl_local_list_rule(const int64_t counts[8], int64_t n_rows, int64_t n_cols, int64_t nnz, int64_t row_bytes,
+                                   int waves_per_cu, const int32_t *list_nnz, int n_lists, int *applied) {
+    if (!counts || (n_lists > 0 && !list_nnz)) return -1;
+    bool on = false;
+    const int k = sgl::pick_local_list(counts, n_rows, n_cols, nnz, row_bytes, waves_per_cu, list_nnz, n_lists, &on);
+    if (applied) *applied = on ? 1 : 0;
+    return k;
+}
diff --git a/sgl_amd/csrc/sgl_csr.h b/sgl_amd/csrc/sgl_csr.h
--- a/sgl_amd/csrc/sgl_csr.h
+++ b/sgl_amd/csrc/sgl_csr.h
@@ -22,4 +22,15 @@
     const int32_t *d_rowmap = nullptr;
     int32_t *d_long_out = nullptr;
     std::shared_ptr<std::atomic<uint64_t>> epoch = std::make_shared<std::atomic<uint64_t>>(0);
+    struct ItemList {
+        int32_t item_nnz = 0;
+        int64_t n_items = 0;
+        int32_t *d_items = nullptr;
+    };
+    int32_t item_nnz = 0, long_row_nnz = 0;
+    int64_t loc_plain[1 + sgl::kLocalityWindows] = {0, 0, 0, 0, 0, 0}, loc_mapped[1 + sgl::kLocalityWindows] = {0, 0, 0, 0, 0, 0};
+    std::vector<ItemList> lists;
+    unsigned long long *d_loc = nullptr;
+    int32_t last_local = 0, last_item_nnz = 0;
+    const int64_t *loc_counts() const { return d_rowmap ? loc_mapped : loc_plain; }
 };
diff --git a/sgl_amd/csrc/sgl_csr.hip b/sgl_amd/csrc/sgl_csr.hip
--- a/sgl_amd/csrc/sgl_csr.hip
+++ b/sgl_amd/csrc/sgl_csr.hip
@@ -11,6 +11,88 @@
     }
     const unsigned bit = 1u << (m & 31);
     if (atomicOr(&seen[m >> 5], bit) & bit) atomicOr(bad, 2);
+}
+
+__global__ __launch_bounds__(256) void rowmap_invert_kernel(const int32_t *__restrict__ map, const int64_t n, int32_t *__restrict__ inv) {
+    const int64_t i = (int64_t)blockIdx.x * blockDim.x + threadIdx.x;
+    if (i >= n) return;
+    const int32_t m = map[i];
+    if (m >= 0 && m < n) inv[m] = (int32_t)i;
+}
+
+constexpr int kLocalityBlocks = 1024;
+__global__ __launch_bounds__(256) void locality_kernel(const int64_t *__restrict__ rowptr, const int32_t *__restrict__ col, const int64_t n_rows,
+                                                       const int64_t nnz, const int32_t *__restrict__ inv, const int64_t n_sample,
+                                                       unsigned long long *__restrict__ counts) {
+    const int lane = threadIdx.x & 63;
+    const int64_t wave = ((int64_t)blockIdx.x * blockDim.x + threadIdx.x) >> 6;
+    const int64_t n_waves = ((int64_t)gridDim.x * blockDim.x) >> 6;
+    const int64_t ns = n_rows < n_sample ? n_rows : n_sample;
+    unsigned long long tot = 0;
+    unsigned cnt[sgl::kLocalityWindows];
+#pragma unroll
+    for (int w = 0; w < sgl::kLocalityWindows; ++w) cnt[w] = 0;
+    for (int64_t s = wave; s < ns; s += n_waves) {
+        const int64_t i = sgl::locality_sample_row(s, n_rows, n_sample);
+        const int64_t b = min(max(rowptr[i], (int64_t)0), nnz), e = min(max(rowptr[i + 1], b), nnz);
+        tot += (unsigned long long)(e - b);
+        for (int64_t p = b + lane; p < e; p += 64) {
+            const int64_t c = col[p];
+            int64_t pos = c;
+            bool ok = true;
+            if (inv) {
+                ok = c >= 0 && c < n_rows;
+                pos = ok ? (int64_t)inv[c] : 0;
+                ok = ok && pos >= 0;
+            }
+            const int64_t dist = pos > i ? pos - i : i - pos;
+#pragma unroll
+            for (int w = 0; w < sgl::kLocalityWindows; ++w) cnt[w] += (ok && dist < ((int64_t)1024 << w)) ? 1u : 0u;
+        }
+    }
+#pragma unroll
+    for (int w = 0; w < sgl::kLocalityWindows; ++w)
+        for (int off = 32; off > 0; off >>= 1) cnt[w] += __shfl_xor(cnt[w], off, 64);
+    if (lane == 0) {
+        if (tot) atomicAdd(&counts[0], tot);
+#pragma unroll
+        for (int w = 0; w < sgl::kLocalityWindows; ++w)
+            if (cnt[w]) atomicAdd(&counts[1 + w], (unsigned long long)cnt[w]);
+    }
+}
+static_assert(sgl::kLocalityWindow[0] == 1024 && sgl::kLocalityWindow[sgl::kLocalityWindows - 1] == ((int64_t)1024 << (sgl::kLocalityWindows - 1)),
+              "locality_kernel counts the windows 1024 << w");
+
+static int queue_locality(sgl_csr_t *h, const int32_t *d_inv, unsigned long long *host, hipStream_t st) {
+    constexpr size_t bytes = (1 + sgl::kLocalityWindows) * sizeof(unsigned long long);
+    if (!h->d_loc) SGL_HIP_CHECK(hipMalloc((void **)&h->d_loc, bytes));
+    SGL_HIP_CHECK(hipMemsetAsync(h->d_loc, 0, bytes, st));
+    if (h->n_rows > 0 && h->nnz > 0) {
+        const int64_t ns = std::min<int64_t>(h->n_rows, sgl::kLocalitySample);
+        const unsigned grid = (unsigned)std::min<int64_t>(kLocalityBlocks, (ns + 3) / 4);
+        hipLaunchKernelGGL(locality_kernel, dim3(grid), dim3(256), 0, st, h->d_rowptr, h->d_col, h->n_rows, h->nnz, d_inv, sgl::kLocalitySample, h->d_loc);
+        SGL_HIP_CHECK(hipGetLastError());
+    }
+    SGL_HIP_CHECK(hipMemcpyAsync(host, h->d_loc, bytes, hipMemcpyDeviceToHost, st));
+    return SGL_OK;
+}
+
+static int build_local_lists(sgl_csr_t *h, const int64_t *h_rowptr, const int64_t *counts, std::vector<std::vector<int32_t>> &keep, hipStream_t st) {
+    if (h->lists.size() > 1 || h->n_items == 0 || !sgl::wants_local_lists(counts)) return SGL_OK;
+    for (const int32_t inz : sgl::kLocalItemNnz) {
+        if (inz >= h->item_nnz) continue;
+        keep.emplace_back();
+        int rc = sgl::build_items(keep.back(), h_rowptr, h->n_rows, inz, h->long_row_nnz);
+        if (rc != SGL_OK) return rc;
+        sgl_csr::ItemList l;
+        l.item_nnz = inz;
+        l.n_items = (int64_t)keep.back().size() / 2;
+        if (l.n_items >= (int64_t)INT32_MAX / 2) break;
+        SGL_HIP_CHECK(hipMalloc((void **)&l.d_items, keep.back().size() * sizeof(int32_t)));
+        h->lists.push_back(l);
+        SGL_HIP_CHECK(hipMemcpyAsync(l.d_items, keep.back().data(), keep.back().size() * sizeof(int32_t), hipMemcpyHostToDevice, st));
+    }
+    return SGL_OK;
 }
 
 static int fetch_rowptr(std::vector<int64_t> &h, const int64_t *d, hipStream_t st) {
@@ -79,10 +161,6 @@
     if (item_nnz <= 0) item_nnz = sgl::default_item_nnz(nnz);
     if (long_row_nnz == 0) long_row_nnz = sgl::default_long_row_nnz(nnz);
     if (flags & SGL_CSR_STRICT_ORDER) long_row_nnz = -1;
-    sgl::Plan plan;
-    int rc = sgl::build_plan(plan, h_rowptr.data(), n_rows, item_nnz, long_row_nnz);
-    if (rc != SGL_OK) return rc;
-
     sgl_csr_t *h = new (std::nothrow) sgl_csr_t();
     if (!h) return sgl::fail(SGL_ERR_ALLOC, "sgl_csr_create: out of memory");
     h->n_rows = n_rows;
@@ -92,6 +170,21 @@
     h->d_col = d_col;
     h->d_val = d_val;
     h->flags = flags;
+    h->item_nnz = item_nnz;
+    h->long_row_nnz = long_row_nnz;
+    unsigned long long loc[1 + sgl::kLocalityWindows] = {0, 0, 0, 0, 0, 0};
+    int rc = queue_locality(h, nullptr, loc, st);
+    sgl::Plan plan;
+    if (rc == SGL_OK) rc = sgl::build_plan(plan, h_rowptr.data(), n_rows, item_nnz, long_row_nnz);
+    if (rc == SGL_OK) {
+        hipError_t e = hipStreamSynchronize(st);
+        if (e != hipSuccess) rc = sgl::fail((int)e, "sgl_csr_create: sync failed: %s", hipGetErrorString(e));
+    }
+    if (rc != SGL_OK) {
+        sgl_csr_destroy(h);
+        return rc;
+    }
+    for (int w = 0; w <= sgl::kLocalityWindows; ++w) h->loc_plain[w] = (int64_t)loc[w];
     h->n_items = (int64_t)plan.items.size() / 2;
     h->n_pieces = (int64_t)plan.pieces.size();
     h->n_long = (int64_t)plan.long_row.size();
@@ -107,6 +200,13 @@
     if (rc == SGL_OK) rc = upload((void **)&h->d_long_row, plan.long_row.data(), plan.long_row.size() * sizeof(int32_t));
     if (rc == SGL_OK && h->n_long > 0)
         rc = upload((void **)&h->d_long_first, plan.long_first.data(), plan.long_first.size() * sizeof(int32_t));
+    sgl_csr::ItemList own;
+    own.item_nnz = item_nnz;
+    own.n_items = h->n_items;
+    own.d_items = h->d_items;
+    h->lists.push_back(own);
+    std::vector<std::vector<int32_t>> local_items;
+    if (rc == SGL_OK) rc = build_local_lists(h, h_rowptr.data(), h->loc_plain, local_items, st);
     if (rc == SGL_OK) {
         hipError_t e = hipStreamSynchronize(st);
         if (e != hipSuccess) rc = sgl::fail((int)e, "sgl_csr_create: sync failed: %s", hipGetErrorString(e));
@@ -123,6 +223,8 @@
     if (!h) return SGL_OK;
     h->epoch->store(~0ull);
     (void)hipFree(h->d_items);
+    for (size_t k = 1; k < h->lists.size(); ++k) (void)hipFree(h->lists[k].d_items);
+    (void)hipFree(h->d_loc);
     (void)hipFree(h->d_pieces);
     (void)hipFree(h->d_long_row);
     (void)hipFree(h->d_long_first);
@@ -170,6 +272,34 @@
         SGL_HIP_CHECK(hipMemcpyAsync(h->d_long_out, rows.data(), rows.size() * sizeof(int32_t), hipMemcpyHostToDevice, st));
         SGL_HIP_CHECK(hipStreamSynchronize(st));
     }
+    if (h->n_rows == h->n_cols && h->nnz > 0) {
+        int32_t *d_inv = nullptr;
+        SGL_HIP_CHECK(hipMalloc((void **)&d_inv, (size_t)h->n_rows * sizeof(int32_t)));
+        unsigned long long loc[1 + sgl::kLocalityWindows] = {0, 0, 0, 0, 0, 0};
+        hipError_t e = hipMemsetAsync(d_inv, 0xff, (size_t)h->n_rows * sizeof(int32_t), st);
+        int rc = SGL_OK;
+        if (e == hipSuccess) {
+            hipLaunchKernelGGL(rowmap_invert_kernel, dim3((unsigned)((h->n_rows + 255) / 256)), dim3(256), 0, st, d_rowmap, h->n_rows, d_inv);
+            e = hipGetLastError();
+        }
+        if (e == hipSuccess) rc = queue_locality(h, d_inv, loc, st);
+        if (e == hipSuccess) e = hipStreamSynchronize(st);
+        (void)hipFree(d_inv);
+        if (e != hipSuccess) return sgl::fail((int)e, "sgl_csr_set_rowmap: locality pass failed: %s", hipGetErrorString(e));
+        if (rc != SGL_OK) return rc;
+        for (int w = 0; w <= sgl::kLocalityWindows; ++w) h->loc_mapped[w] = (int64_t)loc[w];
+        if (h->lists.size() <= 1 && h->n_items > 0 && sgl::wants_local_lists(h->loc_mapped)) {
+            std::vector<int64_t> h_rowptr((size_t)h->n_rows + 1);
+            rc = fetch_rowptr(h_rowptr, h->d_rowptr, st);
+            std::vector<std::vector<int32_t>> local_items;
+            if (rc == SGL_OK) rc = build_local_lists(h, h_rowptr.data(), h->loc_mapped, local_items, st);
+            e = hipStreamSynchronize(st);
+            if (rc != SGL_OK) return rc;
+            if (e != hipSuccess) return sgl::fail((int)e, "sgl_csr_set_rowmap: sync failed: %s", hipGetErrorString(e));
+        }
+    } else {
+        for (int w = 0; w <= sgl::kLocalityWindows; ++w) h->loc_mapped[w] = 0;
+    }
     h->d_rowmap = d_rowmap;
     return SGL_OK;
 }
@@ -179,6 +309,15 @@
     SGL_REQUIRE(h->nnz == 0 || d_val, "sgl_csr_set_values: NULL values");
     if (d_val != h->d_val) h->epoch->fetch_add(1);
     h->d_val = d_val;
+    return SGL_OK;
+}
+
+SGL_EXPORT int sgl_csr_locality(const sgl_csr_t *h, int64_t out[8]) {
+    if (!h || !out) return sgl::fail(SGL_ERR_INVALID, "sgl_csr_locality: NULL");
+    const int64_t *c = h->loc_counts();
+    for (int w = 0; w <= sgl::kLocalityWindows; ++w) out[w] = c[w];
+    out[6] = h->last_local;
+    out[7] = h->last_item_nnz;
     return SGL_OK;
 }
 
diff --git a/sgl_amd/csrc/sgl_spmm.hip b/sgl_amd/csrc/sgl_spmm.hip
--- a/sgl_amd/csrc/sgl_spmm.hip
+++ b/sgl_amd/csrc/sgl_spmm.hip
@@ -115,7 +115,7 @@
     return t < e.lo ? e.lo : (t > e.hi ? e.hi : t);
 }
 
-template <int VEC, int GROUP, int NCH, int U, bool NT, bool MULTI>
+template <int VEC, int GROUP, int NCH, int U, bool NT, bool MULTI, bool TAIL_BATCH = false>
 __device__ __forceinline__ void run_rows(const int32_t *__restrict__ colb, const float *__restrict__ valb,
                                          const int my_rel, const int nrows, const int tot,
                                          const float *__restrict__ x, const int64_t ldx, float *__restrict__ out,
@@ -190,6 +190,35 @@
                 for (int u = 0; u < U; ++u)
 #pragma unroll
                     for (int ch = 0; ch < NCH; ++ch) vfma<VEC>(acc[ch], v[u], xv[u][ch]);
+            }
+            if constexpr (TAIL_BATCH) {
+                constexpr int UB = U > 8 ? 8 : U;
+                for (; t < cnt; t += R * UB) {
+                    int c[UB];
+                    float v[UB];
+                    V xv[UB][NCH];
+#pragma unroll
+                    for (int u = 0; u < UB; ++u) {
+                        const int idx = (o + t + u * R + sh) & 63;
+                        c[u] = bcast_i<R>(my_c, idx);
+                        v[u] = bcast_f<R>(my_v, idx);
+                    }
+#pragma unroll
+                    for (int u = 0; u < UB; ++u) {
+                        const bool valid = (t + u * R + sh) < cnt;
+#pragma unroll
+                        for (int ch = 0; ch < NCH; ++ch)
+                            xv[u][ch] = (valid && on[ch]) ? *reinterpret_cast<const V *>(x + (int64_t)c[u] * ldx + colofs[ch]) : vzero<VEC>();
+                    }
+#pragma unroll
+                    for (int u = 0; u < UB; ++u) {
+                        if ((t + u * R + sh) < cnt) {
+#pragma unroll
+                            for (int ch = 0; ch < NCH; ++ch)
+                                if (on[ch]) vfma<VEC>(acc[ch], v[u], xv[u][ch]);
+                        }
+                    }
+                }
             }
             for (; t < cnt; t += R) {
                 const int idx = (o + t + sh) & 63;
@@ -262,8 +291,8 @@
     }
 }
 
-template <int VEC, int GROUP, int NCH, int U, bool NT, bool MULTI>
-__global__ __launch_bounds__(256) void spmm_kernel(const SpmmArgs a) {
+template <int VEC, int GROUP, int NCH, int U, bool NT, bool MULTI, bool TAIL_BATCH>
+__device__ __forceinline__ void spmm_body(const SpmmArgs a) {
     const int lane = threadIdx.x & 63;
     const int wave = __builtin_amdgcn_readfirstlane(threadIdx.x >> 6);
     const int b = blockIdx.x;
@@ -304,10 +333,19 @@
         mo.mask = (MULTI && a.row_mask) ? a.row_mask + row_begin : nullptr;
 #pragma unroll
         for (int q = 0; q < 7; ++q) mo.p[q] = (MULTI && q < a.n_more) ? a.y_more[q] + (int64_t)row_begin * a.ldy : nullptr;
-        run_rows<VEC, GROUP, NCH, U, NT, MULTI>(a.col + w.base, a.val + w.base, w.my_rel, nrows, w.tot, a.x, a.ldx,
-                                         a.y + first * a.ldy, a.ldy, a.d, a.accumulate != 0, lane, epi,
-                                         a.ldres, mo, rm);
-    }
+        run_rows<VEC, GROUP, NCH, U, NT, MULTI, TAIL_BATCH>(a.col + w.base, a.val + w.base, w.my_rel, nrows, w.tot, a.x, a.ldx,
+                                                            a.y + first * a.ldy, a.ldy, a.d, a.accumulate != 0, lane, epi, a.ldres, mo, rm);
+    }
+}
+
+template <int VEC, int GROUP, int NCH, int U, bool NT, bool MULTI>
+__global__ __launch_bounds__(256) void spmm_kernel(const SpmmArgs a) {
+    spmm_body<VEC, GROUP, NCH, U, NT, MULTI, false>(a);
+}
+
+template <int VEC, int GROUP, int NCH, int U, bool NT>
+__global__ __launch_bounds__(256) void spmm_local_kernel(const SpmmArgs a) {
+    spmm_body<VEC, GROUP, NCH, U, NT, false, true>(a);
 }
 
 __global__ __launch_bounds__(256) void spmm_fixup_kernel(const int32_t *__restrict__ long_row,
@@ -337,9 +375,20 @@
         if (q < mo.n && ((need >> q) & 1)) mo.p[q][(int64_t)row * ldy + k] = acc;
 }
 
+struct How {
+    int *occ;
+    bool local;
+};
 template <int VEC, int GROUP, int NCH, int U, bool NT>
-hipError_t launch_variant(const SpmmArgs &a, int grid, hipStream_t st) {
-    if (a.n_more > 0)
+hipError_t launch_variant(const SpmmArgs &a, int grid, hipStream_t st, const How how) {
+    if (how.occ) {
+        *how.occ = a.n_more > 0 ? resident_waves_per_cu(spmm_kernel<VEC, GROUP, NCH, U, NT, true>, a.map.waves)
+                            : resident_waves_per_cu(spmm_local_kernel<VEC, GROUP, NCH, U, NT>, a.map.waves);
+        return hipSuccess;
+    }
+    if (how.local && a.n_more == 0)
+        hipLaunchKernelGGL((spmm_local_kernel<VEC, GROUP, NCH, U, NT>), dim3(grid), dim3(64 * a.map.waves), 0, st, a);
+    else if (a.n_more > 0)
         hipLaunchKernelGGL((spmm_kernel<VEC, GROUP, NCH, U, NT, true>), dim3(grid), dim3(64 * a.map.waves), 0, st, a);
     else
         hipLaunchKernelGGL((spmm_kernel<VEC, GROUP, NCH, U, NT, false>), dim3(grid), dim3(64 * a.map.waves), 0, st, a);
@@ -347,36 +396,42 @@
 }
 
 template <int VEC, int GROUP, int NCH, int U>
-hipError_t launch_nt(const SpmmArgs &a, int grid, hipStream_t st, bool nt) {
-    return nt ? launch_variant<VEC, GROUP, NCH, U, true>(a, grid, st)
-              : launch_variant<VEC, GROUP, NCH, U, false>(a, grid, st);
+hipError_t launch_nt(const SpmmArgs &a, int grid, hipStream_t st, bool nt, const How how) {
+    return nt ? launch_variant<VEC, GROUP, NCH, U, true>(a, grid, st, how)
+              : launch_variant<VEC, GROUP, NCH, U, false>(a, grid, st, how);
 }
 
 template <int VEC, int GROUP, int NCH>
-hipError_t launch_u(const SpmmArgs &a, int grid, hipStream_t st, bool nt, int ulevel) {
+hipError_t launch_u(const SpmmArgs &a, int grid, hipStream_t st, bool nt, int ulevel, const How how) {
     using sgl::unroll_of;
-    if (ulevel == 2) return launch_nt<VEC, GROUP, NCH, unroll_of(GROUP, NCH, 2)>(a, grid, st, nt);
-    if (ulevel == 3) return launch_nt<VEC, GROUP, NCH, unroll_of(GROUP, NCH, 3)>(a, grid, st, nt);
-    return ulevel == 0 ? launch_nt<VEC, GROUP, NCH, unroll_of(GROUP, NCH, 0)>(a, grid, st, nt)
-                       : launch_nt<VEC, GROUP, NCH, unroll_of(GROUP, NCH, 1)>(a, grid, st, nt);
+    if (ulevel == 2) return launch_nt<VEC, GROUP, NCH, unroll_of(GROUP, NCH, 2)>(a, grid, st, nt, how);
+    if (ulevel == 3) return launch_nt<VEC, GROUP, NCH, unroll_of(GROUP, NCH, 3)>(a, grid, st, nt, how);
+    return ulevel == 0 ? launch_nt<VEC, GROUP, NCH, unroll_of(GROUP, NCH, 0)>(a, grid, st, nt, how)
+                       : launch_nt<VEC, GROUP, NCH, unroll_of(GROUP, NCH, 1)>(a, grid, st, nt, how);
 }
 
 template <int VEC>
-hipError_t launch_group(const SpmmArgs &a, int grid, hipStream_t st, bool nt, int ulevel, int group, int nch) {
+hipError_t launch_group(const SpmmArgs &a, int grid, hipStream_t st, bool nt, int ulevel, int group, int nch, const How how) {
     if (nch == 1) {
         switch (group) {
             case 8:
-                return launch_u<VEC, 8, 1>(a, grid, st, nt, ulevel);
+                return launch_u<VEC, 8, 1>(a, grid, st, nt, ulevel, how);
             case 16:
-                return launch_u<VEC, 16, 1>(a, grid, st, nt, ulevel);
+                return launch_u<VEC, 16, 1>(a, grid, st, nt, ulevel, how);
             case 32:
-                return launch_u<VEC, 32, 1>(a, grid, st, nt, ulevel);
+                return launch_u<VEC, 32, 1>(a, grid, st, nt, ulevel, how);
             default:
-                return launch_u<VEC, 64, 1>(a, grid, st, nt, ulevel);
+                return launch_u<VEC, 64, 1>(a, grid, st, nt, ulevel, how);
         }
     }
-    if (nch == 2) return launch_u<VEC, 64, 2>(a, grid, st, nt, ulevel);
-    return launch_u<VEC, 64, 4>(a, grid, st, nt, ulevel);
+    if (nch == 2) return launch_u<VEC, 64, 2>(a, grid, st, nt, ulevel, how);
+    return launch_u<VEC, 64, 4>(a, grid, st, nt, ulevel, how);
+}
+
+hipError_t launch_vec(const SpmmArgs &a, int vec, int grid, hipStream_t st, const sgl::SpmmLayout &L, const How how) {
+    if (vec == 4) return launch_group<4>(a, grid, st, L.nt, L.ulevel, L.group, L.nch, how);
+    if (vec == 2) return launch_group<2>(a, grid, st, L.nt, L.ulevel, L.group, L.nch, how);
+    return launch_group<1>(a, grid, st, L.nt, L.ulevel, L.group, L.nch, how);
 }
 
 }
@@ -404,13 +459,21 @@
 static int spmm_slice(sgl_csr_t *h, const float *d_x, int64_t ldx, float *d_y, int64_t ldy, int d, int vec,
                       int accumulate, hipStream_t st, const EpiHost &eh, const char *who) {
     SpmmLaunch L;
-    int rc = spmm_launch(L, h, d / vec, d, false, who);
+    auto occ = [&](const sgl::SpmmLayout &lay) {
+        SpmmArgs q;
+        q.n_more = eh.n_more;
+        q.map.waves = lay.waves;
+        int w = 0;
+        (void)launch_vec(q, vec, 0, st, lay, How{&w, false});
+        return w;
+    };
+    int rc = spmm_launch(L, h, d / vec, d, false, ldx * (int64_t)sizeof(float), occ, who);
     if (rc == SGL_OK) rc = grow_partial(h, L.ldp);
     if (rc != SGL_OK) return rc;
     if (L.grid == 0) return SGL_OK;
 
     SpmmArgs a;
-    a.items = h->d_items;
+    a.items = L.items;
     a.pieces = h->d_pieces;
     a.rowptr = h->d_rowptr;
     a.col = h->d_col;
@@ -420,7 +483,7 @@
     a.ldx = ldx;
     a.ldy = ldy;
     a.ldp = L.ldp;
-    a.n_items = (int32_t)h->n_items;
+    a.n_items = (int32_t)L.n_items;
     a.n_pieces = (int32_t)h->n_pieces;
     a.d = d;
     a.accumulate = accumulate;
@@ -441,13 +504,7 @@
     a.rowmap = h->d_rowmap;
     a.map = L.map;
     a.partial = h->d_partial;
-    hipError_t e;
-    if (vec == 4)
-        e = launch_group<4>(a, L.grid, st, L.nt, L.ulevel, L.group, L.nch);
-    else if (vec == 2)
-        e = launch_group<2>(a, L.grid, st, L.nt, L.ulevel, L.group, L.nch);
-    else
-        e = launch_group<1>(a, L.grid, st, L.nt, L.ulevel, L.group, L.nch);
+    hipError_t e = launch_vec(a, vec, L.grid, st, L, How{nullptr, L.local});
     if (e != hipSuccess) return sgl::fail((int)e, "%s: kernel launch failed: %s", who, hipGetErrorString(e));
     if (L.fixup_grid > 0) {
         Epilogue fe;
diff --git a/sgl_amd/csrc/sgl_spmm_bf16.hip b/sgl_amd/csrc/sgl_spmm_bf16.hip
--- a/sgl_amd/csrc/sgl_spmm_bf16.hip
+++ b/sgl_amd/csrc/sgl_spmm_bf16.hip
@@ -331,35 +331,46 @@
 }
 
 template <int BV, int GROUP, int NCH, int U>
-hipError_t launch_variant(const Bf16Args &a, int grid, hipStream_t st) {
+hipError_t launch_variant(const Bf16Args &a, int grid, hipStream_t st, int *occ) {
+    if (occ) {
+        *occ = resident_waves_per_cu(spmm_bf16_kernel<BV, GROUP, NCH, U>, a.map.waves);
+        return hipSuccess;
+    }
     hipLaunchKernelGGL((spmm_bf16_kernel<BV, GROUP, NCH, U>), dim3(grid), dim3(64 * a.map.waves), 0, st, a);
     return hipGetLastError();
 }
 
 template <int BV, int GROUP, int NCH>
-hipError_t launch_u(const Bf16Args &a, int grid, hipStream_t st, int ulevel) {
+hipError_t launch_u(const Bf16Args &a, int grid, hipStream_t st, int ulevel, int *occ) {
     using sgl::unroll_of;
-    if (ulevel == 2) return launch_variant<BV, GROUP, NCH, unroll_of(GROUP, NCH, 2)>(a, grid, st);
-    return ulevel == 0 ? launch_variant<BV, GROUP, NCH, unroll_of(GROUP, NCH, 0)>(a, grid, st)
-                       : launch_variant<BV, GROUP, NCH, unroll_of(GROUP, NCH, 1)>(a, grid, st);
-}
-
-template <int BV>
-hipError_t launch_group(const Bf16Args &a, int grid, hipStream_t st, int ulevel, int group, int nch) {
+    if (ulevel == 2) return launch_variant<BV, GROUP, NCH, unroll_of(GROUP, NCH, 2)>(a, grid, st, occ);
+    return ulevel == 0 ? launch_variant<BV, GROUP, NCH, unroll_of(GROUP, NCH, 0)>(a, grid, st, occ)
+                       : launch_variant<BV, GROUP, NCH, unroll_of(GROUP, NCH, 1)>(a, grid, st, occ);
+}
+
+template <int BV>
+hipError_t launch_group(const Bf16Args &a, int grid, hipStream_t st, int ulevel, int group, int nch, int *occ) {
     if (nch == 1) {
         switch (group) {
             case 8:
-                return launch_u<BV, 8, 1>(a, grid, st, ulevel);
+                return launch_u<BV, 8, 1>(a, grid, st, ulevel, occ);
             case 16:
-                return launch_u<BV, 16, 1>(a, grid, st, ulevel);
+                return launch_u<BV, 16, 1>(a, grid, st, ulevel, occ);
             case 32:
-                return launch_u<BV, 32, 1>(a, grid, st, ulevel);
+                return launch_u<BV, 32, 1>(a, grid, st, ulevel, occ);
             default:
-                return launch_u<BV, 64, 1>(a, grid, st, ulevel);
-        }
-    }
-    if (nch == 2) return launch_u<BV, 64, 2>(a, grid, st, ulevel);
-    return launch_u<BV, 64, 4>(a, grid, st, ulevel);
+                return launch_u<BV, 64, 1>(a, grid, st, ulevel, occ);
+        }
+    }
+    if (nch == 2) return launch_u<BV, 64, 2>(a, grid, st, ulevel, occ);
+    return launch_u<BV, 64, 4>(a, grid, st, ulevel, occ);
+}
+
+hipError_t launch_bv(const Bf16Args &a, int bv, int grid, hipStream_t st, const sgl::SpmmLayout &L, int *occ) {
+    if (bv == 8) return launch_group<8>(a, grid, st, L.ulevel, L.group, L.nch, occ);
+    if (bv == 4) return launch_group<4>(a, grid, st, L.ulevel, L.group, L.nch, occ);
+    if (bv == 2) return launch_group<2>(a, grid, st, L.ulevel, L.group, L.nch, occ);
+    return launch_group<1>(a, grid, st, L.ulevel, L.group, L.nch, occ);
 }
 
 int pick_bv(const uint16_t *d_x, int64_t ldx, const uint16_t *d_y, int64_t ldy, int64_t d) {
@@ -371,13 +382,20 @@
 int spmm_slice(sgl_csr_t *h, const uint16_t *d_x, int64_t ldx, uint16_t *d_y, int64_t ldy, int d, int bv, hipStream_t st,
                const AccEpi &ah, const char *who) {
     SpmmLaunch L;
-    int rc = spmm_launch(L, h, d / bv, d, true, who);
+    auto occ = [&](const sgl::SpmmLayout &lay) {
+        Bf16Args q;
+        q.map.waves = lay.waves;
+        int w = 0;
+        (void)launch_bv(q, bv, 0, st, lay, &w);
+        return w;
+    };
+    int rc = spmm_launch(L, h, d / bv, d, true, ldx * (int64_t)sizeof(uint16_t), occ, who);
     if (rc == SGL_OK) rc = grow_partial(h, L.ldp);
     if (rc != SGL_OK) return rc;
     if (L.grid == 0) return SGL_OK;
 
     Bf16Args a;
-    a.items = h->d_items;
+    a.items = L.items;
     a.pieces = h->d_pieces;
     a.rowptr = h->d_rowptr;
     a.col = h->d_col;
@@ -387,22 +405,14 @@
     a.ldx = ldx;
     a.ldy = ldy;
     a.ldp = L.ldp;
-    a.n_items = (int32_t)h->n_items;
+    a.n_items = (int32_t)L.n_items;
     a.n_pieces = (int32_t)h->n_pieces;
     a.d = d;
     a.epi = ah;
     a.rowmap = h->d_rowmap;
     a.map = L.map;
     a.partial = h->d_partial;
-    hipError_t e;
-    if (bv == 8)
-        e = launch_group<8>(a, L.grid, st, L.ulevel, L.group, L.nch);
-    else if (bv == 4)
-        e = launch_group<4>(a, L.grid, st, L.ulevel, L.group, L.nch);
-    else if (bv == 2)
-        e = launch_group<2>(a, L.grid, st, L.ulevel, L.group, L.nch);
-    else
-        e = launch_group<1>(a, L.grid, st, L.ulevel, L.group, L.nch);
+    hipError_t e = launch_bv(a, bv, L.grid, st, L, nullptr);
     if (e != hipSuccess) return sgl::fail((int)e, "%s: kernel launch failed: %s", who, hipGetErrorString(e));
     if (L.fixup_grid > 0) {
         hipLaunchKernelGGL(spmm_bf16_fixup_kernel, dim3((unsigned)L.fixup_grid), dim3(256), 0, st, h->d_rowmap ? h->d_long_out : h->d_long_row,
diff --git a/sgl_amd/csrc/sgl_spmm_common.h b/sgl_amd/csrc/sgl_spmm_common.h
--- a/sgl_amd/csrc/sgl_spmm_common.h
+++ b/sgl_amd/csrc/sgl_spmm_common.h
@@ -1,5 +1,8 @@
 #pragma once
 #include "sgl_csr.h"
+
+#include <map>
+#include <mutex>
 
 namespace {
 
@@ -60,14 +63,49 @@
     BlockMap map;
     int64_t ldp;
     int grid, fixup_grid;
+    const int32_t *items;
+    int64_t n_items;
+    bool local;
 };
 
-int spmm_launch(SpmmLaunch &L, const sgl_csr_t *h, int lanes, int d, bool bf16, const char *who) {
+template <typename K>
+int resident_waves_per_cu(K kernel, int waves) {
+    static std::mutex mu;
+    static std::map<std::pair<const void *, int>, int> known;
+    const std::pair<const void *, int> key(reinterpret_cast<const void *>(kernel), waves);
+    std::lock_guard<std::mutex> lk(mu);
+    auto it = known.find(key);
+    if (it != known.end()) return it->second;
+    int blocks = 0;
+    if (hipOccupancyMaxActiveBlocksPerMultiprocessor(&blocks, kernel, 64 * waves, 0) != hipSuccess || blocks <= 0) {
+        (void)hipGetLastError();
+        blocks = 32 / waves;
+    }
+    known[key] = blocks * waves;
+    return blocks * waves;
+}
+
+template <typename Occ>
+int spmm_launch(SpmmLaunch &L, sgl_csr_t *h, int lanes, int d, bool bf16, int64_t row_bytes, Occ occ, const char *who) {
     static_cast<sgl::SpmmLayout &>(L) = sgl::spmm_layout(lanes, (h->flags & SGL_CSR_STRICT_ORDER) != 0, h->nnz, h->n_rows, bf16);
     L.ldp = bf16 ? (d + 7) / 8 * 8 : (d + 3) / 4 * 4;
     L.map.waves = L.waves;
     L.map.piece_blocks = (int32_t)((h->n_pieces + L.waves - 1) / L.waves);
-    const int64_t item_blocks = (h->n_items + L.waves - 1) / L.waves;
+    int list = 0;
+    bool local = false;
+    if (h->lists.size() > 1 && sgl::tuning("spmm_local", 0) != 2) {
+        int32_t list_nnz[8];
+        const int n_lists = (int)std::min<size_t>(h->lists.size(), 8);
+        for (int k = 0; k < n_lists; ++k) list_nnz[k] = h->lists[(size_t)k].item_nnz;
+        list = sgl::pick_local_list(h->loc_counts(), h->n_rows, h->n_cols, h->nnz, row_bytes, occ(static_cast<const sgl::SpmmLayout &>(L)),
+                                    list_nnz, n_lists, &local);
+    }
+    L.items = list > 0 ? h->lists[(size_t)list].d_items : h->d_items;
+    L.n_items = list > 0 ? h->lists[(size_t)list].n_items : h->n_items;
+    L.local = local;
+    h->last_local = local ? 1 : 0;
+    h->last_item_nnz = list > 0 ? h->lists[(size_t)list].item_nnz : h->item_nnz;
+    const int64_t item_blocks = (L.n_items + L.waves - 1) / L.waves;
     L.map.xcd_remap = (!(h->flags & SGL_CSR_NO_XCD_REMAP) && sgl::tuning("spmm_xcd_remap", 1) != 0) ? 1 : 0;
     L.map.item_blocks_per_xcd = (int32_t)((item_blocks + 7) / 8);
     const int64_t grid64 = L.map.piece_blocks + (L.map.xcd_remap ? (int64_t)L.map.item_blocks_per_xcd * 8 : item_blocks);
diff --git a/sgl_amd/device.py b/sgl_amd/device.py
--- a/sgl_amd/device.py
+++ b/sgl_amd/device.py
@@ -260,6 +260,15 @@
         check(lib().sgl_csr_info(self._h, a), "sgl_csr_info")
         keys = ("n_rows", "n_cols", "nnz", "n_items", "n_pieces", "n_long_rows", "flags", "workspace_bytes")
         return dict(zip(keys, list(a)))
+
+    LOCALITY_WINDOWS = (1024, 2048, 4096, 8192, 16384)
+
+    def locality(self):
+        a = (c_int64 * 8)()
+        check(lib().sgl_csr_locality(self._h, a), "sgl_csr_locality")
+        tot = max(int(a[0]), 1)
+        return {"sampled_nnz": int(a[0]), "share_within": {w: a[1 + k] / tot for k, w in enumerate(self.LOCALITY_WINDOWS)},
+                "local": bool(a[6]), "item_nnz": int(a[7])}
 
     def spmm(self, x, out=None, accumulate=False):
         _check_mat(x, "x", bf16=True)
```

Result: no change. 1449 billion (median of 2 runs) (+0.1%).
